# michiyasunaga/qagnn

Measured on AMD Instinct MI355X. Metric: QA-subgraphs/sec (batch x num_choice) fwd+bwd, higher is better.
Workload: dtype f32; 1 GPU; configs[1]: CSQA-shaped batch 64 questions x 5 choices = 320 subgraphs per GPU, n=200 node slots, 400..2000 edges/subgraph, 38 relations (run_qagnn__csqa.sh), 5-layer GAT d=200 H=4, QAGNN decoder fwd+bwd (LM encoder excluded: random sent_vecs), dropout 0.2, train-mode BN; subgraphs_per_gpu=320, nodes=64000, edges=396800, edges_with_self_loops=460800, graph_input=load-time int32 blobs (qagnn_graph_from_blobs), 13.3 B/edge on the wire, parallelism=single

## Files before the change

### include/qagnn_hip.h

```cpp
#ifndef QAGNN_HIP_H
#define QAGNN_HIP_H

#include <stdint.h>

#ifdef __cplusplus
extern "C" {
#endif

#define QAGNN_OK 0
#define QAGNN_EINVAL 1
#define QAGNN_EUNSUPPORTED 2
#define QAGNN_EHIP 3

typedef void* qagnn_stream_t;

const char* qagnn_last_error(void);
int qagnn_abi_version(void);

typedef struct qagnn_graph {
  int32_t N, E, Ep, R, T, C;
  int32_t* rowptr_s;
  int32_t* tgt_s;
  int32_t* src_s;
  int32_t* cls_s;
// ... 147 lines not shown

int qagnn_seed_epoch_advance(uint64_t delta, qagnn_stream_t stream);
int qagnn_seed_epoch_set(uint64_t value, qagnn_stream_t stream);

int qagnn_edge_attn_fwd_f32(const qagnn_graph* g, const float* KMQ, int32_t ldk, const float* EkEm, int32_t lde, int32_t HP,
                            float qscale, float* score, float* a, float* alpha, float* aggr, int32_t lda,
                            qagnn_stream_t stream);
int qagnn_edge_attn_bwd_f32(const qagnn_graph* g, const float* KMQ, int32_t ldk, const float* EkEm, int32_t lde, int32_t HP,
                            float qscale, const float* a, const float* alpha, const float* G, int32_t ldg, float* dKMQ,
                            float* dEkEm, float* ga, float* rs, float* cls_part, qagnn_stream_t stream);

typedef struct qagnn_hop_args {
  const qagnn_graph* g;
  int32_t N, DP, SP, HP, T;
  float qscale;
  const float* X;
  const float* S;
  const int64_t* ntype;
  const float* Wx_t; const float* Wx;
  const float* Ws_t; const float* Ws;
  const float* TT;
  const float* EkEm;
  const float* W1t; const float* W1; const float* b1;
  const float* gamma; const float* beta;
  const float* W2t; const float* W2; const float* b2;
  int32_t batch_stats;
  float eps;
  const float* run_mean_p; const float* run_var_p;
  float* run_mean; float* run_var; int64_t* num_batches_tracked;
  const int64_t* dense_pos; int32_t d; float momentum;
  int32_t apply_act; float p_drop; uint64_t seed;
  float* KMQ;
  float* a; float* alpha;
  float* aggr; float* h1; float* out; float* y;
  float* stats;
  const float* dy;
  float* dX;
  float* dS;
  int32_t accumulate_dS; int32_t accumulate_dX;
  float* dWx_t; float* dWs_t;
  float* dTT; float* dEkEm;
  float* dW1t; float* db1;
  float* dbn;
  float* dW2t; float* db2;
  float* ws; int64_t ws_elems;
  int32_t gemm_split;
  int32_t ones_col;
  int32_t tab_col;
  qagnn_stream_t side_stream;
  uint32_t* amax;
  const uint32_t* x_amax;
  const uint32_t* s_amax;
} qagnn_hop_args;
#define QAGNN_HOP_AMAX_WORDS 16
int64_t qagnn_hop_fwd_workspace_elems(int32_t N, int32_t Ep, int32_t DP);
int64_t qagnn_hop_bwd_workspace_elems(int32_t N, int32_t Ep, int32_t DP, int32_t SP,
                                      int32_t cls_part_rows );
int qagnn_hop_fwd_f32(const qagnn_hop_args* h, qagnn_stream_t stream);
int qagnn_hop_bwd_f32(const qagnn_hop_args* h, qagnn_stream_t stream);
int qagnn_stack_fwd_f32(const qagnn_hop_args* hops, int32_t k, qagnn_stream_t stream);
int qagnn_stack_bwd_f32(const qagnn_hop_args* hops, int32_t k, qagnn_stream_t stream);

int qagnn_node_prep_f32(const float* raw_scores, const int64_t* adj_len, const int64_t* node_type, const int64_t* concept_ids,
                        int32_t B, int32_t n, float* score, uint8_t* mask, int64_t* ridx, int64_t table_rows, int32_t* err,
                        qagnn_stream_t stream);

int qagnn_radam_step_f32(int32_t n_tensors, float* const* p, const float* const* g, float* const* m, float* const* v,
                         const int64_t* numel, double beta1, double beta2, double eps, double lr, double weight_decay, double step_size,
                         int32_t mode, qagnn_stream_t stream);

#ifdef __cplusplus
}
#endif
#endif
```

### qagnn_amd/_lib.py

```python
import ctypes as C
import functools
import os

import torch

_HERE = os.path.dirname(os.path.abspath(__file__))
LIB_PATH = os.environ.get('QAGNN_LIB') or os.path.join(_HERE, 'libqagnn_hip.so')

EXPORTS = ['qagnn_last_error', 'qagnn_abi_version', 'qagnn_graph_storage_elems', 'qagnn_graph_prep', 'qagnn_graph_prep_blocked',
           'qagnn_graph_from_blobs', 'qagnn_radam_step_f32', 'qagnn_node_prep_f32', 'qagnn_seed_epoch_advance', 'qagnn_seed_epoch_set',
           'qagnn_gemm_nn_f32', 'qagnn_gemm_nn_split_f32', 'qagnn_gemm_nn_pack_bytes', 'qagnn_gemm_nn_ws_bytes', 'qagnn_gemm_nn_split_ws_f32', 'qagnn_gemm_nn_prepack_bytes', 'qagnn_gemm_nn_prepack_f32',
           'qagnn_gemm_nn_prepack_clear', 'qagnn_gemm_tn_workspace_elems', 'qagnn_gemm_tn_f32', 'qagnn_gemm_tn2_f32', 'qagnn_gemm_tn_colsum_f32',
           'qagnn_colreduce_workspace_elems', 'qagnn_colreduce_f32', 'qagnn_bn_finalize_f32', 'qagnn_bn_stats_finalize_f32', 'qagnn_bn_relu_bwd_f32',
           'qagnn_gelu_dropout_fwd_f32', 'qagnn_gelu_dropout_bwd_f32', 'qagnn_sin_basis_f32',
           'qagnn_bn_relu_bwd_colsum_f32',
           'qagnn_pool_attn_fwd_f32', 'qagnn_pool_attn_bwd_f32', 'qagnn_head_post_fwd_f32', 'qagnn_head_post_bwd_f32', 'qagnn_add_row0_f32', 'qagnn_gather_multi_f32', 'qagnn_gather_multi_sum_f32',
           'qagnn_edge_attn_fwd_f32', 'qagnn_edge_attn_bwd_f32',
           'qagnn_hop_fwd_workspace_elems', 'qagnn_hop_bwd_workspace_elems', 'qagnn_hop_fwd_f32', 'qagnn_hop_bwd_f32',
           'qagnn_stack_fwd_f32', 'qagnn_stack_bwd_f32', 'qagnn_absmax_f32', 'qagnn_zero_words', 'qagnn_gemm_tn_h2_f32', 'qagnn_gelu_dropout_fwd_amax_f32', 'qagnn_gelu_dropout_amax_scratch_elems',
           'qagnn_timing_enable', 'qagnn_timing_read', 'qagnn_gemm_tn_h1_f32', 'qagnn_gelu_dropout_bwd_amax_f32', 'qagnn_packed_min_rows']

CLS_SLICES = 4
ABI_VERSION = 22

_i32, _i64, _f32, _u64, _vp = C.c_int32, C.c_int64, C.c_float, C.c_uint64, C.c_void_p


class qagnn_graph(C.Structure):
    _fields_ = ([(n, _i32) for n in ('N', 'E', 'Ep', 'R', 'T', 'C')] +
                [(n, _vp) for n in ('rowptr_s', 'tgt_s', 'src_s', 'cls_s', 'eid_s', 'rowptr_t', 'src_t', 'tgt_t', 'cls_t', 'pos_t',
                                    'cls_count', 'src_c', 'tgt_c', 'pos_c', 'chunk_cls', 'chunk_beg',
                                    'chunk_len', 'n_chunks', 'chunkptr')] +
                [('max_chunks', _i32), ('err', _vp), ('block_n', _i32), ('n_groups', _i32)])


GATHER_MAX = 160


class qagnn_gather_tabs(C.Structure):
    _fields_ = [('p', _vp * GATHER_MAX), ('n', _i32)]


class qagnn_pack_desc(C.Structure):
    _fields_ = [('B1n', _vp), ('ldn1', _i32), ('K1', _i32), ('B2n', _vp), ('ldn2', _i32), ('K2', _i32), ('No', _i32), ('pieces', _i32)]


class qagnn_gemm_nn_args(C.Structure):
    _fields_ = [('A1', _vp), ('lda1', _i32), ('K1', _i32), ('B1', _vp), ('ldb1', _i32),
                ('A2', _vp), ('lda2', _i32), ('K2', _i32), ('B2', _vp), ('ldb2', _i32),
                ('C', _vp), ('ldc', _i32), ('M', _i32), ('No', _i32),
                ('bias', _vp), ('rowtab', _vp), ('ldt', _i32), ('rowidx', _vp),
                ('a_scale', _vp), ('a_shift', _vp), ('accumulate', _i32), ('a_rowidx', _vp), ('xcd_remap', _i32), ('colstat_part', _vp),
                ('a_amax1', _vp), ('a_amax2', _vp), ('a_rows', _i64), ('pieces', _i32)]


class qagnn_hop_args(C.Structure):
    _fields_ = ([('g', C.POINTER(qagnn_graph))] + [(n, _i32) for n in ('N', 'DP', 'SP', 'HP', 'T')] + [('qscale', _f32)] +
                [(n, _vp) for n in ('X', 'S', 'ntype', 'Wx_t', 'Wx', 'Ws_t', 'Ws', 'TT', 'EkEm', 'W1t', 'W1', 'b1', 'gamma', 'beta',
                                    'W2t', 'W2', 'b2')] +
                [('batch_stats', _i32), ('eps', _f32), ('run_mean_p', _vp), ('run_var_p', _vp), ('run_mean', _vp), ('run_var', _vp),
                 ('num_batches_tracked', _vp), ('dense_pos', _vp), ('d', _i32), ('momentum', _f32),
                 ('apply_act', _i32), ('p_drop', _f32), ('seed', _u64)] +
                [(n, _vp) for n in ('KMQ', 'a', 'alpha', 'aggr', 'h1', 'out', 'y', 'stats', 'dy', 'dX', 'dS')] +
                [('accumulate_dS', _i32), ('accumulate_dX', _i32)] +
                [(n, _vp) for n in ('dWx_t', 'dWs_t', 'dTT', 'dEkEm', 'dW1t', 'db1', 'dbn', 'dW2t', 'db2', 'ws')] +
                [('ws_elems', _i64), ('gemm_split', _i32), ('ones_col', _i32), ('tab_col', _i32), ('side_stream', _vp), ('amax', _vp), ('x_amax', _vp), ('s_amax', _vp)])


HOP_AMAX_WORDS = 16


def load_library(path=LIB_PATH):
    if not os.path.exists(path):
        raise OSError(f'{path} not found: build it with `python -m qagnn_amd.build` (hipcc, gfx950)')
    lib = C.CDLL(path)
    lib.qagnn_last_error.restype = C.c_char_p
    lib.qagnn_abi_version.restype = _i32
    lib.qagnn_graph_storage_elems.restype = _i64
    lib.qagnn_graph_storage_elems.argtypes = [_i32, _i32, _i32, _i32]
    lib.qagnn_graph_prep.argtypes = [C.POINTER(qagnn_graph), _vp, _vp, _vp, _vp, _i32, _i32, _i32, _i32, _vp]
    lib.qagnn_graph_prep_blocked.argtypes = [C.POINTER(qagnn_graph), _vp, _vp, _vp, _vp, _i32, _i32, _i32, _i32, _i32, _vp]
    lib.qagnn_graph_from_blobs.argtypes = [C.POINTER(qagnn_graph), _vp, _vp, _vp, _vp, _vp, _i32, _i32, _i32, _i32, _i32, _vp]
    lib.qagnn_node_prep_f32.argtypes = [_vp, _vp, _vp, _vp, _i32, _i32, _vp, _vp, _vp, _i64, _vp, _vp]
    lib.qagnn_seed_epoch_advance.argtypes = [_u64, _vp]
    lib.qagnn_seed_epoch_set.argtypes = [_u64, _vp]
    lib.qagnn_radam_step_f32.argtypes = [_i32, _vp, _vp, _vp, _vp, _vp] + [C.c_double] * 6 + [_i32, _vp]
    lib.qagnn_gemm_nn_f32.argtypes = [C.POINTER(qagnn_gemm_nn_args), _vp]
    lib.qagnn_gemm_nn_split_f32.argtypes = [C.POINTER(qagnn_gemm_nn_args), _vp, _i32, _vp, _i32, _vp]
    lib.qagnn_gemm_nn_pack_bytes.restype = _i64
    lib.qagnn_gemm_nn_pack_bytes.argtypes = [_i32, _i32, _i32]
    lib.qagnn_gemm_nn_split_ws_f32.argtypes = [C.POINTER(qagnn_gemm_nn_args), _vp, _i32, _vp, _i32, _vp, _i64, _vp]
    lib.qagnn_gemm_nn_ws_bytes.restype = _i64
    lib.qagnn_gemm_nn_ws_bytes.argtypes = [C.POINTER(qagnn_gemm_nn_args), _vp, _i32, _vp, _i32]
    lib.qagnn_gemm_nn_prepack_bytes.restype = _i64
    lib.qagnn_gemm_nn_prepack_bytes.argtypes = [C.POINTER(qagnn_pack_desc), _i32]
    lib.qagnn_gemm_nn_prepack_f32.argtypes = [C.POINTER(qagnn_pack_desc), _i32, _vp, _i64, _i64, _vp]
    lib.qagnn_gemm_nn_prepack_clear.argtypes = [_i64]
    lib.qagnn_gemm_tn_workspace_elems.restype = _i64
    lib.qagnn_gemm_tn_workspace_elems.argtypes = [_i32, _i32, _i32]
    lib.qagnn_gemm_tn_f32.argtypes = [_vp, _i32, _vp, _i32, _vp, _i32, _i32, _i32, _i32, _vp, _vp, _vp, _i32, _vp, _vp]
    lib.qagnn_gemm_tn2_f32.argtypes = [_vp, _i32, _i32, _vp, _i32, _i32, _vp, _i32, _vp, _i32, _i32, _i32, _vp, _vp]
    lib.qagnn_gemm_tn_h2_f32.argtypes = [_vp, _i32, _i32, _vp, _i32, _i32, _vp, _i32, _vp, _i32, _i32, _i32, _vp, _vp, _vp, _vp, _vp, _vp, _vp]
    lib.qagnn_gemm_tn_h1_f32.argtypes = lib.qagnn_gemm_tn_h2_f32.argtypes
    lib.qagnn_absmax_f32.argtypes = [_vp, _i64, _vp, _vp]
    lib.qagnn_zero_words.argtypes = [_vp, _i64, _vp]
    lib.qagnn_timing_enable.argtypes = [_i32]
    lib.qagnn_timing_read.argtypes = [_vp, _vp]
    lib.qagnn_packed_min_rows.restype = _i64
    lib.qagnn_packed_min_rows.argtypes = [_i64]
    lib.qagnn_gemm_tn_colsum_f32.argtypes = [_vp, _i32, _vp, _i32, _vp, _i32, _i32, _i32, _i32, _vp, _vp, _vp, _i32, _vp, _vp, _i32,
                                             _vp, _vp]
    lib.qagnn_colreduce_workspace_elems.restype = _i64
    lib.qagnn_colreduce_workspace_elems.argtypes = [_i32, _i32, _i32]
    lib.qagnn_colreduce_f32.argtypes = [_i32, _vp, _i32, _vp, _i32, _i32, _i32, _vp, _i32, _vp, _vp, _vp, _vp, _vp, _f32, _vp, _vp, _vp]
    lib.qagnn_bn_finalize_f32.argtypes = [_vp, _vp, _vp, _vp, _f32, _vp, _vp, _vp, _i32, _vp, _vp, _vp, _vp, _i32, _f32, _f32, _i32, _vp]
    lib.qagnn_bn_stats_finalize_f32.argtypes = [_vp, _i32, _i32, _i32, _vp, _vp, _f32, _vp, _vp, _vp, _vp, _vp, _i32, _f32, _f32, _i32, _vp]
    lib.qagnn_bn_relu_bwd_f32.argtypes = [_vp, _vp, _vp, _i32, _i32, _i32, _vp, _vp, _vp, _vp, _vp, _vp, _vp, _f32, _vp, _vp]
    lib.qagnn_gelu_dropout_fwd_f32.argtypes = [_vp, _vp, _i64, _f32, _u64, _vp]
    lib.qagnn_gelu_dropout_bwd_f32.argtypes = [_vp, _vp, _vp, _i64, _f32, _u64, _vp]
    lib.qagnn_gelu_dropout_fwd_amax_f32.argtypes = [_vp, _vp, _i64, _f32, _u64, _vp, _vp, _vp]
    lib.qagnn_gelu_dropout_bwd_amax_f32.argtypes = [_vp, _vp, _vp, _i64, _f32, _u64, _vp, _vp, _vp]
    lib.qagnn_gelu_dropout_amax_scratch_elems.restype = _i64
# ... 821 lines not shown
```

### qagnn_amd/csrc/common.h

```cpp
#pragma once
#include <hip/hip_runtime.h>
#include <stdint.h>
#include <stdio.h>

#include <type_traits>

#include "../../include/qagnn_hip.h"

namespace qagnn {

void set_error(const char* fmt, ...);

struct NnProduct {
  const qagnn_gemm_nn_args* a;
  bool split;
  const float* B1n; int ldn1; const float* B2n; int ldn2;
  void* ws; int64_t ws_bytes;
};
enum class NnFamily { FP32, SPLIT, NN2 };
enum class NnB { IN_KERNEL, PACK, IMAGE };
struct NnRoute {
  NnFamily family;
  int nt, np, wv;
  bool affine, flat, stats;
  NnB b; const void* image;
  int64_t ws_bytes;
  int ntiles, grid;
};
inline int num_cus() {
  static int n = [] {
    int dev = 0, v = 0;
    if (hipGetDevice(&dev) != hipSuccess || hipDeviceGetAttribute(&v, hipDeviceAttributeMultiprocessorCount, dev) != hipSuccess || v <= 0) v = 256;
    return v;
  }();
  return n;
}
static inline int cdiv(int64_t a, int64_t b) { return (int)((a + b - 1) / b); }
inline void nn_grid(NnRoute& r, int M, int No, int rows_per_tile, int per_cu) {
  r.ntiles = cdiv(No, r.nt * 16) * cdiv(M, rows_per_tile);
  const int cap = (num_cus() * per_cu) & ~7;
  r.grid = r.ntiles < cap ? r.ntiles : cap;
}
NnRoute nn_route(const NnProduct& p);
bool nn_rows_packed(int64_t M);
int gemm_nn(const NnProduct& p, hipStream_t stream);
int launch_nn(const NnRoute& r, const qagnn_gemm_nn_args& a, hipStream_t stream);
int launch_nn_split(const NnRoute& r, const qagnn_gemm_nn_args& a, const float* B1n, int ldn1, const float* B2n, int ldn2, hipStream_t stream);
int launch_nn2(const NnRoute& r, const qagnn_gemm_nn_args& a, const float* B1n, int ldn1, const float* B2n, int ldn2, hipStream_t stream);
int launch_pack_b(int np, const qagnn_gemm_nn_args& a, const float* B1n, int ldn1, const float* B2n, int ldn2, void* ws, hipStream_t stream);
namespace nn2 { int walk_tiles(int K1, int K2); }
int64_t nn2_pack_bytes(int No, int K1, int K2, int np);
const void* nn2_prepack_lookup(const float* B1n, int ldn1, int K1, const float* B2n, int ldn2, int K2, int No, int np);

struct TnProduct {
  const float* A1; int lda1, Ka1;
  const float* A2; int lda2, Ka2; bool two;
  const float* B; int ldb;
  float* C; int ldc, R, No;
  const float* a_scale; const float* a_shift; const int64_t* a_rowidx; int accumulate;
  float* bsum; const int64_t* b_rowidx; int groups;
  const uint32_t* amax[3]; int np;
  float* ws;
};
inline TnProduct tn_product(const float* A1, int lda1, int Ka1, const float* A2, int lda2, int Ka2, const float* B, int ldb, float* C, int ldc, int R,
                            int No, const float* a_scale, const float* a_shift, float* ws, const uint32_t* amax_a1 = nullptr,
                            const uint32_t* amax_a2 = nullptr, const uint32_t* amax_b = nullptr, int np = 3) {
  TnProduct p = {};
  p.A1 = A1; p.lda1 = lda1; p.Ka1 = Ka1;
  if (A2 && Ka2 > 0) { p.A2 = A2; p.lda2 = lda2; p.Ka2 = Ka2; p.two = true; }
  p.B = B; p.ldb = ldb; p.C = C; p.ldc = ldc; p.R = R; p.No = No; p.a_scale = a_scale; p.a_shift = a_shift; p.ws = ws;
  p.amax[0] = amax_a1; p.amax[1] = amax_a2; p.amax[2] = amax_b; p.np = np;
  return p;
}
enum class TnFamily { RUNTIME, STRIP, SPLIT, WS, PAIR };
struct TnRoute {
  TnFamily family;
  int kt, nt, waves, np;
  bool affine, gather, colsum;
  int chunk_rows, nchunks;
  bool sum_by4;
  dim3 grid;
  int64_t ws_elems;
};
TnRoute tn_route(const TnProduct& p);
int gemm_tn(const TnProduct& p, hipStream_t stream);
int launch_tn(const TnRoute& r, const TnProduct& p, float* Pcs, hipStream_t stream);
int launch_tn_strip(const TnRoute& r, const TnProduct& p, float* Pcs, hipStream_t stream);
int launch_tn_split(const TnRoute& r, const TnProduct& p, hipStream_t stream);
int launch_tn_ws(const TnRoute& r, const TnProduct& p, hipStream_t stream);
int launch_sum_chunks(const float* P, float* C, int ldc, int rows, int No, int nchunks, int accumulate, bool by4, hipStream_t stream);

int launch_gelu_dropout(const float* X, const float* dY, float* out, int64_t n, float p, uint64_t seed, uint32_t* amax, float* amax_part,
                        hipStream_t stream);
int64_t gelu_amax_scratch_elems(int64_t n);
int launch_bn_relu_bwd_colsum(const float* dR, const float* Hh, float* dH, int ld, int R, int Cc, const float* mean, const float* invstd,
                              const float* scale, const float* shift, const float* gamma, const float* sum_dy, const float* sum_dy_hhat,
                              float inv_rows, const float* roww, float* colsum, float* workspace, uint32_t* amax, hipStream_t stream);
int launch_bn_stats_finalize(const float* part, int n_tiles, int R, int Cc, const float* gamma, const float* beta, float eps, float* stats,
                             float* run_mean, float* run_var, int64_t* nbt, int d, float momentum, float unbias, int ones_col, uint32_t* amax_bound,
                             hipStream_t stream);

int launch_edge_attn_fwd(const qagnn_graph* g, const float* KMQ, int32_t ldk, const float* EkEm, int32_t lde, int32_t HP, float qscale,
                         float* score, float* a, float* alpha, float* aggr, int32_t lda, float* amax_part , hipStream_t stream);
int launch_edge_attn_bwd(const qagnn_graph* g, const float* KMQ, int32_t ldk, const float* EkEm, int32_t lde, int32_t HP, float qscale,
                         const float* a, const float* alpha, const float* G, int32_t ldg, float* dKMQ, float* dEkEm, float* ga, float* rs,
                         float* cls_part, float* amax_part , uint32_t* amax_slot, hipStream_t stream);
int launch_amax_reduce(const float* part, int64_t n, uint32_t* slot, hipStream_t stream);

struct TimedScope {
  int kind;
  hipStream_t s;
  hipEvent_t e0, e1;
  bool counted;
  TimedScope(int kind, hipStream_t s);
  ~TimedScope();
  TimedScope(const TimedScope&) = delete;
  TimedScope& operator=(const TimedScope&) = delete;
};

#define QAGNN_REQUIRE(cond, code, ...) \
  do {                                 \
    if (!(cond)) {                     \
      qagnn::set_error(__VA_ARGS__);   \
      return (code);                   \
    }                                  \
  } while (0)

#define QAGNN_LAUNCH_CHECK(name)                                               \
  do {                                                                         \
    hipError_t e__ = hipGetLastError();                                        \
    if (e__ != hipSuccess) {                                                   \
      qagnn::set_error("%s launch failed: %s", name, hipGetErrorString(e__));  \
      return QAGNN_EHIP;                                                       \
    }                                                                          \
  } while (0)

#ifndef QAGNN_NN_OCC
#define QAGNN_NN_OCC 2
#endif

template <int V0, int... Vs, class F>
inline int dispatch_int(int v, F&& f) {
  if constexpr (sizeof...(Vs) == 0) return f(std::integral_constant<int, V0>{});
  else return v == V0 ? f(std::integral_constant<int, V0>{}) : dispatch_int<Vs...>(v, f);
}
template <class F>
inline int dispatch_bool(bool v, F&& f) { return v ? f(std::true_type{}) : f(std::false_type{}); }

template <auto KERNEL>
inline int raise_lds_limit(int bytes, const char* name) {
  static bool raised[64] = {};
  int dev = 0;
  if (hipGetDevice(&dev) != hipSuccess) dev = 0;
  if (bytes <= 64 * 1024 || raised[dev & 63]) return QAGNN_OK;
  hipError_t e = hipFuncSetAttribute((const void*)KERNEL, hipFuncAttributeMaxDynamicSharedMemorySize, bytes);
  if (e != hipSuccess) { set_error("%s: cannot raise the dynamic LDS limit: %s", name, hipGetErrorString(e)); return QAGNN_EHIP; }
// ... 96 lines not shown
  const f16x2 l = {(_Float16)(xs - (float)h[0]), (_Float16)(ys - (float)h[1])};
  hi = __builtin_bit_cast(uint32_t, h);
  lo = __builtin_bit_cast(uint32_t, l);
}
#define QAGNN_BF(V) __builtin_bit_cast(bf16x8, V)
#define QAGNN_HF(V) __builtin_bit_cast(f16x8, V)
template <int NP, bool SWAP = false>
__device__ __forceinline__ f32x4s mfma_pieces(const u32x4s* __restrict__ a, const u32x4s* __restrict__ b, f32x4s c) {
#define QAGNN_MF3(I, J) c = SWAP ? __builtin_amdgcn_mfma_f32_16x16x32_bf16(QAGNN_BF(b[J]), QAGNN_BF(a[I]), c, 0, 0, 0) \
                                 : __builtin_amdgcn_mfma_f32_16x16x32_bf16(QAGNN_BF(a[I]), QAGNN_BF(b[J]), c, 0, 0, 0);
#define QAGNN_MF2(I, J) c = SWAP ? __builtin_amdgcn_mfma_f32_16x16x32_f16(QAGNN_HF(b[J]), QAGNN_HF(a[I]), c, 0, 0, 0) \
                                 : __builtin_amdgcn_mfma_f32_16x16x32_f16(QAGNN_HF(a[I]), QAGNN_HF(b[J]), c, 0, 0, 0);
  if constexpr (NP == 3) {
    QAGNN_MF3(2, 0) QAGNN_MF3(0, 2) QAGNN_MF3(1, 1) QAGNN_MF3(1, 0) QAGNN_MF3(0, 1) QAGNN_MF3(0, 0)
  } else if constexpr (NP == 2) {
    QAGNN_MF2(1, 0) QAGNN_MF2(0, 1) QAGNN_MF2(0, 0)
  } else {
    QAGNN_MF2(0, 0)
  }
#undef QAGNN_MF3
#undef QAGNN_MF2
  return c;
}

__device__ __forceinline__ float4 ld4(const float* p) { return *reinterpret_cast<const float4*>(p); }
__device__ __forceinline__ void st4(float* p, float4 v) { *reinterpret_cast<float4*>(p) = v; }
__device__ __forceinline__ float dot4(float4 a, float4 b) { return a.x * b.x + a.y * b.y + a.z * b.z + a.w * b.w; }
__device__ __forceinline__ float4 add4(float4 a, float4 b) { return make_float4(a.x + b.x, a.y + b.y, a.z + b.z, a.w + b.w); }
__device__ __forceinline__ float4 fma4(float s, float4 a, float4 acc) {
  return make_float4(fmaf(s, a.x, acc.x), fmaf(s, a.y, acc.y), fmaf(s, a.z, acc.z), fmaf(s, a.w, acc.w));
}

__device__ __forceinline__ float wave_amax_lane63(float m) {
  m = row16_max(m);
  int b = __builtin_bit_cast(int, m);
  m = fmaxf(m, __builtin_bit_cast(float, __builtin_amdgcn_update_dpp(b, b, 0x142, 0xA, 0xF, false)));
  b = __builtin_bit_cast(int, m);
  m = fmaxf(m, __builtin_bit_cast(float, __builtin_amdgcn_update_dpp(b, b, 0x143, 0xC, 0xF, false)));
  return m;
}
__device__ __forceinline__ void block_amax_merge(float m, uint32_t* __restrict__ amax, float* __restrict__ red) {
  m = wave_amax_lane63(m);
  const int lane = threadIdx.x & 63, w = threadIdx.x >> 6, nw = (blockDim.x + 63) >> 6;
  if (lane == 63) red[w] = m;
  __syncthreads();
  if (threadIdx.x == 0) {
    float t = red[0];
    for (int i = 1; i < nw; ++i) t = fmaxf(t, red[i]);
    if (t > 0.f) __hip_atomic_fetch_max(amax, __builtin_bit_cast(uint32_t, t), __ATOMIC_RELAXED, __HIP_MEMORY_SCOPE_AGENT);
  }
}
__device__ __forceinline__ float absmax4(float4 v) { return fmaxf(fmaxf(fabsf(v.x), fabsf(v.y)), fmaxf(fabsf(v.z), fabsf(v.w))); }


}
```

### qagnn_amd/csrc/edge_attn.hip

```cpp
#include "common.h"

namespace qagnn {

#ifndef EDGE_UNROLL
#define EDGE_UNROLL 4
#endif
#define TGT_UNROLL 4

typedef __amdgpu_buffer_rsrc_t rsrc_t;
constexpr uint32_t OOB_OFF = 0x7FFFFFF0u;
__device__ __forceinline__ rsrc_t make_rsrc(const void* base, uint32_t bytes) {
  return __builtin_amdgcn_make_buffer_rsrc(const_cast<void*>(base), 0, (int)bytes, 0x00020000);
}
__device__ __forceinline__ float4 buf_ld4(rsrc_t r, uint32_t voff, uint32_t soff) {
  return __builtin_bit_cast(float4, __builtin_amdgcn_raw_buffer_load_b128(r, (int)voff, (int)soff, 0));
}

constexpr int SLAB_ROWS = 72;

struct Lane {
  int lane, w, g, j;
  bool act;
  uint32_t voff;
  int off;
// ... 100 lines not shown
    sc[grp] = -INFINITY;
    if (grp * 16 < cnt) {
      const int gcnt = min(16, cnt - grp * 16);
      for (int i = 0; i < gcnt; i += EDGE_UNROLL) {
        float4 k[EDGE_UNROLL], ek[EDGE_UNROLL];
#pragma unroll
        for (int u = 0; u < EDGE_UNROLL; ++u) {
          const int idx = min(grp * 16 + i + u, cnt - 1);
          k[u] = buf_ld4(rK, L.voff, rl(tv, idx));
          ek[u] = buf_ld4(rE, L.voff, rl(cv, idx));
        }
#pragma unroll
        for (int u = 0; u < EDGE_UNROLL; ++u) {
          const float p = row16_sum(dot4(q, add4(k[u], ek[u]))) * qscale;
          sc[grp] = (L.j == i + u) ? p : sc[grp];
        }
      }
    }
  }
  float m = sc[0];
  m = (L.j < cnt) ? m : -INFINITY;
#pragma unroll
  for (int grp = 1; grp < 4; ++grp)
    if (grp * 16 < cnt) m = (grp * 16 + L.j < cnt) ? fmaxf(m, sc[grp]) : m;
  m = row16_max(m);
  float ex[4], sum = 0.f;
#pragma unroll
  for (int grp = 0; grp < 4; ++grp) {
    ex[grp] = 0.f;
    if (grp * 16 < cnt) {
      ex[grp] = (grp * 16 + L.j < cnt) ? expf(sc[grp] - m) : 0.f;
      sum += ex[grp];
    }
  }
  sum = row16_sum(sum) + 1e-16f;
#pragma unroll
  for (int grp = 0; grp < 4; ++grp) {
    if (grp * 16 < cnt) {
      if (grp * 16 + L.j < cnt) {
        const float av = ex[grp] / sum;
        const int64_t o = (int64_t)(beg + grp * 16 + L.j) * 4 + L.g;
        a[o] = av;
        alpha[o] = av * deg;
      }
    }
  }
}

__device__ __forceinline__ void node_amax(float m, float* __restrict__ part, int node) {
  m = wave_amax_lane63(m);
  if ((threadIdx.x & 63) == 63) part[node] = m;
}

__global__ __launch_bounds__(256) void k_edge_aggregate(const int* __restrict__ rowptr_t, const int* __restrict__ src_t,
                                                        const int* __restrict__ cls_t, const int* __restrict__ pos_t,
                                                        const float* __restrict__ KMQ, int ldk, const float* __restrict__ EkEm,
                                                        int lde, int HP, const float* __restrict__ alpha,
                                                        float* __restrict__ aggr, int lda, int N, int C, const int* __restrict__ xcd_base,
                                                        float* __restrict__ amax_part) {
  __shared__ float4 slab[4][SLAB_ROWS];
  const int t = wave_node(xcd_base);
  if (t >= N) return;
  const Lane L = lane_info(HP);
  const int DP = 4 * HP;
  const uint32_t pk = (uint32_t)ldk * 4u, pe = (uint32_t)lde * 4u, vm = L.voff + (uint32_t)DP * 4u;
  const rsrc_t rK = make_rsrc(KMQ, (uint32_t)N * pk), rE = make_rsrc(EkEm, (uint32_t)C * pe);
  const int beg = __builtin_amdgcn_readfirstlane(rowptr_t[t]), end = __builtin_amdgcn_readfirstlane(rowptr_t[t + 1]);
  if (end - beg == 1) {
    const int sv = __builtin_amdgcn_readfirstlane(src_t[beg]), cv = __builtin_amdgcn_readfirstlane(cls_t[beg]);
    const int pv = __builtin_amdgcn_readfirstlane(pos_t[beg]);
    const float4 m1 = buf_ld4(rK, vm, (uint32_t)sv * pk), em1 = buf_ld4(rE, vm, (uint32_t)cv * pe);
    const float al = alpha[(int64_t)pv * 4 + L.g];
    const float4 o1 = fma4(al, add4(m1, em1), zero4());
    if (L.act) st4(aggr + (int64_t)t * lda + L.off, o1);
    if (amax_part) node_amax(L.act ? absmax4(o1) : 0.f, amax_part, t);
    return;
  }
  slab_init(slab[L.w], L.lane);
  const float* const sl = reinterpret_cast<const float*>(slab[L.w]) + L.g;
  float4 acc = zero4();
  for (int e0 = beg; e0 < end; e0 += 64) {
    const int cnt = min(64, end - e0), lc = e0 + min(L.lane, cnt - 1);
    const uint32_t sv = (uint32_t)src_t[lc] * pk, cv = (uint32_t)cls_t[lc] * pe;
    slab[L.w][L.lane] = L.lane < cnt ? ld4(alpha + (int64_t)pos_t[lc] * 4) : zero4();
    for (int i = 0; i < cnt; i += EDGE_UNROLL) {
      float4 m[EDGE_UNROLL], em[EDGE_UNROLL];
#pragma unroll
      for (int u = 0; u < EDGE_UNROLL; ++u) {
        const int idx = min(i + u, cnt - 1);
        m[u] = buf_ld4(rK, vm, rl(sv, idx));
        em[u] = buf_ld4(rE, vm, rl(cv, idx));
      }
#pragma unroll
      for (int u = 0; u < EDGE_UNROLL; ++u) acc = fma4(sl[(i + u) * 4], add4(m[u], em[u]), acc);
    }
  }
  if (L.act) st4(aggr + (int64_t)t * lda + L.off, acc);
  if (amax_part) node_amax(L.act ? absmax4(acc) : 0.f, amax_part, t);
}

__global__ __launch_bounds__(256) void k_edge_bwd_src1(const int* __restrict__ rowptr_s, const int* __restrict__ tgt_s,
                                                       const int* __restrict__ cls_s, const float* __restrict__ KMQ, int ldk,
                                                       const float* __restrict__ EkEm, int lde, int HP,
                                                       const float* __restrict__ a, const float* __restrict__ alpha,
                                                       const float* __restrict__ G, int ldg, float* __restrict__ dKMQ,
                                                       float* __restrict__ ga, float* __restrict__ rs, int N, int C,
                                                       const int* __restrict__ xcd_base, float* __restrict__ amax_part) {
  __shared__ float4 slab[3][4][SLAB_ROWS];
  const int s = wave_node(xcd_base);
  if (s >= N) return;
  const Lane L = lane_info(HP);
  const int DP = 4 * HP;
  const uint32_t pk = (uint32_t)ldk * 4u, pe = (uint32_t)lde * 4u, pg = (uint32_t)ldg * 4u, vm = L.voff + (uint32_t)DP * 4u;
  const rsrc_t rK = make_rsrc(KMQ, (uint32_t)N * pk), rE = make_rsrc(EkEm, (uint32_t)C * pe), rG = make_rsrc(G, (uint32_t)N * pg);
  const int beg = __builtin_amdgcn_readfirstlane(rowptr_s[s]), end = __builtin_amdgcn_readfirstlane(rowptr_s[s + 1]);
  if (end - beg == 1) {
    const float4 g1 = buf_ld4(rG, L.voff, (uint32_t)s * pg);
    if (L.act) st4(dKMQ + (int64_t)s * ldk + DP + L.off, g1);
    if (amax_part) node_amax(L.act ? absmax4(g1) : 0.f, amax_part, s);
    if (L.lane == 0) {
      st4(ga + (int64_t)beg * 4, zero4());
      st4(rs + (int64_t)s * 4, zero4());
    }
    return;
  }
  const float4 mrow = buf_ld4(rK, vm, (uint32_t)s * pk);
  const float deg = (float)(end - beg);
  slab_init(slab[0][L.w], L.lane);
  slab_init(slab[1][L.w], L.lane);
  const float* const sl_a = reinterpret_cast<const float*>(slab[0][L.w]) + L.g;
  const float* const sl_al = reinterpret_cast<const float*>(slab[1][L.w]) + L.g;
  float* const sl_ga = reinterpret_cast<float*>(slab[2][L.w]) + L.g;
  float4 dM = zero4();
  float r = 0.f;
  for (int e0 = beg; e0 < end; e0 += 64) {
    const int cnt = min(64, end - e0), lc = e0 + min(L.lane, cnt - 1);
    const uint32_t tv = (uint32_t)tgt_s[lc] * pg, cv = (uint32_t)cls_s[lc] * pe;
    slab[0][L.w][L.lane] = L.lane < cnt ? ld4(a + (int64_t)lc * 4) : zero4();
    slab[1][L.w][L.lane] = L.lane < cnt ? ld4(alpha + (int64_t)lc * 4) : zero4();
    for (int i = 0; i < cnt; i += EDGE_UNROLL) {
      float4 g4[EDGE_UNROLL], em[EDGE_UNROLL];
#pragma unroll
      for (int u = 0; u < EDGE_UNROLL; ++u) {
        const int idx = min(i + u, cnt - 1);
        g4[u] = buf_ld4(rG, L.voff, rl(tv, idx));
        em[u] = buf_ld4(rE, vm, rl(cv, idx));
      }
#pragma unroll
      for (int u = 0; u < EDGE_UNROLL; ++u) {
        dM = fma4(sl_al[(i + u) * 4], g4[u], dM);
        const float gae = deg * row16_sum(dot4(add4(mrow, em[u]), g4[u]));
// ... 165 lines not shown
    int seen = 0;
    for (int g = sl; g < NG; g += QAGNN_CLS_SLICES) {
      const int kb = cp_lo[g], ke = cp_hi[g];
      const int first = (part - seen % P + P) % P;
      for (int k = kb + first; k < ke; k += P) acc = add4(acc, ld4(cls_part + (int64_t)k * DP2 + col4 * 4));
      seen += ke - kb;
    }
    sm4[part * ncol4 + col4] = acc;
  }
  __syncthreads();
  if (threadIdx.x < ncol4) {
    float4 s = sm4[threadIdx.x];
    for (int q = 1; q < P; ++q) s = add4(s, sm4[q * ncol4 + threadIdx.x]);
    st4(slices + ((int64_t)c * QAGNN_CLS_SLICES + sl) * DP2 + threadIdx.x * 4, s);
  }
}
__global__ __launch_bounds__(256) void k_cls_reduce2(const float* __restrict__ slices, float* __restrict__ dEkEm, int lde, int DP2, int C,
                                                     const float* __restrict__ amax_part, int npart, uint32_t* __restrict__ amax_slot) {
  const int ncol4 = DP2 >> 2;
  const int i = blockIdx.x * blockDim.x + threadIdx.x;
  if (i < C * ncol4) {
    const int c = i / ncol4, col4 = i - c * ncol4;
    const float* p = slices + (int64_t)c * QAGNN_CLS_SLICES * DP2 + col4 * 4;
    float4 s = ld4(p);
#pragma unroll
    for (int q = 1; q < QAGNN_CLS_SLICES; ++q) s = add4(s, ld4(p + (int64_t)q * DP2));
    st4(dEkEm + (int64_t)c * lde + col4 * 4, s);
  }
  if (amax_part) {
    __shared__ float red[16];
    float m = 0.f;
    for (int k = i; k < npart; k += (int)(gridDim.x * blockDim.x)) m = fmaxf(m, amax_part[k]);
    block_amax_merge(m, amax_slot, red);
  }
}

static int check_common(const qagnn_graph* g, const float* KMQ, int ldk, const float* EkEm, int lde, int HP, const char* who) {
  QAGNN_REQUIRE(g && KMQ && EkEm, QAGNN_EINVAL, "%s: null pointer", who);
  QAGNN_REQUIRE(HP > 0 && HP % 4 == 0 && HP <= 64, QAGNN_EUNSUPPORTED, "%s: head pitch HP=%d must be a multiple of 4, <= 64", who, HP);
  QAGNN_REQUIRE(ldk >= 12 * HP && ldk % 4 == 0 && lde >= 8 * HP && lde % 4 == 0, QAGNN_EINVAL, "%s: ldk=%d lde=%d too small for HP=%d",
                who, ldk, lde, HP);
  QAGNN_REQUIRE(aligned16(KMQ) && aligned16(EkEm), QAGNN_EINVAL, "%s: operands must be 16-byte aligned", who);
  QAGNN_REQUIRE((int64_t)g->N * ldk * 4 < (int64_t)OOB_OFF && (int64_t)g->C * lde * 4 < (int64_t)OOB_OFF, QAGNN_EUNSUPPORTED,
                "%s: N=%d x ldk=%d floats exceed the 2 GiB a buffer descriptor of these kernels addresses", who, g->N, ldk);
  return QAGNN_OK;
}

}

using namespace qagnn;

namespace qagnn {
int launch_edge_attn_fwd(const qagnn_graph* g, const float* KMQ, int32_t ldk, const float* EkEm, int32_t lde, int32_t HP, float qscale,
                         float* score, float* a, float* alpha, float* aggr, int32_t lda, float* amax_part, hipStream_t stream) {
  TimedScope timed(2, stream);
  int rc = check_common(g, KMQ, ldk, EkEm, lde, HP, "edge_attn_fwd");
  if (rc != QAGNN_OK) return rc;
  QAGNN_REQUIRE(score && a && alpha && aggr && lda >= 4 * HP && lda % 4 == 0 && aligned16(aggr), QAGNN_EINVAL,
                "edge_attn_fwd: bad output arguments");
  const int nb = 8 * edge_xcd_cap(g->N);
  k_edge_scores<<<nb, 256, 0, stream>>>(g->rowptr_s, g->tgt_s, g->cls_s, KMQ, ldk, EkEm, lde, HP, qscale, score, a, alpha, g->N, g->C, g->err + 4);
  QAGNN_LAUNCH_CHECK("k_edge_scores");
  k_edge_aggregate<<<nb, 256, 0, stream>>>(g->rowptr_t, g->src_t, g->cls_t, g->pos_t, KMQ, ldk, EkEm, lde, HP, alpha, aggr, lda, g->N, g->C, g->err + 4, amax_part);
  QAGNN_LAUNCH_CHECK("k_edge_aggregate");
  return QAGNN_OK;
}
}

extern "C" int qagnn_edge_attn_fwd_f32(const qagnn_graph* g, const float* KMQ, int32_t ldk, const float* EkEm, int32_t lde,
                                       int32_t HP, float qscale, float* score, float* a, float* alpha, float* aggr, int32_t lda,
                                       qagnn_stream_t stream_) {
  return launch_edge_attn_fwd(g, KMQ, ldk, EkEm, lde, HP, qscale, score, a, alpha, aggr, lda, nullptr, (hipStream_t)stream_);
}

extern "C" int qagnn_edge_attn_bwd_f32(const qagnn_graph* g, const float* KMQ, int32_t ldk, const float* EkEm, int32_t lde,
                                       int32_t HP, float qscale, const float* a, const float* alpha, const float* G, int32_t ldg,
                                       float* dKMQ, float* dEkEm, float* ga, float* rs, float* cls_part, qagnn_stream_t stream_) {
  return launch_edge_attn_bwd(g, KMQ, ldk, EkEm, lde, HP, qscale, a, alpha, G, ldg, dKMQ, dEkEm, ga, rs, cls_part, nullptr, nullptr, (hipStream_t)stream_);
}

int qagnn::launch_edge_attn_bwd(const qagnn_graph* g, const float* KMQ, int32_t ldk, const float* EkEm, int32_t lde, int32_t HP, float qscale,
                                const float* a, const float* alpha, const float* G, int32_t ldg, float* dKMQ, float* dEkEm, float* ga, float* rs,
                                float* cls_part, float* amax_part, uint32_t* amax_slot, hipStream_t stream) {
  TimedScope timed(3, stream);
  int rc = check_common(g, KMQ, ldk, EkEm, lde, HP, "edge_attn_bwd");
  if (rc != QAGNN_OK) return rc;
  QAGNN_REQUIRE(a && alpha && G && dKMQ && dEkEm && ga && rs && cls_part, QAGNN_EINVAL, "edge_attn_bwd: null pointer");
  QAGNN_REQUIRE(ldg >= 4 * HP && ldg % 4 == 0 && aligned16(G) && aligned16(dKMQ) && aligned16(dEkEm) && aligned16(cls_part),
                QAGNN_EINVAL, "edge_attn_bwd: bad pitch / alignment");
  QAGNN_REQUIRE((int64_t)g->N * ldg * 4 < (int64_t)OOB_OFF, QAGNN_EUNSUPPORTED, "edge_attn_bwd: G exceeds 2 GiB");
  const int DP2 = 8 * HP;
  QAGNN_REQUIRE(DP2 / 4 <= 1024, QAGNN_EUNSUPPORTED, "edge_attn_bwd: HP too large");
  const int nb = 8 * edge_xcd_cap(g->N);
  k_edge_bwd_src1<<<nb, 256, 0, stream>>>(g->rowptr_s, g->tgt_s, g->cls_s, KMQ, ldk, EkEm, lde, HP, a, alpha, G, ldg, dKMQ, ga, rs, g->N, g->C, g->err + 4, amax_part);
  QAGNN_LAUNCH_CHECK("k_edge_bwd_src1");
  k_edge_bwd_src2<<<nb, 256, 0, stream>>>(g->rowptr_s, g->tgt_s, g->cls_s, KMQ, ldk, EkEm, lde, HP, qscale, a, dKMQ, ga, rs, g->N, g->C, g->err + 4, amax_part ? amax_part + g->N : nullptr);
  QAGNN_LAUNCH_CHECK("k_edge_bwd_src2");
  k_edge_bwd_tgt<<<nb, 256, 0, stream>>>(g->rowptr_t, g->src_t, g->pos_t, KMQ, ldk, HP, ga, dKMQ, g->N, g->err + 4, amax_part ? amax_part + 2 * (int64_t)g->N : nullptr);
  QAGNN_LAUNCH_CHECK("k_edge_bwd_tgt");
  k_edge_bwd_cls<<<cdiv(g->max_chunks, 4), 256, 0, stream>>>(g->n_chunks, g->chunk_beg, g->chunk_len, g->src_c, g->tgt_c, g->pos_c,
                                                             KMQ, ldk, HP, alpha, ga, G, ldg, cls_part, g->N);
  QAGNN_LAUNCH_CHECK("k_edge_bwd_cls");
  const int cr_threads = g->Ep < 65536 && DP2 / 4 <= 128 ? 256 : 1024;
  const int P = cr_threads / (DP2 / 4);
  float* slices = cls_part + (int64_t)g->max_chunks * DP2;
  k_cls_reduce<<<dim3(g->C, QAGNN_CLS_SLICES), cr_threads, (size_t)P * (DP2 / 4) * sizeof(float4), stream>>>(g->chunkptr, cls_part, slices, DP2,
                                                                                                          g->C, g->n_groups);
  QAGNN_LAUNCH_CHECK("k_cls_reduce");
  k_cls_reduce2<<<cdiv((int64_t)g->C * (DP2 / 4), 256), 256, 0, stream>>>(slices, dEkEm, lde, DP2, g->C, amax_slot ? amax_part : nullptr, 3 * g->N, amax_slot);
  QAGNN_LAUNCH_CHECK("k_cls_reduce2");
  return QAGNN_OK;
}
```

### qagnn_amd/csrc/elementwise.hip

```cpp
#include "common.h"

namespace qagnn {

constexpr int CR_WR_BIG = 32, CR_WR_SMALL = 8;
static inline int cr_wr(int R) { return R < 32768 ? CR_WR_SMALL : CR_WR_BIG; }

template <int MODE, int CR_WR>
__global__ __launch_bounds__(256) void k_colreduce(const float* __restrict__ X, int ldx, const float* __restrict__ X2, int ldx2,
                                                   int R, int Cc, const int64_t* __restrict__ rowidx, int groups,
                                                   const float* __restrict__ mean, const float* __restrict__ invstd,
                                                   const float* __restrict__ scale, const float* __restrict__ shift,
                                                   const float* __restrict__ roww, float* __restrict__ part) {
  constexpr int NOUT = MODE == 0 ? 4 : (MODE == 2 ? 2 : 1);
  __shared__ __attribute__((aligned(16))) float red[4][NOUT][256];
  const int lane = threadIdx.x & 63, w = threadIdx.x >> 6;
  const int col = blockIdx.x * 256 + lane * 4;
  const bool act = col < Cc;
  constexpr int CR_ROWS = 4 * CR_WR;
  const int r0 = blockIdx.y * CR_ROWS + w * CR_WR;
  float4 acc[NOUT];
#pragma unroll
  for (int o = 0; o < NOUT; ++o) acc[o] = make_float4(0.f, 0.f, 0.f, 0.f);
  float4 mu = make_float4(0.f, 0.f, 0.f, 0.f), is = mu, sc = mu, sh = mu;
  if (act && MODE >= 1) mu = ld4(mean + col);
// ... 174 lines not shown
    }
    __syncthreads();
  }
  if (q == 0 && c < Cc) {
    const float mean = a.mean, var = fmaxf(a.m2 / (float)R, 0.f);
    const float is = rsqrtf(var + eps), sc = gamma[c] * is;
    stats[c] = mean;
    stats[Cc + c] = var;
    stats[2 * Cc + c] = is;
    stats[3 * Cc + c] = c == ones_col ? 0.f : sc;
    stats[4 * Cc + c] = c == ones_col ? 1.f : beta[c] - mean * sc;
    if (amax_bound) {
      const float bnd = c == ones_col ? 1.f : 1.01f * (fabsf(gamma[c]) * sqrtf((float)R) + fabsf(beta[c]));
      atomicMax(amax_bound, __builtin_bit_cast(uint32_t, bnd));
    }
    if (run_mean) {
      const int HP = Cc >> 2, dh = d >> 2, h = c / HP, j = c - h * HP;
      if (j < dh) {
        const int i = h * dh + j;
        run_mean[i] += momentum * (mean - run_mean[i]);
        run_var[i] += momentum * (var * unbias - run_var[i]);
      }
    }
  }
  if (nbt && blockIdx.x == 0 && threadIdx.x == 0) *nbt += 1;
}

__device__ __forceinline__ float gelu_f(float x) {
  const float u = 0.7978845608028654f * (x + 0.044715f * x * x * x);
  return 0.5f * x * (1.f + tanhf(u));
}
__device__ __forceinline__ float gelu_grad_f(float x) {
  const float x2 = x * x;
  const float u = 0.7978845608028654f * (x + 0.044715f * x * x2);
  const float t = tanhf(u);
  return 0.5f * (1.f + t) + 0.5f * x * (1.f - t * t) * 0.7978845608028654f * (1.f + 3.f * 0.044715f * x2);
}
template <bool BWD>
__device__ __forceinline__ float4 gelu_dropout_val(float4 x, float4 g, int64_t i, float p, uint64_t seed, float inv) {
  float4 o;
#define ONE(f, k)                                                                  \
  {                                                                                \
    const float keep = (p > 0.f && uniform01(seed, (uint64_t)i * 4 + k) < p) ? 0.f : inv; \
    o.f = BWD ? g.f * keep * gelu_grad_f(x.f) : keep * gelu_f(x.f);                \
  }
  ONE(x, 0) ONE(y, 1) ONE(z, 2) ONE(w, 3)
#undef ONE
  return o;
}
template <bool BWD>
__device__ __forceinline__ float4 gelu_dropout_one(const float* __restrict__ X, const float* __restrict__ dY, int64_t i, float p, uint64_t seed, float inv) {
  return gelu_dropout_val<BWD>(ld4(X + i * 4), BWD ? ld4(dY + i * 4) : make_float4(1.f, 1.f, 1.f, 1.f), i, p, seed, inv);
}
template <bool BWD, bool AMAX = false>
__global__ __launch_bounds__(256) void k_gelu_dropout(const float* __restrict__ X, const float* __restrict__ dY, float* __restrict__ out, int64_t n4,
                                                      float p, uint64_t seed, const unsigned long long* __restrict__ epoch,
                                                      float* __restrict__ amax_part = nullptr) {
  if (p > 0.f) seed = epoch_seed(seed, epoch);
  const float inv = p > 0.f ? 1.f / (1.f - p) : 1.f;
  const int64_t i = (int64_t)blockIdx.x * blockDim.x + threadIdx.x;
  if (!AMAX && i >= n4) return;
  float4 o = make_float4(0.f, 0.f, 0.f, 0.f);
  if (i < n4) {
    o = gelu_dropout_one<BWD>(X, dY, i, p, seed, inv);
    st4(out + i * 4, o);
  }
  if constexpr (AMAX) {
    __shared__ float red[4];
    const float m = wave_amax_lane63(absmax4(o));
    if ((threadIdx.x & 63) == 63) red[threadIdx.x >> 6] = m;
    __syncthreads();
    if (threadIdx.x == 0) amax_part[blockIdx.x] = fmaxf(fmaxf(red[0], red[1]), fmaxf(red[2], red[3]));
  }
}

template <bool N1>
__global__ __launch_bounds__(256) void k_absmax(const float* __restrict__ x, int64_t n, uint32_t* __restrict__ slot) {
  __shared__ float red[16];
  float m = 0.f;
  for (int64_t i = (int64_t)blockIdx.x * 256 + threadIdx.x; i < n; i += (int64_t)gridDim.x * 256) {
    if constexpr (N1) m = fmaxf(m, fabsf(x[i]));
    else m = fmaxf(m, absmax4(ld4(x + i * 4)));
  }
  block_amax_merge(m, slot, red);
}
__global__ void k_zero_words(uint32_t* __restrict__ p, int64_t n) {
  for (int64_t i = (int64_t)blockIdx.x * blockDim.x + threadIdx.x; i < n; i += (int64_t)gridDim.x * blockDim.x) p[i] = 0u;
}

template <int CR_WR>
__global__ __launch_bounds__(256) void k_bn_relu_bwd_colsum(const float* __restrict__ dR, const float* __restrict__ Hh, float* __restrict__ dH,
                                                            int ld, int R, int Cc, const float* __restrict__ mean,
                                                            const float* __restrict__ invstd, const float* __restrict__ scale,
                                                            const float* __restrict__ shift, const float* __restrict__ gamma,
                                                            const float* __restrict__ k1v, const float* __restrict__ k2v, float inv_rows,
                                                            const float* __restrict__ roww, float* __restrict__ part,
                                                            uint32_t* __restrict__ amax) {
  __shared__ __attribute__((aligned(16))) float red[4][256];
  const int lane = threadIdx.x & 63, w = threadIdx.x >> 6;
  const int col = blockIdx.x * 256 + lane * 4;
  const bool act = col < Cc;
  constexpr int CR_ROWS = 4 * CR_WR;
  const int r0 = blockIdx.y * CR_ROWS + w * CR_WR;
  float4 acc = make_float4(0.f, 0.f, 0.f, 0.f);
  float am = 0.f;
  if (act) {
    const float4 mu = ld4(mean + col), is = ld4(invstd + col), sc = ld4(scale + col), sh = ld4(shift + col);
    const float4 ga = ld4(gamma + col), k1 = ld4(k1v + col), k2 = ld4(k2v + col);
    const int rend = min(R, r0 + CR_WR);
    for (int rb = r0; rb < rend; rb += 8) {
      float4 xs[8], hs[8];
#pragma unroll
      for (int u = 0; u < 8; ++u) {
        const int r = min(rb + u, rend - 1);
        xs[u] = ld4(dR + (int64_t)r * ld + col);
        hs[u] = ld4(Hh + (int64_t)r * ld + col);
      }
#pragma unroll
      for (int u = 0; u < 8; ++u) {
        const int r = rb + u;
        if (r >= rend) break;
        const float4 x = xs[u], h = hs[u];
        const float ir = roww ? roww[r] : inv_rows;
        float4 o;
#define ONE(f)                                                          \
// ... 118 lines not shown

namespace qagnn {
int launch_bn_stats_finalize(const float* part, int n_tiles, int R, int Cc, const float* gamma, const float* beta, float eps, float* stats,
                             float* run_mean, float* run_var, int64_t* nbt, int d, float momentum, float unbias, int ones_col, uint32_t* amax_bound,
                             hipStream_t stream) {
  k_bn_stats_finalize<<<cdiv(Cc, BF_COLS), BF_COLS * BF_PARTS, 0, stream>>>(part, n_tiles, R, Cc, gamma, beta, eps, stats, run_mean, run_var, nbt, d,
                                                                            momentum, unbias, ones_col, amax_bound);
  QAGNN_LAUNCH_CHECK("k_bn_stats_finalize");
  return QAGNN_OK;
}
}

extern "C" int qagnn_bn_stats_finalize_f32(const float* part, int32_t n_tiles, int32_t R, int32_t Cc, const float* gamma, const float* beta,
                                           float eps, float* stats, float* run_mean, float* run_var, int64_t* num_batches_tracked,
                                           const int64_t* dense_pos, int32_t d, float momentum, float unbias, int32_t ones_col,
                                           qagnn_stream_t stream_) {
  hipStream_t stream = (hipStream_t)stream_;
  QAGNN_REQUIRE(part && gamma && beta && stats && R > 0 && Cc > 0 && n_tiles == cdiv(R, ST_TILE), QAGNN_EINVAL,
                "bn_stats_finalize: bad arguments (R=%d needs %d tiles of %d rows, got %d)", R, cdiv(R, ST_TILE), ST_TILE, n_tiles);
  QAGNN_REQUIRE(!run_mean || (run_var && d > 0 && d % 4 == 0 && Cc % 4 == 0 && d <= Cc), QAGNN_EINVAL, "bn_stats_finalize: running-stat arguments");
  (void)dense_pos;
  return launch_bn_stats_finalize(part, n_tiles, R, Cc, gamma, beta, eps, stats, run_mean, run_var, num_batches_tracked, d, momentum, unbias, ones_col,
                                  nullptr, stream);
}

__global__ __launch_bounds__(256) void k_gather_multi(qagnn_gather_tabs t, const int* __restrict__ tid, const int* __restrict__ off,
                                                     float* __restrict__ out, int total) {
  __shared__ const float* ps[QAGNN_GATHER_MAX];
  for (int i = threadIdx.x; i < t.n; i += blockDim.x) ps[i] = t.p[i];
  __syncthreads();
  const int i = blockIdx.x * blockDim.x + threadIdx.x;
  if (i >= total) return;
  const int k = tid[i];
  out[i] = k >= 0 ? ps[k][off[i]] : 0.f;
}

__global__ __launch_bounds__(256) void k_gather_multi_sum(qagnn_gather_tabs t, const int* __restrict__ tid, const int* __restrict__ off, int K, int S,
                                                         float* __restrict__ out) {
  __shared__ const float* ps[QAGNN_GATHER_MAX];
  for (int i = threadIdx.x; i < t.n; i += blockDim.x) ps[i] = t.p[i];
  __syncthreads();
  const int s = blockIdx.x * blockDim.x + threadIdx.x;
  if (s >= S) return;
  float acc = 0.f;
  for (int k = 0; k < K; ++k) {
    const int g = tid[(int64_t)k * S + s];
    const float* p = g >= 0 ? ps[g] : nullptr;
    const float v = p != nullptr ? p[off[(int64_t)k * S + s]] : 0.f;
    acc = k == 0 ? v : acc + v;
  }
  out[s] = acc;
}

extern "C" int qagnn_gather_multi_f32(const qagnn_gather_tabs* t, const int32_t* tid, const int32_t* off, float* out, int32_t total,
                                      qagnn_stream_t stream_) {
  QAGNN_REQUIRE(t && t->n > 0 && t->n <= QAGNN_GATHER_MAX && tid && off && out && total > 0, QAGNN_EINVAL, "gather_multi: bad arguments");
  for (int i = 0; i < t->n; ++i) QAGNN_REQUIRE(t->p[i] != nullptr, QAGNN_EINVAL, "gather_multi: null source %d", i);
  k_gather_multi<<<cdiv(total, 256), 256, 0, (hipStream_t)stream_>>>(*t, tid, off, out, total);
  QAGNN_LAUNCH_CHECK("k_gather_multi");
  return QAGNN_OK;
}

extern "C" int qagnn_gather_multi_sum_f32(const qagnn_gather_tabs* t, const int32_t* tid, const int32_t* off, int32_t K, int32_t S, float* out,
                                          qagnn_stream_t stream_) {
  QAGNN_REQUIRE(t && t->n > 0 && t->n <= QAGNN_GATHER_MAX && tid && off && out && K > 0 && S > 0, QAGNN_EINVAL, "gather_multi_sum: bad arguments");
  k_gather_multi_sum<<<cdiv(S, 256), 256, 0, (hipStream_t)stream_>>>(*t, tid, off, K, S, out);
  QAGNN_LAUNCH_CHECK("k_gather_multi_sum");
  return QAGNN_OK;
}

namespace qagnn {
int64_t gelu_amax_scratch_elems(int64_t n) { return cdiv(n / 4, 256); }
int launch_gelu_dropout(const float* X, const float* dY, float* out, int64_t n, float p, uint64_t seed, uint32_t* amax, float* amax_part,
                        hipStream_t stream) {
  const int grid = cdiv(n / 4, 256);
  if (amax && !amax_part) { set_error("gelu_dropout: the maximum needs its scratch"); return QAGNN_EINVAL; }
  if (dY) {
    if (amax) k_gelu_dropout<true, true><<<grid, 256, 0, stream>>>(X, dY, out, n / 4, p, seed, seed_epoch_ptr(), amax_part);
    else k_gelu_dropout<true><<<grid, 256, 0, stream>>>(X, dY, out, n / 4, p, seed, seed_epoch_ptr());
  } else {
    if (amax) k_gelu_dropout<false, true><<<grid, 256, 0, stream>>>(X, nullptr, out, n / 4, p, seed, seed_epoch_ptr(), amax_part);
    else k_gelu_dropout<false><<<grid, 256, 0, stream>>>(X, nullptr, out, n / 4, p, seed, seed_epoch_ptr());
  }
  QAGNN_LAUNCH_CHECK("k_gelu_dropout");
  return amax ? launch_amax_reduce(amax_part, grid, amax, stream) : QAGNN_OK;
}
}

extern "C" int qagnn_gelu_dropout_fwd_f32(const float* X, float* Y, int64_t n, float p, uint64_t seed, qagnn_stream_t stream_) {
  hipStream_t stream = (hipStream_t)stream_;
  QAGNN_REQUIRE(X && Y && n > 0 && n % 4 == 0 && aligned16(X) && aligned16(Y), QAGNN_EINVAL, "gelu_dropout_fwd: bad args");
  QAGNN_REQUIRE(p >= 0.f && p < 1.f, QAGNN_EINVAL, "gelu_dropout_fwd: p=%f", p);
  return launch_gelu_dropout(X, nullptr, Y, n, p, seed, nullptr, nullptr, stream);
}

extern "C" int64_t qagnn_gelu_dropout_amax_scratch_elems(int64_t n) { return gelu_amax_scratch_elems(n); }
extern "C" int qagnn_gelu_dropout_fwd_amax_f32(const float* X, float* Y, int64_t n, float p, uint64_t seed, uint32_t* amax, float* scratch,
                                               qagnn_stream_t stream_) {
  QAGNN_REQUIRE(X && Y && amax && scratch && n > 0 && n % 4 == 0 && aligned16(X) && aligned16(Y), QAGNN_EINVAL, "gelu_dropout_fwd_amax: bad args");
  QAGNN_REQUIRE(p >= 0.f && p < 1.f, QAGNN_EINVAL, "gelu_dropout_fwd_amax: p=%f", p);
  return launch_gelu_dropout(X, nullptr, Y, n, p, seed, amax, scratch, (hipStream_t)stream_);
}

extern "C" int qagnn_gelu_dropout_bwd_amax_f32(const float* X, const float* dY, float* dX, int64_t n, float p, uint64_t seed, uint32_t* amax,
                                               float* scratch, qagnn_stream_t stream_) {
  QAGNN_REQUIRE(X && dY && dX && amax && scratch && n > 0 && n % 4 == 0 && aligned16(X) && aligned16(dY) && aligned16(dX), QAGNN_EINVAL,
                "gelu_dropout_bwd_amax: bad args");
  QAGNN_REQUIRE(p >= 0.f && p < 1.f, QAGNN_EINVAL, "gelu_dropout_bwd_amax: p=%f", p);
  return launch_gelu_dropout(X, dY, dX, n, p, seed, amax, scratch, (hipStream_t)stream_);
}

extern "C" int qagnn_gelu_dropout_bwd_f32(const float* X, const float* dY, float* dX, int64_t n, float p, uint64_t seed,
                                          qagnn_stream_t stream_) {
  hipStream_t stream = (hipStream_t)stream_;
  QAGNN_REQUIRE(X && dY && dX && n > 0 && n % 4 == 0 && aligned16(X) && aligned16(dY) && aligned16(dX), QAGNN_EINVAL,
                "gelu_dropout_bwd: bad args");
  QAGNN_REQUIRE(p >= 0.f && p < 1.f, QAGNN_EINVAL, "gelu_dropout_bwd: p=%f", p);
  return launch_gelu_dropout(X, dY, dX, n, p, seed, nullptr, nullptr, stream);
}

extern "C" int qagnn_absmax_f32(const float* x, int64_t n, uint32_t* slot, qagnn_stream_t stream_) {
  QAGNN_REQUIRE(x && slot && n > 0 && n % 4 == 0 && aligned16(x), QAGNN_EINVAL, "absmax: bad arguments");
  const int64_t n4 = n / 4;
  const int grid = (int)(n4 / 256 + 1 < 1024 ? n4 / 256 + 1 : 1024);
  k_absmax<false><<<grid, 256, 0, (hipStream_t)stream_>>>(x, n4, slot);
  QAGNN_LAUNCH_CHECK("k_absmax");
  return QAGNN_OK;
}

int qagnn::launch_amax_reduce(const float* part, int64_t n, uint32_t* slot, hipStream_t stream) {
  const int grid = (int)(n / 1024 + 1 < 64 ? n / 1024 + 1 : 64);
  k_absmax<true><<<grid, 256, 0, stream>>>(part, n, slot);
  QAGNN_LAUNCH_CHECK("k_amax_reduce");
  return QAGNN_OK;
}

extern "C" int qagnn_zero_words(uint32_t* p, int64_t n, qagnn_stream_t stream_) {
  QAGNN_REQUIRE(p && n > 0, QAGNN_EINVAL, "zero_words: bad arguments");
// ... 110 lines not shown
```

### qagnn_amd/csrc/gemm_dispatch.hip

```cpp
#include <stdlib.h>

#include <atomic>
#include <initializer_list>

#include "common.h"

namespace qagnn {

static int pick_nt(int No) {
  const int cands[5] = {13, 7, 8, 4, 2};
  for (int c : cands)
    if (No % (c * 16) == 0) return c;
  int best = 4;
  int64_t best_cost = INT64_MAX;
  for (int c : cands) {
    const int64_t cost = (int64_t)cdiv(No, c * 16) * c * 16;
    if (cost < best_cost) { best_cost = cost; best = c; }
  }
  return best;
}

static std::atomic<int64_t> g_pack_min_m{8192};
bool nn_rows_packed(int64_t M) { return M >= g_pack_min_m.load(std::memory_order_relaxed); }

// ... 2 lines not shown
  if (a.a_rowidx && !(a.a_rows > 0 && a.a_rows * (int64_t)a.lda1 * 4 < lim && a.K2 == 0)) return false;
  if (a.K1 % 8 != 0 || a.K2 % 8 != 0) return false;
  if ((int64_t)a.M * a.lda1 * 4 >= lim || (int64_t)a.No * ldn1 * 4 >= lim || (int64_t)a.M * a.ldc * 4 >= lim) return false;
  if (a.K2 > 0 && ((int64_t)a.M * a.lda2 * 4 >= lim || (int64_t)a.No * ldn2 * 4 >= lim)) return false;
  if (a.K2 > 0 && (a.K1 & 31) != 0 && a.K2 < 32 - (a.K1 & 31)) return false;
  if (a.a_scale && a.K1 > 256) return false;
  return true;
}
static bool nn2_staggered(int nt, const qagnn_gemm_nn_args& a) {
  return nt >= 8 && nn2::walk_tiles(a.K1, a.K2) >= 10 && (int64_t)cdiv(a.No, nt * 16) * cdiv(a.M, 256) * 10 >= num_cus() * 9;
}

NnRoute nn_route(const NnProduct& p) {
  const qagnn_gemm_nn_args& a = *p.a;
  NnRoute r = {};
  r.np = 3;
  r.affine = a.a_scale != nullptr;
  if (!p.split) {
    r.family = NnFamily::FP32;
    r.nt = pick_nt(a.No);
    r.wv = 8;
    nn_grid(r, a.M, a.No, 128, QAGNN_NN_OCC > 0 ? QAGNN_NN_OCC : 1);
    return r;
  }
  const int nt16 = cdiv(a.No, 16);
  r.nt = nt16 >= 13 ? 13 : nt16 >= 8 ? 8 : nt16 >= 7 ? 7 : nt16 >= 4 ? 4 : 2;
  for (int c : {7, 4, 2})
    if (cdiv(a.M, 128) * cdiv(a.No, r.nt * 16) < num_cus() * 3 / 2 && c < r.nt) r.nt = c;
  r.wv = 4;
  r.stats = a.colstat_part != nullptr;
  if (!nn2_ok(a, p.ldn1, p.ldn2)) {
    const int64_t lim = (int64_t)0x7FFFFFFF;
    r.family = NnFamily::SPLIT;
    r.flat = a.a_rowidx || (int64_t)a.M * a.lda1 * 4 >= lim || (int64_t)a.M * a.lda2 * 4 >= lim || (int64_t)a.No * p.ldn1 * 4 >= lim ||
             (int64_t)a.No * p.ldn2 * 4 >= lim;
    nn_grid(r, a.M, a.No, 128, 2);
    return r;
  }
  r.family = NnFamily::NN2;
  auto image = [&](int np) {
    const int64_t need = nn2_pack_bytes(a.No, a.K1, a.K2, np);
    if ((r.image = nn2_prepack_lookup(p.B1n, p.ldn1, a.K1, p.B2n, p.ldn2, a.K2, a.No, np))) r.b = NnB::IMAGE;
    else if (p.ws && nn_rows_packed(a.M) && p.ws_bytes >= need && (np == 3 || aligned16(p.ws))) { r.b = NnB::PACK; r.ws_bytes = need; }
    else return false;
    r.np = np;
    return true;
  };
  const bool scaled = nn_rows_packed(a.M) && a.a_amax1 && (a.K2 == 0 || a.a_amax2);
  if (!(scaled && image(a.pieces == 1 ? 1 : 2)) && !image(3)) r.b = NnB::IN_KERNEL;
  if (r.b != NnB::IN_KERNEL && r.np == 3 && nn2_staggered(r.nt, a)) r.wv = 8;
  nn_grid(r, a.M, a.No, r.wv * 32, r.wv == 8 ? 1 : 2);
  return r;
}

static int nn_validate(const NnProduct& p) {
  QAGNN_REQUIRE(p.a, QAGNN_EINVAL, "gemm_nn: null pointer");
  const qagnn_gemm_nn_args& a = *p.a;
  const float* B1 = p.split ? p.B1n : a.B1, *B2 = p.split ? p.B2n : a.B2;
  const int ldb1 = p.split ? p.ldn1 : a.ldb1, ldb2 = p.split ? p.ldn2 : a.ldb2, km = p.split ? 4 : 16;
  QAGNN_REQUIRE(a.A1 && B1 && a.C, QAGNN_EINVAL, "gemm_nn: null pointer");
  QAGNN_REQUIRE(a.M > 0 && a.No > 0 && a.K1 > 0, QAGNN_EINVAL, "gemm_nn: bad sizes M=%d No=%d K1=%d", a.M, a.No, a.K1);
  QAGNN_REQUIRE(a.K1 % km == 0 && a.K2 % km == 0 && a.K2 >= 0, QAGNN_EINVAL, "gemm_nn: K1=%d K2=%d must be multiples of %d", a.K1, a.K2, km);
  QAGNN_REQUIRE(a.No % 4 == 0, QAGNN_EINVAL, "gemm_nn: No=%d must be a multiple of 4", a.No);
  QAGNN_REQUIRE(a.lda1 % 4 == 0 && ldb1 % 4 == 0 && (!p.split || ldb1 >= a.K1) && aligned16(a.A1) && aligned16(B1), QAGNN_EINVAL,
                "gemm_nn: operand 1 must be 16-byte aligned with pitches multiple of 4");
  QAGNN_REQUIRE(a.K2 == 0 || (a.A2 && B2 && a.lda2 % 4 == 0 && ldb2 % 4 == 0 && (!p.split || ldb2 >= a.K2) && aligned16(a.A2) && aligned16(B2)),
                QAGNN_EINVAL, "gemm_nn: operand 2 must be 16-byte aligned with pitches multiple of 4");
  QAGNN_REQUIRE(!a.rowtab || a.rowidx, QAGNN_EINVAL, "gemm_nn: rowtab without rowidx");
  QAGNN_REQUIRE(a.ldc % 4 == 0 && aligned16(a.C) && (!a.bias || aligned16(a.bias)) && (!a.rowtab || (aligned16(a.rowtab) && a.ldt % 4 == 0)),
                QAGNN_EINVAL, "gemm_nn: C / bias / rowtab must be 16-byte aligned with pitches multiple of 4");
  QAGNN_REQUIRE(!a.a_scale || (a.a_shift && aligned16(a.a_scale) && aligned16(a.a_shift)), QAGNN_EINVAL,
                "gemm_nn: a_scale/a_shift must both be given and 16-byte aligned");
  if (p.split && a.colstat_part) {
    const int64_t lim = (int64_t)0x7FFFFFFF;
    QAGNN_REQUIRE(cdiv(a.No, 16) == 13 && !a.a_scale && !a.a_rowidx && !a.rowtab && !a.accumulate && a.K2 == 0, QAGNN_EUNSUPPORTED,
                  "gemm_nn: column statistics need 193..208 output columns and a bias-only epilogue (No=%d)", a.No);
    QAGNN_REQUIRE((int64_t)a.M * a.lda1 * 4 < lim && (int64_t)a.No * ldb1 * 4 < lim, QAGNN_EUNSUPPORTED,
                  "gemm_nn: column statistics with operands of 2 GB and more");
  }
  return QAGNN_OK;
}

int gemm_nn(const NnProduct& p, hipStream_t stream) {
  TimedScope timed(0, stream);
  if (int rc = nn_validate(p)) return rc;
  const qagnn_gemm_nn_args& a = *p.a;
  const NnRoute r = nn_route(p);
  if (r.family == NnFamily::FP32) return launch_nn(r, a, stream);
  if (r.family == NnFamily::SPLIT) return launch_nn_split(r, a, p.B1n, p.ldn1, p.B2n, p.ldn2, stream);
  if (r.b == NnB::IN_KERNEL) return launch_nn2(r, a, p.B1n, p.ldn1, p.B2n, p.ldn2, stream);
  if (r.b == NnB::PACK) {
    QAGNN_REQUIRE(aligned16(p.ws), QAGNN_EINVAL, "gemm_nn: the pack workspace must be 16-byte aligned");
    if (int rc = launch_pack_b(r.np, a, p.B1n, p.ldn1, p.B2n, p.ldn2, p.ws, stream)) return rc;
  }
  return launch_nn2(r, a, static_cast<const float*>(r.b == NnB::PACK ? p.ws : r.image), cdiv(a.No, 16), nullptr, 0, stream);
}

static int tn_chunk_rows(int R, int blocks_per_chunk, int per_cu, int ktile, int lo) {
  const int target = num_cus() * per_cu / blocks_per_chunk;
  const int rows = cdiv(cdiv(R, target > 0 ? target : 1), ktile) * ktile, lo_k = cdiv(lo, ktile) * ktile;
  return rows > lo_k ? rows : lo_k;
}
static int tn_min_chunk(int R, bool split) { return R > 4096 ? 256 : split ? 32 : 64; }
static int64_t tn_ws_bound(int R, int Ka, int No) { return (int64_t)cdiv(R, tn_min_chunk(R, true)) * ((int64_t)Ka * No + 4 * (int64_t)No); }
constexpr int TN_WS_MIN_TILES = 28;

static int pick_tn_waves(int Ka) {
  int best = 4, best_waste = INT32_MAX;
  for (int nw = 16; nw >= 4; --nw) {
    const int bm = nw * 16, waste = cdiv(Ka, bm) * bm - Ka;
    if (waste < best_waste) { best_waste = waste; best = nw; }
  }
  return best;
}
static bool tn_split_ok(const TnProduct& p, int Ka, int lda) {
  static const int mode = getenv("QAGNN_GEMM_SPLIT") ? atoi(getenv("QAGNN_GEMM_SPLIT")) : 1;
  const bool gather = p.a_rowidx != nullptr;
  const int64_t big = (int64_t)p.R * ((lda > p.ldb && !gather) ? lda : p.ldb) * 4;
  if (gather && (Ka <= 112 || p.a_scale)) return false;
  return mode != 0 && Ka >= 64 && p.No >= 104 && p.R >= 1024 && big < (int64_t)0x7FFFFFFF;
}

TnRoute tn_route(const TnProduct& p) {
  TnRoute r = {};
  r.np = 3;
  r.affine = p.a_scale != nullptr;
  r.gather = p.a_rowidx != nullptr;
  r.colsum = p.bsum != nullptr;
  r.sum_by4 = p.ldc % 4 == 0 && aligned16(p.C);
  const bool split = !r.colsum && tn_split_ok(p, p.Ka1, p.lda1) && (!p.two || (r.sum_by4 && tn_split_ok(p, p.Ka2, p.lda2)));
  const int lo = tn_min_chunk(p.R, split);
  int row_blocks;
  if (split) {
    if (r.sum_by4 && !r.gather && p.amax[0] && p.amax[2] && (!p.two || p.amax[1])) r.np = p.np;
    r.kt = (p.two || p.Ka1 <= 112) ? 7 : 13;
    r.nt = 20 - r.kt;
    row_blocks = cdiv(p.Ka1, r.kt * 16) + (p.two ? cdiv(p.Ka2, r.kt * 16) : 0);
    const int bpc = cdiv(p.No, r.nt * 16) * row_blocks;
    r.chunk_rows = tn_chunk_rows(p.R, bpc, 2, 32, lo);
    r.family = TnFamily::SPLIT;
    if (p.two) {
      const int rows1 = tn_chunk_rows(p.R, bpc, 1, 32, lo);
      if (rows1 >= 2 * TN_WS_MIN_TILES * 32) r.chunk_rows = rows1;
      if (r.chunk_rows >= TN_WS_MIN_TILES * 32) r.family = TnFamily::WS;
    }
  } else if (p.two) {
    r.family = TnFamily::PAIR;
    return r;
// ... 123 lines not shown
```

### qagnn_amd/csrc/gemm_nn2.hip

```cpp
#include <stdlib.h>


#include "common.h"

namespace qagnn {


namespace nn2 {

#ifndef QAGNN_NN2_ABL
#define QAGNN_NN2_ABL 0
#endif

constexpr int BK = 32;
constexpr uint32_t OOB = 0x80000000u;

__device__ __forceinline__ u32x4s bload(__amdgpu_buffer_rsrc_t rsrc, uint32_t voff, uint32_t soff) {
  return __builtin_bit_cast(u32x4s, __builtin_amdgcn_raw_buffer_load_b128(rsrc, (int)voff, (int)soff, 0));
}

__device__ __forceinline__ void split3(uint32_t u, uint32_t& h1, uint32_t& h2, uint32_t& h3) {
  h1 = u & 0xFFFF0000u;
  const float r1 = __builtin_bit_cast(float, u) - __builtin_bit_cast(float, h1);
  h2 = __builtin_bit_cast(uint32_t, r1) & 0xFFFF0000u;
// ... 12 lines not shown
    float x = __builtin_bit_cast(float, ux), y = __builtin_bit_cast(float, uy);
    if constexpr (AFFINE) {
      x = fmaxf(fmaf(x, sc[e], sh[e]), lo);
      y = fmaxf(fmaf(y, sc[e + 1], sh[e + 1]), lo);
    }
    if constexpr (NP == 2) split2(x, y, s, ph[e >> 1], pl[e >> 1]);
    else split1(x, y, s, ph[e >> 1]);
  }
  f[0] = (u32x4s){ph[0], ph[1], ph[2], ph[3]};
  if constexpr (NP == 2) f[1] = (u32x4s){pl[0], pl[1], pl[2], pl[3]};
}

template <bool AFFINE>
__device__ __forceinline__ void split_frag(const u32x4s (&r)[2], u32x4s (&f)[3], const float* __restrict__ sc, const float* __restrict__ sh, float lo) {
  uint32_t h1[8], h2[8], h3[8];
#pragma unroll
  for (int e = 0; e < 8; ++e) {
    uint32_t u = r[e >> 2][e & 3];
    if constexpr (AFFINE) u = __builtin_bit_cast(uint32_t, fmaxf(fmaf(__builtin_bit_cast(float, u), sc[e], sh[e]), lo));
    split3(u, h1[e], h2[e], h3[e]);
  }
  const u32x4s p1 = {pack_hi(h1[0], h1[1]), pack_hi(h1[2], h1[3]), pack_hi(h1[4], h1[5]), pack_hi(h1[6], h1[7])};
  const u32x4s p2 = {pack_hi(h2[0], h2[1]), pack_hi(h2[2], h2[3]), pack_hi(h2[4], h2[5]), pack_hi(h2[6], h2[7])};
  const u32x4s p3 = {pack_hi(h3[0], h3[1]), pack_hi(h3[2], h3[3]), pack_hi(h3[4], h3[5]), pack_hi(h3[6], h3[7])};
  f[0] = p1;
  f[1] = p2;
  f[2] = p3;
}

__device__ __forceinline__ void store_b4(unsigned char* __restrict__ dst, u32x4s v) {
  uint32_t a1, a2, a3, b1, b2, b3, c1, c2, c3, d1, d2, d3;
  split3(v[0], a1, a2, a3);
  split3(v[1], b1, b2, b3);
  split3(v[2], c1, c2, c3);
  split3(v[3], d1, d2, d3);
  *reinterpret_cast<uint2*>(dst) = make_uint2(pack_hi(a1, b1), pack_hi(c1, d1));
  *reinterpret_cast<uint2*>(dst + 1024) = make_uint2(pack_hi(a2, b2), pack_hi(c2, d2));
  *reinterpret_cast<uint2*>(dst + 2048) = make_uint2(pack_hi(a3, b3), pack_hi(c3, d3));
}

#define QAGNN_NN2_SIX_T(C, AF, BF) C = mfma_pieces<NP, true>(AF, BF, C);
#define QAGNN_NN2_SIX(C, AF, BF) C = mfma_pieces<NP>(AF, BF, C);

template <int NT, bool STATS, int WV, int NP = 3>
constexpr int nn2_lds_bytes(int aff_bytes) {
  const int ring = (WV == 8 ? 3 : 2) * NT * NP * 1024 + aff_bytes;
  const int epi = WV * 16 * (NT * 16 + 4) * 4 + (STATS ? WV * 2 * NT * 16 * 4 : 0);
  return ring > epi ? ring : epi;
}

template <int NT, bool AFFINE, bool STATS, int NP, bool PACKED, int WV = 4>
__global__ __launch_bounds__(WV * 64) __attribute__((amdgpu_waves_per_eu(2, 2))) void k_gemm_nn2(qagnn_gemm_nn_args a, const float* __restrict__ B1n,
                                                                                          int ldn1, const float* __restrict__ B2n, int ldn2,
                                                                                          int ntiles) {
  static_assert(WV == 4 || (WV == 8 && PACKED), "the staggered block takes B by DMA only");
  static_assert(NP == 3 || (NP <= 2 && PACKED && WV == 4), "the scaled fp16 forms (two pieces: three MFMAs; one piece: one MFMA): packed B, 4-wave blocks");
  static_assert(!(AFFINE && STATS), "no product needs both");
  constexpr bool STAG = WV == 8;
  constexpr bool DIRECT = PACKED && !STATS;
  constexpr int THR = WV * 64, BM = WV * 32;
  constexpr int BN = NT * 16;
  constexpr int IMG = NT * NP * 1024;
  constexpr int RING_B = (STAG ? 3 : 2) * IMG;
  constexpr int BR = (NT + 1) / 2;
  constexpr int PS = BN + 4, SLAB_ROWS = 16;
  constexpr int SLAB_B = WV * SLAB_ROWS * PS * 4;
  static_assert(DIRECT || SLAB_B + (STATS ? WV * 2 * BN * 4 : 0) <= (AFFINE ? RING_B : nn2_lds_bytes<NT, STATS, WV, NP>(0)), "the epilogue reuses the k-loop's LDS");
  extern __shared__ __attribute__((aligned(16))) unsigned char smem[];
  float* const aff = reinterpret_cast<float*>(smem + RING_B);

  const int tid = threadIdx.x, lane = tid & 63;
  const int w = __builtin_amdgcn_readfirstlane(tid >> 6);
  const int M = a.M, No = a.No, K1 = a.K1, K2 = a.K2;
  const int ncb = (No + BN - 1) / BN;
  const int r1 = K2 > 0 ? (K1 & 31) : 0;
  const int mixi = r1 != 0 ? 1 : 0;
  const int n1 = mixi ? (K1 >> 5) : ((K1 + 31) >> 5);
  const int s2 = mixi ? 32 - r1 : 0;
  const int n2 = K2 > s2 ? ((K2 - s2 + 31) >> 5) : 0;
  const int nkt = mixi + n1 + n2;
  const int KA = (K1 + 31) & ~31;

  const __amdgpu_buffer_rsrc_t rA1 = __builtin_amdgcn_make_buffer_rsrc(const_cast<float*>(a.A1), 0, (a.a_rowidx ? (int)a.a_rows : M) * a.lda1 * 4, 0x00020000);
  const __amdgpu_buffer_rsrc_t rA2 = __builtin_amdgcn_make_buffer_rsrc(const_cast<float*>(a.A2), 0, K2 > 0 ? M * a.lda2 * 4 : 0, 0x00020000);
  const __amdgpu_buffer_rsrc_t rB1 = __builtin_amdgcn_make_buffer_rsrc(const_cast<float*>(B1n), 0, No * ldn1 * 4, 0x00020000);
  const __amdgpu_buffer_rsrc_t rB2 = __builtin_amdgcn_make_buffer_rsrc(const_cast<float*>(B2n), 0, K2 > 0 ? No * ldn2 * 4 : 0, 0x00020000);
  const uint32_t bstep1 = 128u * (uint32_t)ldn1, bstep2 = 128u * (uint32_t)ldn2;
  const unsigned char* const pk = reinterpret_cast<const unsigned char*>(B1n);

  if constexpr (AFFINE) {
    for (int i = tid; i < 2 * KA; i += THR) {
      const int k = i < KA ? i : i - KA;
      aff[i] = k < K1 ? (i < KA ? a.a_scale[k] : a.a_shift[k]) : 0.f;
    }
  }

  uint32_t fa = 127u;
  float sa = 1.f;
  if constexpr (NP <= 2) {
    uint32_t mb = a.a_amax1[0];
    if (K2 > 0 && a.a_amax2) mb = max(mb, a.a_amax2[0]);
    fa = __builtin_amdgcn_readfirstlane(h2_scale_field(mb));
    sa = h2_field_to_scale(fa);
  }
  const int ac = lane >> 4;
  const int nl = tid >> 3, kq = tid & 7;
  const int bx = nl & 15, bc = kq >> 1;
  const int wr_off = ((nl >> 4) * 3 * 64 + ((bx ^ (2 * bc)) + 16 * bc)) * 16 + (kq & 1) * 8;
  const int rd_off = (((lane & 15) ^ (2 * ac)) + 16 * ac) * 16;
  const bool last_round_on = (NT & 1) == 0 || w < 2;

  int g = 0;
  if constexpr (STAG) {
    int* const cnt = reinterpret_cast<int*>(smem);
    if (tid < 4) cnt[tid] = 0;
    __syncthreads();
    const int simd = (int)__builtin_amdgcn_s_getreg((1 << 11) | (4 << 6) | 4) & 3;
    int slot = 0;
    if (lane == 0) slot = atomicAdd(&cnt[simd], 1);
    g = __builtin_amdgcn_readfirstlane(slot) & 1;
    __syncthreads();
  }

  int tile = 0, m0 = 0, n0 = 0;
  uint32_t arow1[2], arow2[2];
#define QAGNN_NN2_SET_TILE(VB)                                                                                           \
  {                                                                                                                      \
    tile = a.xcd_remap ? xcd_remap((VB), ntiles) : (VB);                                                                 \
    m0 = (tile / ncb) * BM;                                                                                              \
    n0 = (tile % ncb) * BN;                                                                                              \
    _Pragma("unroll") for (int i = 0; i < 2; ++i) {                                                                      \
      const int row = m0 + w * 32 + i * 16 + (lane & 15);                                                                \
         \
      const int64_t grow = (a.a_rowidx && row < M) ? a.a_rowidx[row] : (int64_t)row;                                     \
      arow1[i] = (row < M && grow >= 0) ? (uint32_t)grow * (uint32_t)a.lda1 * 4u + (uint32_t)ac * 32u : OOB;             \
      arow2[i] = row < M ? (uint32_t)row * (uint32_t)a.lda2 * 4u + (uint32_t)ac * 32u : OOB;                             \
    }                                                                                                                    \
  }
  bool loaded = false;
  u32x4s ra[2][2];
  for (int vb = blockIdx.x; vb < ntiles; vb += gridDim.x) {
    if (!loaded) QAGNN_NN2_SET_TILE(vb)
    const int nvalid = min(BN, No - n0) - nl;

    f32x4s acc[2][NT];
#pragma unroll
    for (int i = 0; i < 2; ++i)
#pragma unroll
      for (int j = 0; j < NT; ++j) acc[i][j] = (f32x4s){0.f, 0.f, 0.f, 0.f};

    const uint32_t bbase1 = (uint32_t)(n0 + nl) * (uint32_t)ldn1 * 4u + (uint32_t)kq * 16u;
    const uint32_t bbase2 = (uint32_t)(n0 + nl) * (uint32_t)ldn2 * 4u + (uint32_t)kq * 16u;

// ... 334 lines not shown
#pragma unroll
            for (int r = 0; r < SLAB_ROWS; ++r) {
              const float dlt = r < rows ? (v[r] + bcv) - x0r[cc] : 0.f;
              s1[cc] += dlt;
              s2v[cc] = fmaf(dlt, dlt, s2v[cc]);
            }
          }
        }
      }
#pragma unroll
      for (int itx = 0; itx < ST_IT; ++itx) {
        const int idx = lane + itx * 64;
        if (idx >= TILE_F4) break;
        const int slr = idx / ROW_F4, c4 = idx % ROW_F4;
        const int row = m0 + (w * 2 + i) * 16 + slr, col = n0 + c4 * 4;
        if (row >= M || col >= No) continue;
        float4 v = ld4(St + slr * PS + c4 * 4);
        if (a.bias) v = add4(v, ld4(a.bias + col));
        if (a.rowtab) v = add4(v, ld4(a.rowtab + (int64_t)a.rowidx[row] * a.ldt + col));
        float* dst = a.C + (int64_t)row * a.ldc + col;
        if (a.accumulate) v = add4(v, ld4(dst));
        if constexpr (QAGNN_NN2_ABL & 64) {
          if (v.x == 1.2345e-30f) st4(dst, v);
        } else {
          st4(dst, v);
        }
      }
    }
    if constexpr (STATS) {
#pragma unroll
      for (int cc = 0; cc < SC; ++cc) {
        const int c = lane + cc * 64;
        if (c < BN) { cstat[w][0][c] = s1[cc]; cstat[w][1][c] = s2v[cc]; }
      }
      __syncthreads();
      const int hw = w & 3, hf = w >> 2, col = hw * 64 + lane;
      if (col < BN && n0 + col < No && m0 + hf * 128 < M) {
        float x0c = x0r[0];
#pragma unroll
        for (int cc = 1; cc < SC; ++cc) x0c = (hw == cc) ? x0r[cc] : x0c;
        float* const pt = a.colstat_part + ((int64_t)(tile / ncb) * (WV / 4) + hf) * 3 * No + n0 + col;
        const int w0 = hf * 4;
        pt[0] = x0c;
        pt[No] = (cstat[w0][0][col] + cstat[w0 + 1][0][col]) + (cstat[w0 + 2][0][col] + cstat[w0 + 3][0][col]);
        pt[2 * No] = (cstat[w0][1][col] + cstat[w0 + 1][1][col]) + (cstat[w0 + 2][1][col] + cstat[w0 + 3][1][col]);
      }
    }
  }
}
#undef QAGNN_NN2_SIX
#undef QAGNN_NN2_SIX_T

template <int NT, bool AFFINE, bool STATS, int NP, bool PACKED, int WV>
static int launch_i(const NnRoute& r, const qagnn_gemm_nn_args& b, const float* B1n, int ldn1, const float* B2n, int ldn2, hipStream_t stream) {
  const size_t lds = nn2_lds_bytes<NT, STATS, WV, NP>(AFFINE ? 2 * ((b.K1 + 31) & ~31) * 4 : 0);
  constexpr int lds_max = nn2_lds_bytes<NT, STATS, WV, NP>(AFFINE ? 2 * 256 * 4 : 0);
  if (int rc = raise_lds_limit<k_gemm_nn2<NT, AFFINE, STATS, NP, PACKED, WV>>(lds_max, "k_gemm_nn2")) return rc;
  k_gemm_nn2<NT, AFFINE, STATS, NP, PACKED, WV><<<r.grid, WV * 64, lds, stream>>>(b, B1n, ldn1, B2n, ldn2, r.ntiles);
  QAGNN_LAUNCH_CHECK("k_gemm_nn2");
  return QAGNN_OK;
}

template <int NP>
__device__ __forceinline__ void pack_b_wave(const float* __restrict__ B1n, int ldn1, int K1, const float* __restrict__ B2n, int ldn2, int K2, int No,
                                            int NJ, int nkt, int it, int j, unsigned char* __restrict__ out) {
  const int lane = threadIdx.x & 63;
  if (j >= NJ) return;
  float sb = 1.f;
  if constexpr (NP <= 2) {
    const int nn = j * 16 + (lane & 15);
    float m = 0.f;
    if (nn < No) {
      for (int k = (lane >> 4) * 4; k < K1; k += 16) {
        const float4 v = ld4(B1n + (int64_t)nn * ldn1 + k);
        m = fmaxf(fmaxf(m, fmaxf(fabsf(v.x), fabsf(v.y))), fmaxf(fabsf(v.z), fabsf(v.w)));
      }
      for (int k = (lane >> 4) * 4; k < K2; k += 16) {
        const float4 v = ld4(B2n + (int64_t)nn * ldn2 + k);
        m = fmaxf(fmaxf(m, fmaxf(fabsf(v.x), fabsf(v.y))), fmaxf(fabsf(v.z), fabsf(v.w)));
      }
    }
    const uint32_t fb = h2_scale_field(__builtin_bit_cast(uint32_t, wave_max(m)));
    sb = h2_field_to_scale(fb);
    if (it == 0 && lane == 0) reinterpret_cast<uint32_t*>(out + ((int64_t)nkt * NJ + 13) * (NP * 1024))[j] = fb;
  }
  const int r1 = K2 > 0 ? (K1 & 31) : 0;
  const int mixi = r1 != 0 ? 1 : 0;
  const int n1 = mixi ? (K1 >> 5) : ((K1 + 31) >> 5);
  const int s2 = mixi ? 32 - r1 : 0;
  const int kk = (lane >> 4) * 8, n = j * 16 + (lane & 15);
  const float* src = nullptr;
  if (n < No) {
    if (mixi && it == 0) {
      if (kk < r1) src = B1n + (int64_t)n * ldn1 + (K1 - r1 + kk);
      else if (kk - r1 < K2) src = B2n + (int64_t)n * ldn2 + (kk - r1);
    } else {
      const int u = it - mixi;
      if (u < n1) {
        if (u * 32 + kk < K1) src = B1n + (int64_t)n * ldn1 + (u * 32 + kk);
      } else {
        const int k2 = s2 + (u - n1) * 32 + kk;
        if (k2 < K2) src = B2n + (int64_t)n * ldn2 + k2;
      }
    }
  }
  u32x4s r[2] = {{0u, 0u, 0u, 0u}, {0u, 0u, 0u, 0u}};
  if (src) {
    r[0] = *reinterpret_cast<const u32x4s*>(src);
    r[1] = *reinterpret_cast<const u32x4s*>(src + 4);
  }
  u32x4s f[NP];
  if constexpr (NP <= 2) split_frag2<false, NP>(r, f, nullptr, nullptr, 0.f, sb);
  else split_frag<false>(r, f, nullptr, nullptr, 0.f);
  unsigned char* dst = out + ((int64_t)it * NJ + j) * (NP * 1024) + (((lane & 15) ^ (2 * (lane >> 4))) + 16 * (lane >> 4)) * 16;
#pragma unroll
  for (int p = 0; p < NP; ++p) *reinterpret_cast<u32x4s*>(dst + p * 1024) = f[p];
}

template <int NP>
__global__ __launch_bounds__(256) void k_pack_b(const float* __restrict__ B1n, int ldn1, int K1, const float* __restrict__ B2n, int ldn2, int K2,
                                               int No, int NJ, int nkt, unsigned char* __restrict__ out) {
  pack_b_wave<NP>(B1n, ldn1, K1, B2n, ldn2, K2, No, NJ, nkt, blockIdx.y, blockIdx.x * 4 + (threadIdx.x >> 6), out);
}

constexpr int PACK_MAX = 60;
struct PackOne { const float* B1n; const float* B2n; long long out_off; int ldn1, K1, ldn2, K2, No, NJ, jb, blk0, np, nkt; };
struct PackArgs { int n; int nblk; PackOne d[PACK_MAX]; };
__global__ __launch_bounds__(256) void k_pack_b_multi(PackArgs a, unsigned char* __restrict__ out) {
  int i = 0;
  while (i + 1 < a.n && (int)blockIdx.x >= a.d[i + 1].blk0) ++i;
  const PackOne& d = a.d[i];
  const int lb = (int)blockIdx.x - d.blk0;
  const int it = lb / d.jb, j = (lb % d.jb) * 4 + (threadIdx.x >> 6);
  if (d.np == 2) pack_b_wave<2>(d.B1n, d.ldn1, d.K1, d.B2n, d.ldn2, d.K2, d.No, d.NJ, d.nkt, it, j, out + d.out_off);
  else if (d.np == 1) pack_b_wave<1>(d.B1n, d.ldn1, d.K1, d.B2n, d.ldn2, d.K2, d.No, d.NJ, d.nkt, it, j, out + d.out_off);
  else pack_b_wave<3>(d.B1n, d.ldn1, d.K1, d.B2n, d.ldn2, d.K2, d.No, d.NJ, d.nkt, it, j, out + d.out_off);
}

int walk_tiles(int K1, int K2) {
  const int r1 = K2 > 0 ? (K1 & 31) : 0;
  const int mixi = r1 != 0 ? 1 : 0;
  const int n1 = mixi ? (K1 >> 5) : ((K1 + 31) >> 5);
  const int s2 = mixi ? 32 - r1 : 0;
  const int n2 = K2 > s2 ? ((K2 - s2 + 31) >> 5) : 0;
  return mixi + n1 + n2;
}

}

int launch_nn2(const NnRoute& r, const qagnn_gemm_nn_args& a, const float* B1n, int ldn1, const float* B2n, int ldn2, hipStream_t stream) {
  qagnn_gemm_nn_args b = a;
  b.xcd_remap = 1;
  const int shape = r.b == NnB::IN_KERNEL ? 0 : r.wv == 8 ? 4 : r.np;
  return dispatch_int<13, 8, 7, 4, 2>(r.nt, [&](auto nt) {
    return dispatch_int<0, 1, 2, 3, 4>(shape, [&](auto sh) {
      constexpr int NT = nt.value, NP = (sh.value == 0 || sh.value == 4) ? 3 : sh.value, WV = sh.value == 4 ? 8 : 4;
      constexpr bool PACKED = sh.value != 0;
      if constexpr (WV == 8 && NT != 13 && NT != 8) {
        set_error("k_gemm_nn2: no staggered block with %d column tiles", NT);
        return QAGNN_EUNSUPPORTED;
      } else {
        if constexpr (NT != 8) {
          if (r.stats) return nn2::launch_i<NT, false, true, NP, PACKED, WV>(r, b, B1n, ldn1, B2n, ldn2, stream);
        }
        return dispatch_bool(r.affine, [&](auto aff) { return nn2::launch_i<NT, aff.value, false, NP, PACKED, WV>(r, b, B1n, ldn1, B2n, ldn2, stream); });
      }
    });
  });
}

int64_t nn2_pack_bytes(int No, int K1, int K2, int np) {
  const int64_t img = ((int64_t)nn2::walk_tiles(K1, K2) * cdiv(No, 16) + 13) * (np * 1024);
  return np <= 2 ? img + (((int64_t)cdiv(No, 16) + 13) * 4 + 15) / 16 * 16 : img;
}

int launch_pack_b(int np, const qagnn_gemm_nn_args& a, const float* B1n, int ldn1, const float* B2n, int ldn2, void* ws, hipStream_t stream) {
  const int NJ = cdiv(a.No, 16), nkt = nn2::walk_tiles(a.K1, a.K2);
  return dispatch_int<3, 2, 1>(np, [&](auto p) {
    nn2::k_pack_b<p.value><<<dim3(cdiv(NJ, 4), nkt), 256, 0, stream>>>(B1n, ldn1, a.K1, B2n, ldn2, a.K2, a.No, NJ, nkt, reinterpret_cast<unsigned char*>(ws));
    QAGNN_LAUNCH_CHECK("k_pack_b");
    return QAGNN_OK;
  });
}

}
#include <mutex>
#include <vector>
namespace qagnn {
struct PrepackEntry { long long tag; const float* B1n; const float* B2n; int ldn1, K1, ldn2, K2, No, np; const void* pk; };
static std::mutex g_prepack_mu;
static std::vector<PrepackEntry> g_prepack;

const void* nn2_prepack_lookup(const float* B1n, int ldn1, int K1, const float* B2n, int ldn2, int K2, int No, int np) {
  std::lock_guard<std::mutex> lk(g_prepack_mu);
  for (size_t i = g_prepack.size(); i-- > 0;) {
    const PrepackEntry& e = g_prepack[i];
    if (e.np == np && e.B1n == B1n && e.K1 == K1 && e.No == No && e.ldn1 == ldn1 && e.K2 == K2 && (K2 == 0 || (e.B2n == B2n && e.ldn2 == ldn2))) return e.pk;
  }
  return nullptr;
}

static bool prepack_takes(const qagnn_pack_desc& d) {
  if (!d.B1n || d.No <= 0 || d.K1 < 8 || d.K1 % 8 != 0 || d.K2 < 0 || d.K2 % 8 != 0 || d.ldn1 < d.K1 || d.ldn1 % 4 != 0 || !aligned16(d.B1n)) return false;
  if (d.K2 > 0 && (!d.B2n || d.ldn2 < d.K2 || d.ldn2 % 4 != 0 || !aligned16(d.B2n))) return false;
  if (d.K2 > 0 && (d.K1 & 31) != 0 && d.K2 < 32 - (d.K1 & 31)) return false;
  return true;
}

}

using namespace qagnn;

extern "C" int64_t qagnn_gemm_nn_prepack_bytes(const qagnn_pack_desc* d, int32_t n) {
  int64_t tot = 0;
  for (int i = 0; i < n; ++i)
    if (prepack_takes(d[i])) tot += nn2_pack_bytes(d[i].No, d[i].K1, d[i].K2, (d[i].pieces == 2 || d[i].pieces == 1) ? d[i].pieces : 3);
  return tot;
}
// ... 46 lines not shown
```

### qagnn_amd/csrc/gemm_split.hip

```cpp
#include <stdlib.h>

#include <type_traits>

#include "common.h"

namespace qagnn {


__device__ __forceinline__ float4 bload4(__amdgpu_buffer_rsrc_t rsrc, uint32_t voff, uint32_t soff = 0) {
  return __builtin_bit_cast(float4, __builtin_amdgcn_raw_buffer_load_b128(rsrc, (int)voff, (int)soff, 0));
}

constexpr int SBK = 32, SBM = 128, SWAVES = 4, SRT = 2, STHR = SWAVES * 64;

__device__ __forceinline__ void split3(float x, uint32_t& h1, uint32_t& h2, uint32_t& h3) {
  const uint32_t u = __builtin_bit_cast(uint32_t, x);
  h1 = u & 0xFFFF0000u;
  const float r1 = x - __builtin_bit_cast(float, h1);
  h2 = __builtin_bit_cast(uint32_t, r1) & 0xFFFF0000u;
  const float r2 = r1 - __builtin_bit_cast(float, h2);
  h3 = __builtin_bit_cast(uint32_t, r2);
}
__device__ __forceinline__ uint32_t pack_hi(uint32_t lo, uint32_t hi) { return __builtin_amdgcn_perm(hi, lo, 0x07060302u); }

// ... 275 lines not shown
        QAGNN_LAUNCH_CHECK("k_gemm_nn_split");
        return QAGNN_OK;
      });
    });
  });
}


constexpr int TKR = 32, TCP = 40, TTHR = 256;

template <int NP>
__device__ __forceinline__ void store_col8(uint16_t* __restrict__ dst, int img_elems, const float (&x)[8], float s) {
  if constexpr (NP == 2) {
    uint32_t ph[4], pl[4];
#pragma unroll
    for (int e = 0; e < 8; e += 2) split2(x[e], x[e + 1], s, ph[e >> 1], pl[e >> 1]);
    *reinterpret_cast<uint4*>(dst) = make_uint4(ph[0], ph[1], ph[2], ph[3]);
    *reinterpret_cast<uint4*>(dst + img_elems) = make_uint4(pl[0], pl[1], pl[2], pl[3]);
    return;
  }
  if constexpr (NP == 1) {
    uint32_t ph[4];
#pragma unroll
    for (int e = 0; e < 8; e += 2) split1(x[e], x[e + 1], s, ph[e >> 1]);
    *reinterpret_cast<uint4*>(dst) = make_uint4(ph[0], ph[1], ph[2], ph[3]);
    return;
  }
  uint32_t h1[8], h2[8], h3[8];
#pragma unroll
  for (int i = 0; i < 8; ++i) split3(x[i], h1[i], h2[i], h3[i]);
  *reinterpret_cast<uint4*>(dst) = make_uint4(pack_hi(h1[0], h1[1]), pack_hi(h1[2], h1[3]), pack_hi(h1[4], h1[5]), pack_hi(h1[6], h1[7]));
  *reinterpret_cast<uint4*>(dst + img_elems) = make_uint4(pack_hi(h2[0], h2[1]), pack_hi(h2[2], h2[3]), pack_hi(h2[4], h2[5]), pack_hi(h2[6], h2[7]));
  *reinterpret_cast<uint4*>(dst + 2 * img_elems) = make_uint4(pack_hi(h3[0], h3[1]), pack_hi(h3[2], h3[3]), pack_hi(h3[4], h3[5]), pack_hi(h3[6], h3[7]));
}

template <bool AFF, int NP>
__device__ __forceinline__ void store_task(uint16_t* __restrict__ img, int img_elems, int off, const float4 (&r)[8], float4 sc, float4 sh, float s) {
#pragma unroll
  for (int j = 0; j < 4; ++j) {
    float x[8];
#pragma unroll
    for (int i = 0; i < 8; ++i) {
      float v = j == 0 ? r[i].x : j == 1 ? r[i].y : j == 2 ? r[i].z : r[i].w;
      if (AFF) {
        const float s = j == 0 ? sc.x : j == 1 ? sc.y : j == 2 ? sc.z : sc.w, h = j == 0 ? sh.x : j == 1 ? sh.y : j == 2 ? sh.z : sh.w;
        v = fmaxf(fmaf(v, s, h), 0.f);
      }
      x[i] = v;
    }
    store_col8<NP>(img + off + j * TCP, img_elems, x, s);
  }
}

struct TnAmax { const uint32_t* a; const uint32_t* a2; const uint32_t* b; };
template <int KT, int NT, bool AFFINE, bool GATHER, int NP = 3>
__global__ __launch_bounds__(TTHR) __attribute__((amdgpu_waves_per_eu(2, 2))) void k_gemm_tn_split(
    const float* __restrict__ A, int lda, const float* __restrict__ B, int ldb, float* __restrict__ P, int R, int Ka, int No,
    const float* __restrict__ a_scale, const float* __restrict__ a_shift, int chunk_rows, const int64_t* __restrict__ a_rowidx,
    const float* __restrict__ A2, int lda2, int Ka2, TnAmax amax) {
  extern __shared__ __attribute__((aligned(16))) unsigned char smem_tn[];
  constexpr int AC = KT * 16, BC = NT * 16, A_EL = AC * TCP, B_EL = BC * TCP;
  constexpr int MT = KT / 4, REM = KT % 4, RS = (REM * NT + 3) / 4;
  constexpr int A_TW = (AC + 63) / 64, B_TW = (BC + 63) / 64;
  constexpr bool A_MAJOR = A_TW >= B_TW;
  constexpr int MAJ_TW = A_MAJOR ? A_TW : B_TW, MIN_TW = A_MAJOR ? B_TW : A_TW;
  constexpr int MAJ_C = A_MAJOR ? AC : BC, MIN_C = A_MAJOR ? BC : AC, MAJ_EL = A_MAJOR ? A_EL : B_EL, MIN_EL = A_MAJOR ? B_EL : A_EL;
  static_assert(MAJ_TW <= 4 && MIN_TW <= 4, "task-waves per operand");
  static_assert(NP == 3 || !GATHER, "the gathered table goes through the exact split");
  uint16_t* const As = reinterpret_cast<uint16_t*>(smem_tn);
  uint16_t* const Bs = As + NP * A_EL;
  uint16_t* const Maj = A_MAJOR ? As : Bs;
  uint16_t* const Min = A_MAJOR ? Bs : As;
  const int tid = threadIdx.x, lane = tid & 63, w = __builtin_amdgcn_readfirstlane(tid >> 6);
  const int ka_total = Ka + (A2 ? Ka2 : 0);
  int bx = blockIdx.x, by = blockIdx.y, chunk = blockIdx.z, row_shift = 0;
  if (chunk_rows < 0) {
    chunk_rows = -chunk_rows;
  } else {
    const int lin = bx + (int)gridDim.x * (by + (int)gridDim.y * chunk);
    const int v = xcd_remap(lin, (int)(gridDim.x * gridDim.y * gridDim.z));
    bx = v % (int)gridDim.x;
    by = (v / (int)gridDim.x) % (int)gridDim.y;
    chunk = v / (int)(gridDim.x * gridDim.y);
  }
  bool second = false;
  if (A2 != nullptr) {
    const int n1 = (Ka + AC - 1) / AC;
    if (by >= n1) { by -= n1; row_shift = Ka; A = A2; lda = lda2; Ka = Ka2; second = true; }
  }
  uint32_t fa = 127u, fb = 127u;
  float sa = 1.f, sb = 1.f;
  if constexpr (NP <= 2) {
    fa = __builtin_amdgcn_readfirstlane(h2_scale_field(second ? amax.a2[0] : amax.a[0]));
    fb = __builtin_amdgcn_readfirstlane(h2_scale_field(amax.b[0]));
    sa = h2_field_to_scale(fa);
    sb = h2_field_to_scale(fb);
  }
  const int n0 = bx * BC, m0 = by * AC;
  const int r_beg = chunk * chunk_rows, r_end = min(R, r_beg + chunk_rows);
  const int ntile = (r_end - r_beg + TKR - 1) / TKR;

  static_assert(!GATHER || A_MAJOR, "the gathered operand is handled as the wide one");
  const __amdgpu_buffer_rsrc_t rsA = __builtin_amdgcn_make_buffer_rsrc(const_cast<float*>(A), 0, GATHER ? 0 : R * lda * 4, 0x00020000);
  const __amdgpu_buffer_rsrc_t rsB = __builtin_amdgcn_make_buffer_rsrc(const_cast<float*>(B), 0, R * ldb * 4, 0x00020000);
  const __amdgpu_buffer_rsrc_t rsMaj = A_MAJOR ? rsA : rsB, rsMin = A_MAJOR ? rsB : rsA;
  const int maj0 = A_MAJOR ? m0 : n0, min0 = A_MAJOR ? n0 : m0, majDim = A_MAJOR ? Ka : No, minDim = A_MAJOR ? No : Ka;
  const uint32_t ldMaj4 = (uint32_t)(A_MAJOR ? lda : ldb) * 4u, ldMin4 = (uint32_t)(A_MAJOR ? ldb : lda) * 4u;
  constexpr uint32_t OOB = 0x80000000u;

  const int g = lane & 3;
  const int c4j = w * 16 + (lane >> 2);
  const bool maj_act = w < MAJ_TW && c4j * 4 < MAJ_C;
  const bool maj_in = maj_act && maj0 + c4j * 4 < majDim;
  uint32_t maj_voff = maj_in ? ((uint32_t)(r_beg + g * 8) * ldMaj4 + (uint32_t)(maj0 + c4j * 4) * 4u) : OOB;
  const int maj_off = c4j * 4 * TCP + ((g ^ ((c4j ^ (c4j >> 1)) & 1)) << 3);
  float4 scj = make_float4(1.f, 1.f, 1.f, 1.f), shj = make_float4(0.f, 0.f, 0.f, 0.f);
  if (AFFINE && A_MAJOR) {
    const int cc = min(maj0 + c4j * 4, Ka - 4);
    scj = ld4(a_scale + cc);
    shj = ld4(a_shift + cc);
  }

  f32x4s acc[MT > 0 ? MT : 1][NT], accr[RS > 0 ? RS : 1];
#pragma unroll
  for (int i = 0; i < MT; ++i)
#pragma unroll
    for (int j = 0; j < NT; ++j) acc[i][j] = (f32x4s){0.f, 0.f, 0.f, 0.f};
#pragma unroll
  for (int q = 0; q < RS; ++q) accr[q] = (f32x4s){0.f, 0.f, 0.f, 0.f};

  float4 rj[8], rn[8];
  int gi[GATHER ? 8 : 1];
  const float* const Acol = A + min(maj0 + c4j * 4, Ka - 4);
  auto gidx = [&](int t) {
    if constexpr (GATHER) {
      const int r0 = r_beg + t * TKR + g * 8;
#pragma unroll
      for (int i = 0; i < 8; ++i) {
        const int64_t v = a_rowidx[min(r0 + i, R - 1)];
        gi[i] = (maj_in && r0 + i < R && v >= 0) ? (int)v : -1;
      }
    }
  };
  auto gload = [&](int t) {
    if constexpr (GATHER) {
#pragma unroll
      for (int i = 0; i < 8; ++i) {
// ... 112 lines not shown
#pragma unroll
  for (int j = 0; j < 4; ++j) {
    float x[8];
#pragma unroll
    for (int i = 0; i < 8; ++i) {
      float v = j == 0 ? r[i].x : j == 1 ? r[i].y : j == 2 ? r[i].z : r[i].w;
      if (AFF) {
        const float s_ = j == 0 ? sc.x : j == 1 ? sc.y : j == 2 ? sc.z : sc.w, h = j == 0 ? sh.x : j == 1 ? sh.y : j == 2 ? sh.z : sh.w;
        v = fmaxf(fmaf(v, s_, h), lo);
      }
      x[i] = v;
    }
    store_col8<NP>(img + off + j * TCP, img_elems, x, s);
  }
}

template <int KT, int NT, bool AFFINE, int NP = 3>
__global__ __launch_bounds__(WTHR) __attribute__((amdgpu_waves_per_eu(2, 2))) void k_gemm_tn_ws(
    const float* __restrict__ A, int lda, const float* __restrict__ B, int ldb, float* __restrict__ P, int R, int Ka, int No,
    const float* __restrict__ a_scale, const float* __restrict__ a_shift, int chunk_rows, const float* __restrict__ A2, int lda2, int Ka2,
    TnAmax amax) {
  extern __shared__ __attribute__((aligned(16))) unsigned char smem_tw[];
  constexpr int AC = KT * 16, BC = NT * 16, A_EL = AC * TCP, B_EL = BC * TCP;
  constexpr int IMG_EL = NP * (A_EL + B_EL), IMG_B = IMG_EL * 2;
  constexpr bool MAJ_A = KT >= NT;
  constexpr int MAJT = MAJ_A ? KT : NT, MINT = MAJ_A ? NT : KT;
  constexpr int MT = MAJT / 4, REM = MAJT % 4, RS = (REM * MINT + 3) / 4;
  constexpr int MAJ_PIECE = (MAJ_A ? A_EL : B_EL) * 2, MIN_PIECE = (MAJ_A ? B_EL : A_EL) * 2;
  constexpr int STRIP_B = 16 * TCP * 2;
  constexpr int NC4 = (AC + BC) / 4, NTW = (NC4 + 15) / 16;
  static_assert(MT >= 1 && NTW >= 4 && NTW <= 8, "shapes: (13, 7) and (7, 13)");
  const int tid = threadIdx.x, lane = tid & 63, w = __builtin_amdgcn_readfirstlane(tid >> 6);

  const int ka_total = Ka + (A2 ? Ka2 : 0);
  int bx = blockIdx.x, by = blockIdx.y, chunk = blockIdx.z, row_shift = 0;
  if (chunk_rows < 0) {
    chunk_rows = -chunk_rows;
  } else {
    const int lin = bx + (int)gridDim.x * (by + (int)gridDim.y * chunk);
    const int v = xcd_remap(lin, (int)(gridDim.x * gridDim.y * gridDim.z));
    bx = v % (int)gridDim.x;
    by = (v / (int)gridDim.x) % (int)gridDim.y;
    chunk = v / (int)(gridDim.x * gridDim.y);
  }
  bool second = false;
  if (A2 != nullptr) {
    const int n1 = (Ka + AC - 1) / AC;
    if (by >= n1) { by -= n1; row_shift = Ka; A = A2; lda = lda2; Ka = Ka2; second = true; }
  }
  uint32_t fa = 127u, fb = 127u;
  float sa = 1.f, sb = 1.f;
  if constexpr (NP <= 2) {
    fa = __builtin_amdgcn_readfirstlane(h2_scale_field(second ? amax.a2[0] : amax.a[0]));
    fb = __builtin_amdgcn_readfirstlane(h2_scale_field(amax.b[0]));
    sa = h2_field_to_scale(fa);
    sb = h2_field_to_scale(fb);
  }
  const int n0 = bx * BC, m0 = by * AC;
  const int r_beg = chunk * chunk_rows, r_end = min(R, r_beg + chunk_rows);
  const int ntile = (r_end - r_beg + TKR - 1) / TKR;

  int* const ctl = reinterpret_cast<int*>(smem_tw + 2 * IMG_B);
  if (tid < 8) ctl[tid] = 0;
  __syncthreads();
  int role, idx;
  {
    const int simd = (int)__builtin_amdgcn_s_getreg((1 << 11) | (4 << 6) | 4) & 3;
    int v = 0;
    if (lane == 0) v = atomicAdd(&ctl[simd], 1);
    role = __builtin_amdgcn_readfirstlane(v) & 1;
    if (lane == 0) v = atomicAdd(&ctl[4 + role], 1);
    idx = __builtin_amdgcn_readfirstlane(v);
    __syncthreads();
    if (ctl[4] != 4 || ctl[5] != 4) { role = w >> 2; idx = w & 3; }
  }
#define QAGNN_TNW_BAR                                                  \
  {                                                                    \
    __builtin_amdgcn_sched_barrier(0);                                 \
    asm volatile("s_waitcnt lgkmcnt(0)\n\ts_barrier" ::: "memory");    \
    __builtin_amdgcn_sched_barrier(0);                                 \
  }
  __syncthreads();

  const int ntile4 = (ntile + 3) & ~3;
  if (role == 1) {
    auto produce = [&](auto IDXC) {
      constexpr int IDX = decltype(IDXC)::value;
      const int g = lane & 3;
      const __amdgpu_buffer_rsrc_t rsA = __builtin_amdgcn_make_buffer_rsrc(const_cast<float*>(A), 0, R * lda * 4, 0x00020000);
      const __amdgpu_buffer_rsrc_t rsB = __builtin_amdgcn_make_buffer_rsrc(const_cast<float*>(B), 0, R * ldb * 4, 0x00020000);
      constexpr uint32_t OOB = 0x80000000u;
      const uint32_t ldA4 = (uint32_t)lda * 4u, ldB4 = (uint32_t)ldb * 4u;
      constexpr int TW[2] = {IDX, 4};
      constexpr bool HAS_A[2] = {TW[0] * 16 < AC / 4, TW[1] * 16 < AC / 4};
      constexpr bool HAS_B[2] = {TW[0] * 16 + 15 >= AC / 4, TW[1] * 16 + 15 >= AC / 4};
      uint32_t voA[2], voB[2];
      int off[2], iel[2];
      float4 sc[2], sh[2];
      float lo[2], ssc[2];
#pragma unroll
      for (int k = 0; k < 2; ++k) {
        const int c4u = TW[k] * 16 + (lane >> 2);
        const bool act = c4u < NC4 && (k == 0 || NTW > 4);
        const bool isA = c4u < AC / 4;
        const int c4 = isA ? c4u : c4u - AC / 4;
        voA[k] = act && isA && m0 + c4 * 4 < Ka ? (uint32_t)(r_beg + g * 8) * ldA4 + (uint32_t)(m0 + c4 * 4) * 4u : OOB;
        voB[k] = act && !isA && n0 + c4 * 4 < No ? (uint32_t)(r_beg + g * 8) * ldB4 + (uint32_t)(n0 + c4 * 4) * 4u : OOB;
// ... 155 lines not shown
#pragma unroll
      for (int s_ = 0; s_ < MT; ++s_) {
        f32x4s c = acc[s_][n];
        if constexpr (MAJ_A) { QAGNN_TNW_SIX(c, mf[s_], bfn) } else { QAGNN_TNW_SIX(c, bfn, mf[s_]) }
        acc[s_][n] = c;
      }
      __builtin_amdgcn_sched_barrier(0);
    }
#pragma unroll
    for (int s_ = 0; s_ < RS; ++s_) {
      if (ci + 4 * s_ < REM * MINT) {
        u32x4s ar[NP], br[NP];
        QAGNN_TNW_FRAG(ar, rem_maj[s_] + cur, 0, MAJ_PIECE)
        QAGNN_TNW_FRAG(br, rem_min[s_] + cur, 0, MIN_PIECE)
        QAGNN_TNW_WAIT(ar, 0);
        QAGNN_TNW_TOUCH(br)
        f32x4s c = accr[s_];
        if constexpr (MAJ_A) { QAGNN_TNW_SIX(c, ar, br) } else { QAGNN_TNW_SIX(c, br, ar) }
        accr[s_] = c;
      }
    }
    __builtin_amdgcn_s_setprio(0);
    QAGNN_TNW_BAR
  }
#undef QAGNN_TNW_FRAG
#undef QAGNN_TNW_WAIT
#undef QAGNN_TNW_TOUCH
#undef QAGNN_TNW_SIX
#undef QAGNN_TNW_BAR

  float* const Pc = P + (int64_t)chunk * ka_total * No;
  const float inv = NP <= 2 ? h2_inv_scale(fa, fb) : 1.f;
  auto put = [&](int maj_strip, int min_tile, const f32x4s& c) {
    const int rstrip = MAJ_A ? maj_strip : min_tile, ctile = MAJ_A ? min_tile : maj_strip;
#pragma unroll
    for (int r = 0; r < 4; ++r) {
      const int row = m0 + rstrip * 16 + (lane >> 4) * 4 + r, col = n0 + ctile * 16 + (lane & 15);
      if (row < Ka && col < No) Pc[(int64_t)(row + row_shift) * No + col] = NP <= 2 ? c[r] * inv : c[r];
    }
  };
#pragma unroll
  for (int s_ = 0; s_ < MT; ++s_)
#pragma unroll
    for (int n = 0; n < MINT; ++n) put(ci + 4 * s_, n, acc[s_][n]);
#pragma unroll
  for (int s_ = 0; s_ < RS; ++s_) {
    const int q = ci + 4 * s_;
    if (q < REM * MINT) put(4 * MT + q / MINT, q % MINT, accr[s_]);
  }
}

#define QAGNN_TN_ARGS p.A1, p.lda1, p.B, p.ldb, p.ws, p.R, p.Ka1, p.No, p.a_scale, p.a_shift, r.chunk_rows
static TnAmax tn_amax(const TnRoute& r, const TnProduct& p) {
  return r.np == 3 ? TnAmax{nullptr, nullptr, nullptr} : TnAmax{p.amax[0], p.two ? p.amax[1] : nullptr, p.amax[2]};
}
template <int KT, int NT, bool AFFINE, int NP = 3>
static int launch_tn_ws_i(const TnRoute& r, const TnProduct& p, hipStream_t stream) {
  constexpr int lds = 2 * NP * (KT * 16 + NT * 16) * TCP * (int)sizeof(uint16_t) + 64;
  if (int rc = raise_lds_limit<k_gemm_tn_ws<KT, NT, AFFINE, NP>>(lds, "k_gemm_tn_ws")) return rc;
  k_gemm_tn_ws<KT, NT, AFFINE, NP><<<r.grid, WTHR, lds, stream>>>(QAGNN_TN_ARGS, p.A2, p.lda2, p.Ka2, tn_amax(r, p));
  QAGNN_LAUNCH_CHECK("k_gemm_tn_ws");
  return QAGNN_OK;
}
template <int KT, int NT, bool AFFINE, bool GATHER = false, int NP = 3>
static int launch_tn_split_i(const TnRoute& r, const TnProduct& p, hipStream_t stream) {
  constexpr int lds = NP * (KT * 16 + NT * 16) * TCP * (int)sizeof(uint16_t);
  if (int rc = raise_lds_limit<k_gemm_tn_split<KT, NT, AFFINE, GATHER, NP>>(lds, "k_gemm_tn_split")) return rc;
  k_gemm_tn_split<KT, NT, AFFINE, GATHER, NP><<<r.grid, TTHR, lds, stream>>>(QAGNN_TN_ARGS, p.a_rowidx, p.A2, p.lda2, p.Ka2, tn_amax(r, p));
  QAGNN_LAUNCH_CHECK("k_gemm_tn_split");
  return QAGNN_OK;
}
#undef QAGNN_TN_ARGS

int launch_tn_ws(const TnRoute& r, const TnProduct& p, hipStream_t stream) {
  return dispatch_int<3, 2, 1>(r.np, [&](auto np) { return launch_tn_ws_i<7, 13, false, np.value>(r, p, stream); });
}
int launch_tn_split(const TnRoute& r, const TnProduct& p, hipStream_t stream) {
  if (r.gather) return launch_tn_split_i<13, 7, false, true>(r, p, stream);
  return dispatch_bool(r.kt == 7, [&](auto wide_b) {
    return dispatch_bool(r.affine, [&](auto aff) {
      return dispatch_int<3, 2, 1>(r.np, [&](auto np) {
        constexpr int KT = wide_b.value ? 7 : 13;
        return launch_tn_split_i<KT, 20 - KT, aff.value, false, np.value>(r, p, stream);
      });
    });
  });
}

}
```

### qagnn_amd/csrc/graph_prep.hip

```cpp
#include <stdarg.h>

#include <stdlib.h>

#include "common.h"

namespace qagnn {

static thread_local char g_err[512] = "";
void set_error(const char* fmt, ...) {
  va_list ap;
  va_start(ap, fmt);
  vsnprintf(g_err, sizeof(g_err), fmt, ap);
  va_end(ap);
}

__global__ void k_decode_count(const int64_t* __restrict__ edge_index, const int64_t* __restrict__ edge_type,
                               const int64_t* __restrict__ node_type, int N, int E, int R, int T, int* __restrict__ es,
                               int* __restrict__ et, int* __restrict__ ec, int* __restrict__ cnt_s, int* __restrict__ cnt_t,
                               int* __restrict__ err, int block_n) {
  const int e = blockIdx.x * blockDim.x + threadIdx.x;
  const int Ep = E + N;
  if (e >= Ep) return;
  int s, t, c;
  bool bad = false;
// ... 373 lines not shown
  int32_t *eid_t, *gc_cnt, *gcptr, *nch, *cnt_s, *cnt_t, *es, *et, *ec, *tmp_s, *tmp_t, *srcpos, *hist;
  int nblk, gb, NG, pairs;
};
static carved carve(qagnn_graph* g, int32_t* storage, int N, int E, int R, int T, int block_n) {
  carved cv;
  const int Ep = E + N, C = R * T * T + T;
  cls_groups(Ep, &cv.nblk, &cv.gb, &cv.NG);
  cv.pairs = cv.NG * C;
  const int maxch = Ep / QAGNN_CLS_CHUNK + cv.pairs + 1;
  int32_t* p = storage;
  auto take = [&](int64_t n) { int32_t* r = p; p += up4(n); return r; };
  g->N = N; g->E = E; g->Ep = Ep; g->R = R; g->T = T; g->C = C; g->max_chunks = maxch; g->block_n = block_n;
  g->n_groups = cv.NG;
  g->rowptr_s = take(N + 1); g->rowptr_t = take(N + 1);
  g->tgt_s = take(Ep); g->src_s = take(Ep); g->cls_s = take(Ep); g->eid_s = take(Ep);
  g->src_t = take(Ep); g->tgt_t = take(Ep); g->cls_t = take(Ep); g->pos_t = take(Ep);
  g->src_c = take(Ep); g->tgt_c = take(Ep); g->pos_c = take(Ep);
  cv.eid_t = take(Ep);
  cv.gc_cnt = take(cv.pairs + 1); cv.gcptr = take(cv.pairs + 1);
  g->chunkptr = take(cv.pairs + 1);
  cv.nch = take(cv.pairs + 1);
  g->cls_count = take(C);
  g->chunk_cls = take(maxch); g->chunk_beg = take(maxch); g->chunk_len = take(maxch);
  g->n_chunks = take(4); g->err = take(16);
  cv.cnt_s = take(N); cv.cnt_t = take(N);
  cv.es = take(Ep); cv.et = take(Ep); cv.ec = take(Ep);
  cv.tmp_s = take(Ep); cv.tmp_t = take(Ep); cv.srcpos = take(Ep);
  cv.hist = take((int64_t)cv.nblk * C);
  return cv;
}

static int class_pass(qagnn_graph* g, int32_t* hist, int32_t* gc_cnt, int32_t* gcptr, int32_t* nch, int nblk, int gb, int NG, int pairs,
                      hipStream_t stream) {
  const int TB = 256, C = g->C;
  const int* Ep = g->rowptr_s + g->N;
  k_cls_hist<<<nblk, 256, C * sizeof(int), stream>>>(g->cls_s, hist, g->cls_count, Ep, C);
  QAGNN_LAUNCH_CHECK("k_cls_hist");
  k_grp_count<<<cdiv(pairs, TB), TB, 0, stream>>>(hist, gc_cnt, nblk, C, gb, NG);
  QAGNN_LAUNCH_CHECK("k_grp_count");
  k_chunk_counts<<<cdiv(pairs, 1024), 1024, 0, stream>>>(gc_cnt, nch, pairs);
  QAGNN_LAUNCH_CHECK("k_chunk_counts");
  k_scan_pairs<<<2, 1024, 0, stream>>>(gc_cnt, gcptr, nch, g->chunkptr, pairs);
  QAGNN_LAUNCH_CHECK("k_scan_pairs");
  k_grp_base<<<cdiv(pairs, TB), TB, 0, stream>>>(hist, gcptr, nblk, C, gb, NG);
  QAGNN_LAUNCH_CHECK("k_grp_base");
  k_cls_scatter<<<nblk, 64, C * sizeof(int), stream>>>(g->cls_s, g->src_s, g->tgt_s, hist, g->src_c, g->tgt_c, g->pos_c, Ep, C);
  QAGNN_LAUNCH_CHECK("k_cls_scatter");
  k_chunk_fill<<<cdiv(pairs, 256), 256, 0, stream>>>(gcptr, g->chunkptr, g->chunk_cls, g->chunk_beg, g->chunk_len, g->n_chunks, C, pairs);
  QAGNN_LAUNCH_CHECK("k_chunk_fill");
  return QAGNN_OK;
}

extern "C" const char* qagnn_last_error(void) { return g_err; }
extern "C" int qagnn_abi_version(void) { return 22; }

extern "C" int64_t qagnn_graph_storage_elems(int32_t N, int32_t E, int32_t R, int32_t T) {
  const int64_t Ep = (int64_t)E + N, C = (int64_t)R * T * T + T;
  int nblk_i, gb, NG;
  cls_groups((int)Ep, &nblk_i, &gb, &NG);
  const int64_t pairs = (int64_t)NG * C;
  const int64_t maxch = Ep / QAGNN_CLS_CHUNK + pairs + 1;
  const int64_t nblk = nblk_i;
  int64_t tot = 0;
  tot += 2 * up4(N + 1);
  tot += 12 * up4(Ep);
  tot += 4 * up4(pairs + 1);
  tot += up4(C);
  tot += 3 * up4(maxch);
  tot += up4(4) + up4(16);
  tot += 2 * up4(N);
  tot += 6 * up4(Ep);
  tot += up4(nblk * C);
  return tot;
}

extern "C" int qagnn_graph_prep(qagnn_graph* g, int32_t* storage, const int64_t* edge_index, const int64_t* edge_type,
                                const int64_t* node_type, int32_t N, int32_t E, int32_t R, int32_t T, qagnn_stream_t stream_) {
  return qagnn_graph_prep_blocked(g, storage, edge_index, edge_type, node_type, N, E, R, T, 0, stream_);
}

extern "C" int qagnn_graph_prep_blocked(qagnn_graph* g, int32_t* storage, const int64_t* edge_index, const int64_t* edge_type,
                                        const int64_t* node_type, int32_t N, int32_t E, int32_t R, int32_t T, int32_t block_n,
                                        qagnn_stream_t stream_) {
  hipStream_t stream = (hipStream_t)stream_;
  QAGNN_REQUIRE(block_n >= 0 && (block_n == 0 || N % block_n == 0), QAGNN_EINVAL, "graph_prep: N=%d is not a multiple of block_n=%d", N, block_n);
  QAGNN_REQUIRE(g && storage && node_type, QAGNN_EINVAL, "graph_prep: null pointer");
  QAGNN_REQUIRE(N > 0 && E >= 0 && R > 0 && T > 0, QAGNN_EINVAL, "graph_prep: bad sizes N=%d E=%d R=%d T=%d", N, E, R, T);
  QAGNN_REQUIRE(E == 0 || (edge_index && edge_type), QAGNN_EINVAL, "graph_prep: null edge arrays with E=%d", E);
  QAGNN_REQUIRE(aligned16(storage), QAGNN_EINVAL, "graph_prep: storage must be 16-byte aligned");
  const int64_t Ep64 = (int64_t)E + N, C64 = (int64_t)R * T * T + T;
  QAGNN_REQUIRE(Ep64 < (1ll << 30), QAGNN_EUNSUPPORTED, "graph_prep: E+N=%lld too large", (long long)Ep64);
  QAGNN_REQUIRE(C64 <= 8192, QAGNN_EUNSUPPORTED, "graph_prep: %lld edge classes > 8192", (long long)C64);
  const int Ep = (int)Ep64;
  carved cv = carve(g, storage, N, E, R, T, block_n);
  int32_t *cnt_s = cv.cnt_s, *cnt_t = cv.cnt_t, *es = cv.es, *et = cv.et, *ec = cv.ec, *tmp_s = cv.tmp_s, *tmp_t = cv.tmp_t;
  int32_t *srcpos = cv.srcpos, *eid_t = cv.eid_t, *hist = cv.hist, *gc_cnt = cv.gc_cnt, *gcptr = cv.gcptr, *nch = cv.nch;
  const int nblk = cv.nblk, gb = cv.gb, NG = cv.NG, pairs = cv.pairs;

  hipError_t he = zero_range(g->cls_count, (size_t)((char*)es - (char*)g->cls_count), stream);
  if (he != hipSuccess) { set_error("graph_prep: k_zero16 failed: %s", hipGetErrorString(he)); return QAGNN_EHIP; }
  const int TB = 256;
  k_decode_count<<<cdiv(Ep, TB), TB, 0, stream>>>(edge_index, edge_type, node_type, N, E, R, T, es, et, ec, cnt_s, cnt_t,
                                                   g->err, block_n);
  QAGNN_LAUNCH_CHECK("k_decode_count");
  k_scan3<<<2, 1024, 0, stream>>>(cnt_s, g->rowptr_s, N, cnt_t, g->rowptr_t, N, nullptr, nullptr, 0);
  QAGNN_LAUNCH_CHECK("k_scan3");
  k_fill<<<cdiv(Ep, TB), TB, 0, stream>>>(es, et, g->rowptr_s, g->rowptr_t, cnt_s, cnt_t, tmp_s, tmp_t, Ep);
// ... 35 lines not shown
```

### qagnn_amd/csrc/hop.hip

```cpp
#include "common.h"

#include <mutex>

namespace qagnn {

static inline int64_t up4(int64_t x) { return (x + 3) & ~(int64_t)3; }
static inline int64_t max64(int64_t a, int64_t b) { return a > b ? a : b; }

struct Carver {
  float* p;
  float* end;
  float* take(int64_t n) {
    float* r = p;
    p += up4(n);
    return r;
  }
  bool ok() const { return p <= end; }
};

static int check_hop(const qagnn_hop_args* h, const char* who) {
  QAGNN_REQUIRE(h && h->g, QAGNN_EINVAL, "%s: null argument block / graph", who);
  QAGNN_REQUIRE(h->N == h->g->N && h->N > 0, QAGNN_EINVAL, "%s: N=%d does not match the graph (N=%d)", who, h->N, h->g->N);
  QAGNN_REQUIRE(h->HP > 0 && h->HP % 4 == 0 && h->DP == 4 * h->HP, QAGNN_EINVAL, "%s: DP=%d must be 4*HP (HP=%d)", who, h->DP, h->HP);
  QAGNN_REQUIRE(h->DP % 16 == 0 && h->SP >= 0 && h->SP % 16 == 0, QAGNN_EUNSUPPORTED,
                "%s: DP=%d and SP=%d must be multiples of 16 (GEMM k-tile)", who, h->DP, h->SP);
  QAGNN_REQUIRE(h->T >= 1 && h->T <= 4, QAGNN_EUNSUPPORTED, "%s: %d node types (the type-table gradient handles 1..4)", who, h->T);
  QAGNN_REQUIRE(h->X && h->ntype && h->Wx_t && h->Wx && h->TT && h->EkEm && h->W1t && h->W1 && h->b1 && h->gamma && h->beta &&
                    h->W2t && h->W2 && h->b2,
                QAGNN_EINVAL, "%s: null parameter pointer", who);
  QAGNN_REQUIRE(h->SP == 0 || (h->S && h->Ws_t && h->Ws), QAGNN_EINVAL, "%s: SP=%d but S / Ws_t / Ws missing", who, h->SP);
  QAGNN_REQUIRE(h->KMQ && h->a && h->alpha && h->aggr && h->h1 && h->out && h->stats, QAGNN_EINVAL, "%s: null saved-buffer pointer", who);
  QAGNN_REQUIRE(h->batch_stats || (h->run_mean_p && h->run_var_p), QAGNN_EINVAL, "%s: running statistics missing", who);
  QAGNN_REQUIRE(!h->apply_act || h->y, QAGNN_EINVAL, "%s: apply_act without an output buffer y", who);
  QAGNN_REQUIRE(h->ws, QAGNN_EINVAL, "%s: null workspace", who);
  return QAGNN_OK;
}

enum { AM_X = 0, AM_S = 1, AM_AGGR = 2, AM_H1 = 3, AM_Y = 4, AM_DOUT = 5, AM_DH1 = 6, AM_DKMQ = 7 };
struct HopAmax {
  bool on;
  uint32_t* x;
  uint32_t* s;
  uint32_t* y;
  uint32_t* own;
};
static bool hop_h2(const qagnn_hop_args* h) { return h->gemm_split >= 2 && h->amax != nullptr && h->batch_stats && nn_rows_packed(h->N); }
static int hop_pieces(const qagnn_hop_args* h) { return h->gemm_split == 3 ? 1 : 0; }
static HopAmax hop_amax_single(const qagnn_hop_args* h) {
  HopAmax m{hop_h2(h), nullptr, nullptr, nullptr, h->amax};
  if (m.on) {
    m.x = h->x_amax ? const_cast<uint32_t*>(h->x_amax) : h->amax + AM_X;
    m.s = h->s_amax ? const_cast<uint32_t*>(h->s_amax) : h->amax + AM_S;
    m.y = h->amax + AM_Y;
  }
  return m;
}
static HopAmax hop_amax_stack(const qagnn_hop_args* hops, int k, int l) {
  HopAmax m = hop_amax_single(&hops[l]);
  if (!m.on) return m;
  if (l > 0 && hop_h2(&hops[l - 1]) && hops[l].X == hops[l - 1].y && hops[l - 1].apply_act && !hops[l].x_amax) m.x = hops[l - 1].amax + AM_Y;
  if (l > 0 && hop_h2(&hops[0]) && hops[l].S == hops[0].S && hops[l].SP == hops[0].SP && !hops[l].s_amax)
    m.s = hops[0].s_amax ? const_cast<uint32_t*>(hops[0].s_amax) : hops[0].amax + AM_S;
  return m;
}

}

using namespace qagnn;

#define HOP_TRY(call)              \
  do {                             \
    int rc__ = (call);             \
    if (rc__ != QAGNN_OK) return rc__; \
  } while (0)

static int64_t hop_pack_elems(int DP) { return up4((qagnn_gemm_nn_pack_bytes(3 * DP, DP, DP) + 3) / 4); }

extern "C" int64_t qagnn_hop_fwd_workspace_elems(int32_t N, int32_t Ep, int32_t DP) {
  return up4((int64_t)Ep * 4) + up4(max64(qagnn_colreduce_workspace_elems(N, DP, 1), (int64_t)cdiv(N, 128) * 3 * DP)) + hop_pack_elems(DP) +
         up4(max64(N, gelu_amax_scratch_elems((int64_t)N * DP)));
}

static int hop_nn(const qagnn_hop_args* h, const qagnn_gemm_nn_args* a, const float* B1n, int ldn1, const float* B2n, int ldn2,
                  float* pkws, int64_t pk_elems, qagnn_stream_t stream) {
  return gemm_nn(NnProduct{a, h->gemm_split != 0, B1n, ldn1, B2n, ldn2, pkws, pk_elems * 4}, (hipStream_t)stream);
}
static int hop_tn(const qagnn_hop_args* h, const float* A1, int Ka1, const float* A2, int Ka2, const float* B, int No, float* C, const float* sc,
                  const float* sh, const uint32_t* am_a1, const uint32_t* am_a2, const uint32_t* am_b, float* tnws, qagnn_stream_t stream) {
  return gemm_tn(tn_product(A1, Ka1, Ka1, A2, Ka2, Ka2, B, No, C, No, h->N, No, sc, sh, tnws, am_a1, am_a2, am_b, h->gemm_split == 3 ? 1 : 2),
                 (hipStream_t)stream);
}

static int hop_fwd_one(const qagnn_hop_args* h, const HopAmax& am, bool x_ready, bool s_ready, qagnn_stream_t stream) {
  HOP_TRY(check_hop(h, "hop_fwd"));
  const int N = h->N, DP = h->DP, SP = h->SP, Ep = h->g->Ep;
  Carver w{h->ws, h->ws + h->ws_elems};
  float* score = w.take((int64_t)Ep * 4);
  float* crws = w.take(max64(qagnn_colreduce_workspace_elems(N, DP, 1), (int64_t)cdiv(N, 128) * 3 * DP));
  const int64_t pk_elems = hop_pack_elems(DP);
  float* pkws = w.take(pk_elems);
  float* ampart = w.take(max64(N, gelu_amax_scratch_elems((int64_t)N * DP)));
  QAGNN_REQUIRE(w.ok(), QAGNN_EINVAL, "hop_fwd: workspace of %lld floats is too small", (long long)h->ws_elems);
  float* mean = h->stats, *var = h->stats + DP, *invstd = h->stats + 2 * DP, *scale = h->stats + 3 * DP, *shift = h->stats + 4 * DP;

  if (am.on) {
    if (!x_ready) HOP_TRY(qagnn_absmax_f32(h->X, (int64_t)N * DP, am.x, stream));
    if (SP > 0 && !s_ready) HOP_TRY(qagnn_absmax_f32(h->S, (int64_t)N * SP, am.s, stream));
  }
  qagnn_gemm_nn_args ga = {};
  ga.A1 = h->X; ga.lda1 = DP; ga.K1 = DP; ga.B1 = h->Wx_t; ga.ldb1 = 3 * DP;
  if (SP > 0) { ga.A2 = h->S; ga.lda2 = SP; ga.K2 = SP; ga.B2 = h->Ws_t; ga.ldb2 = 3 * DP; }
  ga.C = h->KMQ; ga.ldc = 3 * DP; ga.M = N; ga.No = 3 * DP;
  ga.rowtab = h->TT; ga.ldt = 3 * DP; ga.rowidx = h->ntype;
  if (am.on) { ga.a_amax1 = am.x; ga.a_amax2 = SP > 0 ? am.s : nullptr; ga.pieces = hop_pieces(h); }
  HOP_TRY(hop_nn(h, &ga, h->Wx, DP, SP > 0 ? h->Ws : nullptr, SP, pkws, pk_elems, stream));
  HOP_TRY(launch_edge_attn_fwd(h->g, h->KMQ, 3 * DP, h->EkEm, 2 * DP, h->HP, h->qscale, score, h->a, h->alpha, h->aggr, DP,
                               am.on ? ampart : nullptr, (hipStream_t)stream));
  if (am.on) HOP_TRY(launch_amax_reduce(ampart, N, am.own + AM_AGGR, (hipStream_t)stream));
  qagnn_gemm_nn_args g1 = {};
  g1.A1 = h->aggr; g1.lda1 = DP; g1.K1 = DP; g1.B1 = h->W1t; g1.ldb1 = DP; g1.C = h->h1; g1.ldc = DP; g1.M = N; g1.No = DP; g1.bias = h->b1;
  const bool fused_stats = h->batch_stats && h->gemm_split && DP > 192 && DP <= 208;
  if (fused_stats) g1.colstat_part = crws;
  if (am.on) { g1.a_amax1 = am.own + AM_AGGR; g1.pieces = hop_pieces(h); }
  HOP_TRY(hop_nn(h, &g1, h->W1, DP, nullptr, 0, pkws, pk_elems, stream));
  const double Rd = (double)N;
  const float unbias = (float)(Rd / (Rd - 1.0 > 1.0 ? Rd - 1.0 : 1.0));
  const bool h1_bound = am.on && fused_stats;
  if (fused_stats) {
    QAGNN_REQUIRE(!h->run_mean || (h->run_var && h->d > 0 && h->d % 4 == 0 && h->d <= DP), QAGNN_EINVAL, "hop_fwd: running-stat arguments");
    HOP_TRY(launch_bn_stats_finalize(crws, cdiv(N, 128), N, DP, h->gamma, h->beta, h->eps, h->stats, h->run_mean, h->run_var, h->num_batches_tracked,
                                     h->d, h->momentum, unbias, h->ones_col, h1_bound ? am.own + AM_H1 : nullptr, (hipStream_t)stream));
  } else {
    const float* mean_u = mean;
    const float* var_u = var;
    if (h->batch_stats) {
      const float inv_rows = (float)(1.0 / (double)N);
      HOP_TRY(qagnn_colreduce_f32(0, h->h1, DP, nullptr, DP, N, DP, nullptr, 1, nullptr, nullptr, nullptr, nullptr, nullptr, inv_rows, mean, crws,
                                  stream));
      HOP_TRY(qagnn_colreduce_f32(1, h->h1, DP, nullptr, DP, N, DP, nullptr, 1, mean, nullptr, nullptr, nullptr, nullptr, inv_rows, var, crws,
                                  stream));
    } else {
      mean_u = h->run_mean_p;
      var_u = h->run_var_p;
    }
    HOP_TRY(qagnn_bn_finalize_f32(mean_u, var_u, h->gamma, h->beta, h->eps, invstd, scale, shift, DP, h->run_mean, h->run_var,
                                  h->num_batches_tracked, h->dense_pos, h->d, h->momentum, unbias, h->ones_col, stream));
  }
  qagnn_gemm_nn_args g2 = {};
  g2.A1 = h->h1; g2.lda1 = DP; g2.K1 = DP; g2.B1 = h->W2t; g2.ldb1 = DP; g2.C = h->out; g2.ldc = DP; g2.M = N; g2.No = DP; g2.bias = h->b2;
  g2.a_scale = scale; g2.a_shift = shift;
  if (h1_bound) { g2.a_amax1 = am.own + AM_H1; g2.pieces = hop_pieces(h); }
  HOP_TRY(hop_nn(h, &g2, h->W2, DP, nullptr, 0, pkws, pk_elems, stream));
  if (h->apply_act) {
    QAGNN_REQUIRE(h->p_drop >= 0.f && h->p_drop < 1.f, QAGNN_EINVAL, "hop_fwd: p=%f", h->p_drop);
    HOP_TRY(launch_gelu_dropout(h->out, nullptr, h->y, (int64_t)N * DP, h->p_drop, h->seed, am.on ? am.y : nullptr, ampart, (hipStream_t)stream));
  }
  return QAGNN_OK;
}

extern "C" int qagnn_hop_fwd_f32(const qagnn_hop_args* h, qagnn_stream_t stream) {
  QAGNN_REQUIRE(h, QAGNN_EINVAL, "hop_fwd: null argument block");
  const HopAmax am = hop_amax_single(h);
  if (am.on) HOP_TRY(qagnn_zero_words(h->amax, QAGNN_HOP_AMAX_WORDS, stream));
  return hop_fwd_one(h, am, h->x_amax != nullptr, h->s_amax != nullptr, stream);
}

extern "C" int64_t qagnn_hop_bwd_workspace_elems(int32_t N, int32_t Ep, int32_t DP, int32_t SP, int32_t cls_part_rows) {
  int64_t tn = max64(qagnn_gemm_tn_workspace_elems(N, DP, DP), qagnn_gemm_tn_workspace_elems(N, DP, 3 * DP));
  if (SP > 0) tn = max64(tn, qagnn_gemm_tn_workspace_elems(N, DP + SP, 3 * DP));
  return 2 * (2 * up4((int64_t)N * DP) + up4((int64_t)N * 3 * DP)) + up4((int64_t)N * DP) + up4((int64_t)Ep * 4) + up4((int64_t)N * 4) +
         up4((int64_t)cls_part_rows * 2 * DP) + up4(tn) + up4(qagnn_colreduce_workspace_elems(N, 3 * DP, 4)) + hop_pack_elems(DP) +
         up4(max64((int64_t)3 * N, gelu_amax_scratch_elems((int64_t)N * DP)));
}

namespace qagnn {

constexpr int HOP_MAX_DEV = 16, HOP_EV_POOL = 64;
static hipEvent_t g_hop_ev[HOP_MAX_DEV][HOP_EV_POOL];
static bool g_hop_ev_made[HOP_MAX_DEV];
static std::mutex g_hop_ev_mu;

struct SideSync {
  hipStream_t main, side;
  hipEvent_t* ev;
  int next;
  hipEvent_t take() { return ev[next++ % HOP_EV_POOL]; }
};

static int side_sync_init(SideSync* s, hipStream_t main, hipStream_t side) {
  s->main = main;
  s->side = (side && side != main) ? side : nullptr;
  s->ev = nullptr;
  s->next = 0;
  if (!s->side) return QAGNN_OK;
  int dev = 0;
  hipError_t he = hipGetDevice(&dev);
  QAGNN_REQUIRE(he == hipSuccess && dev >= 0 && dev < HOP_MAX_DEV, QAGNN_EHIP, "hop_bwd: device %d outside the event table", dev);
  std::lock_guard<std::mutex> lk(g_hop_ev_mu);
  if (!g_hop_ev_made[dev]) {
    for (int i = 0; i < HOP_EV_POOL; ++i) {
      he = hipEventCreateWithFlags(&g_hop_ev[dev][i], hipEventDisableTiming);
      QAGNN_REQUIRE(he == hipSuccess, QAGNN_EHIP, "hop_bwd: hipEventCreate failed: %s", hipGetErrorString(he));
    }
    g_hop_ev_made[dev] = true;
  }
  s->ev = g_hop_ev[dev];
  return QAGNN_OK;
}
static int stream_after(hipStream_t to, hipStream_t from, hipEvent_t ev) {
  hipError_t he = hipEventRecord(ev, from);
  if (he == hipSuccess) he = hipStreamWaitEvent(to, ev, 0);
  QAGNN_REQUIRE(he == hipSuccess, QAGNN_EHIP, "hop_bwd: stream fork / join failed: %s", hipGetErrorString(he));
  return QAGNN_OK;
}

static int hop_bwd_one(const qagnn_hop_args* h, const HopAmax& am, SideSync* ss, int set, hipEvent_t* done) {
  HOP_TRY(check_hop(h, "hop_bwd"));
  QAGNN_REQUIRE(h->dy && h->dWx_t && h->dTT && h->dEkEm && h->dW1t && h->db1 && h->dbn && h->dW2t && h->db2, QAGNN_EINVAL,
                "hop_bwd: null gradient pointer");
  QAGNN_REQUIRE(h->SP == 0 || h->dWs_t, QAGNN_EINVAL, "hop_bwd: dWs_t missing");
  const int N = h->N, DP = h->DP, SP = h->SP, Ep = h->g->Ep;
  Carver w{h->ws, h->ws + h->ws_elems};
  float *bufA2[2], *bufC2[2], *dKMQ2[2];
  for (int i = 0; i < 2; ++i) {
    bufA2[i] = w.take((int64_t)N * DP);
    bufC2[i] = w.take((int64_t)N * DP);
    dKMQ2[i] = w.take((int64_t)N * 3 * DP);
  }
  float* bufA = bufA2[set];
  float* bufC = bufC2[set];
  float* dKMQ = dKMQ2[set];
  float* bufB = w.take((int64_t)N * DP);
  float* gab = w.take((int64_t)Ep * 4);
  float* rs = w.take((int64_t)N * 4);
  float* cls_part = w.take(((int64_t)h->g->max_chunks + (int64_t)QAGNN_CLS_SLICES * h->g->C) * 2 * DP);
  int64_t tn = max64(qagnn_gemm_tn_workspace_elems(N, DP, DP), qagnn_gemm_tn_workspace_elems(N, DP, 3 * DP));
  if (SP > 0) tn = max64(tn, qagnn_gemm_tn_workspace_elems(N, DP + SP, 3 * DP));
  float* tnws = w.take(tn);
  float* crws = w.take(qagnn_colreduce_workspace_elems(N, 3 * DP, 4));
  const int64_t pk_elems = hop_pack_elems(DP);
  float* pkws = w.take(pk_elems);
  float* ampart = w.take(max64((int64_t)3 * N, gelu_amax_scratch_elems((int64_t)N * DP)));
  QAGNN_REQUIRE(w.ok(), QAGNN_EINVAL, "hop_bwd: workspace of %lld floats is too small", (long long)h->ws_elems);
  const float* mean = h->batch_stats ? h->stats : h->run_mean_p;
  const float* invstd = h->stats + 2 * DP, *scale = h->stats + 3 * DP, *shift = h->stats + 4 * DP;
  const qagnn_stream_t stream = (qagnn_stream_t)ss->main;
  const qagnn_stream_t wstream = (qagnn_stream_t)(ss->side ? ss->side : ss->main);

  const float* dout = h->dy;
  const bool h2 = am.on && DP > 192 && DP <= 208;
  uint32_t* const w_dout = h2 ? am.own + AM_DOUT : nullptr, *const w_dh1 = h2 ? am.own + AM_DH1 : nullptr, *const w_dkmq = h2 ? am.own + AM_DKMQ : nullptr;
  const uint32_t* const w_h1 = h2 ? am.own + AM_H1 : nullptr, *const w_aggr = h2 ? am.own + AM_AGGR : nullptr;
  if (h->apply_act) {
    HOP_TRY(launch_gelu_dropout(h->out, h->dy, bufA, (int64_t)N * DP, h->p_drop, h->seed, w_dout, ampart, (hipStream_t)stream));
    dout = bufA;
  } else if (h2) {
    HOP_TRY(qagnn_absmax_f32(dout, (int64_t)N * DP, w_dout, stream));
  }
  if (h->ones_col < 0)
    HOP_TRY(qagnn_colreduce_f32(0, dout, DP, nullptr, DP, N, DP, nullptr, 1, nullptr, nullptr, nullptr, nullptr, nullptr, 1.0f, h->db2, crws, stream));
  if (ss->side) HOP_TRY(stream_after(ss->side, ss->main, ss->take()));
  HOP_TRY(hop_tn(h, h->h1, DP, nullptr, 0, dout, DP, h->dW2t, scale, shift, w_h1, nullptr, w_dout, tnws, wstream));
  if (h->ones_col >= 0 && h->db2 != h->dW2t + (int64_t)h->ones_col * DP) {
    hipError_t he = hipMemcpyAsync(h->db2, h->dW2t + (int64_t)h->ones_col * DP, (size_t)DP * sizeof(float), hipMemcpyDeviceToDevice, (hipStream_t)wstream);
    if (he != hipSuccess) { set_error("hop_bwd: db2 copy failed: %s", hipGetErrorString(he)); return QAGNN_EHIP; }
  }
  qagnn_gemm_nn_args gr = {};
  gr.A1 = dout; gr.lda1 = DP; gr.K1 = DP; gr.B1 = h->W2; gr.ldb1 = DP; gr.C = bufB; gr.ldc = DP; gr.M = N; gr.No = DP;
  gr.a_amax1 = w_dout; gr.pieces = hop_pieces(h);
  HOP_TRY(hop_nn(h, &gr, h->W2t, DP, nullptr, 0, pkws, pk_elems, stream));
  HOP_TRY(qagnn_colreduce_f32(2, bufB, DP, h->h1, DP, N, DP, nullptr, 1, mean, invstd, scale, shift, nullptr, 1.0f, h->dbn, crws, stream));
  HOP_TRY(launch_bn_relu_bwd_colsum(bufB, h->h1, bufC, DP, N, DP, mean, invstd, scale, shift, h->gamma, h->dbn, h->dbn + DP,
                                    h->batch_stats ? (float)(1.0 / (double)N) : 0.f, nullptr, h->db1, crws, w_dh1, (hipStream_t)stream));
  if (ss->side) HOP_TRY(stream_after(ss->side, ss->main, ss->take()));
  HOP_TRY(hop_tn(h, h->aggr, DP, nullptr, 0, bufC, DP, h->dW1t, nullptr, nullptr, w_aggr, nullptr, w_dh1, tnws, wstream));
  qagnn_gemm_nn_args gg = {};
  gg.A1 = bufC; gg.lda1 = DP; gg.K1 = DP; gg.B1 = h->W1; gg.ldb1 = DP; gg.C = bufB; gg.ldc = DP; gg.M = N; gg.No = DP;
  gg.a_amax1 = w_dh1; gg.pieces = hop_pieces(h);
  HOP_TRY(hop_nn(h, &gg, h->W1t, DP, nullptr, 0, pkws, pk_elems, stream));
  HOP_TRY(launch_edge_attn_bwd(h->g, h->KMQ, 3 * DP, h->EkEm, 2 * DP, h->HP, h->qscale, h->a, h->alpha, bufB, DP, dKMQ, h->dEkEm, gab, rs, cls_part,
                               h2 ? ampart : nullptr, w_dkmq, (hipStream_t)stream));
  if (ss->side) HOP_TRY(stream_after(ss->side, ss->main, ss->take()));
  if (SP > 0 && h->dWs_t == h->dWx_t + (int64_t)DP * 3 * DP) {
    HOP_TRY(hop_tn(h, h->X, DP, h->S, SP, dKMQ, 3 * DP, h->dWx_t, nullptr, nullptr, am.x, am.s, w_dkmq, tnws, wstream));
  } else {
    HOP_TRY(hop_tn(h, h->X, DP, nullptr, 0, dKMQ, 3 * DP, h->dWx_t, nullptr, nullptr, am.x, nullptr, w_dkmq, tnws, wstream));
    if (SP > 0) HOP_TRY(hop_tn(h, h->S, SP, nullptr, 0, dKMQ, 3 * DP, h->dWs_t, nullptr, nullptr, am.s, nullptr, w_dkmq, tnws, wstream));
  }
  if (SP > 0 && h->tab_col >= 0) {
    QAGNN_REQUIRE(h->tab_col + h->T <= SP, QAGNN_EINVAL, "hop_bwd: tab_col=%d + T=%d exceeds SP=%d", h->tab_col, h->T, SP);
    if (h->dTT != h->dWs_t + (int64_t)h->tab_col * 3 * DP) {
      hipError_t he = hipMemcpyAsync(h->dTT, h->dWs_t + (int64_t)h->tab_col * 3 * DP, (size_t)h->T * 3 * DP * sizeof(float), hipMemcpyDeviceToDevice,
                                     (hipStream_t)wstream);
      if (he != hipSuccess) { set_error("hop_bwd: dTT copy failed: %s", hipGetErrorString(he)); return QAGNN_EHIP; }
    }
  } else {
    HOP_TRY(qagnn_colreduce_f32(0, dKMQ, 3 * DP, nullptr, 3 * DP, N, 3 * DP, h->ntype, h->T, nullptr, nullptr, nullptr, nullptr, nullptr, 1.0f, h->dTT,
                                crws, stream));
  }
  if (ss->side) {
    *done = ss->take();
    hipError_t he = hipEventRecord(*done, ss->side);
    QAGNN_REQUIRE(he == hipSuccess, QAGNN_EHIP, "hop_bwd: hipEventRecord failed: %s", hipGetErrorString(he));
  }
  if (h->dX) {
    qagnn_gemm_nn_args gx = {};
    gx.A1 = dKMQ; gx.lda1 = 3 * DP; gx.K1 = 3 * DP; gx.B1 = h->Wx; gx.ldb1 = DP; gx.C = h->dX; gx.ldc = DP; gx.M = N; gx.No = DP;
    gx.accumulate = h->accumulate_dX;
    gx.a_amax1 = w_dkmq; gx.pieces = hop_pieces(h);
    HOP_TRY(hop_nn(h, &gx, h->Wx_t, 3 * DP, nullptr, 0, pkws, pk_elems, stream));
  }
  if (SP > 0 && h->dS) {
    qagnn_gemm_nn_args gs = {};
    gs.A1 = dKMQ; gs.lda1 = 3 * DP; gs.K1 = 3 * DP; gs.B1 = h->Ws; gs.ldb1 = SP; gs.C = h->dS; gs.ldc = SP; gs.M = N; gs.No = SP;
    gs.accumulate = h->accumulate_dS;
    gs.a_amax1 = w_dkmq; gs.pieces = hop_pieces(h);
    HOP_TRY(hop_nn(h, &gs, h->Ws_t, 3 * DP, nullptr, 0, pkws, pk_elems, stream));
  }
  return QAGNN_OK;
}

static int stack_bwd_impl(const qagnn_hop_args* hops, int k, hipStream_t main) {
  SideSync ss;
// ... 48 lines not shown
```

Before: 44630 QA-subgraphs/s.

## Replace amax partial-reduce passes with slotted atomic-max arrays folded in consumer GEMMs

Producers of absmax values (edge aggregate, gelu-dropout fwd/bwd) now write into 64 strided slot words using relaxed atomic max, guarded by a peek of the current value. Consumer GEMMs fold the slots directly, so the separate amax reduce kernel launches are dropped. The gather_multi kernels also gain a vectorized float4 path. This removes several small kernels and partial-array round trips per hop, at the cost of atomic contention on the slots and a larger per-hop amax block.

New measurement: 44530 QA-subgraphs/s. Within noise of the previous version (-0.2%).

```diff
diff --git a/include/qagnn_hip.h b/include/qagnn_hip.h
--- a/include/qagnn_hip.h
+++ b/include/qagnn_hip.h
@@ -223,7 +223,7 @@
   const uint32_t* x_amax;
   const uint32_t* s_amax;
 } qagnn_hop_args;
-#define QAGNN_HOP_AMAX_WORDS 16
+#define QAGNN_HOP_AMAX_WORDS (16 + 3 * 2048)
 int64_t qagnn_hop_fwd_workspace_elems(int32_t N, int32_t Ep, int32_t DP);
 int64_t qagnn_hop_bwd_workspace_elems(int32_t N, int32_t Ep, int32_t DP, int32_t SP,
                                       int32_t cls_part_rows );
diff --git a/qagnn_amd/_lib.py b/qagnn_amd/_lib.py
--- a/qagnn_amd/_lib.py
+++ b/qagnn_amd/_lib.py
@@ -21,7 +21,7 @@
            'qagnn_timing_enable', 'qagnn_timing_read', 'qagnn_gemm_tn_h1_f32', 'qagnn_gelu_dropout_bwd_amax_f32', 'qagnn_packed_min_rows']
 
 CLS_SLICES = 4
-ABI_VERSION = 22
+ABI_VERSION = 23
 
 _i32, _i64, _f32, _u64, _vp = C.c_int32, C.c_int64, C.c_float, C.c_uint64, C.c_void_p
 
@@ -67,7 +67,7 @@
                 [('ws_elems', _i64), ('gemm_split', _i32), ('ones_col', _i32), ('tab_col', _i32), ('side_stream', _vp), ('amax', _vp), ('x_amax', _vp), ('s_amax', _vp)])
 
 
-HOP_AMAX_WORDS = 16
+HOP_AMAX_WORDS = 16 + 3 * 2048
 
 
 def load_library(path=LIB_PATH):
diff --git a/qagnn_amd/csrc/common.h b/qagnn_amd/csrc/common.h
--- a/qagnn_amd/csrc/common.h
+++ b/qagnn_amd/csrc/common.h
@@ -16,6 +16,7 @@
   bool split;
   const float* B1n; int ldn1; const float* B2n; int ldn2;
   void* ws; int64_t ws_bytes;
+  const uint32_t* a1_slots;
 };
 enum class NnFamily { FP32, SPLIT, NN2 };
 enum class NnB { IN_KERNEL, PACK, IMAGE };
@@ -46,7 +47,8 @@
 int gemm_nn(const NnProduct& p, hipStream_t stream);
 int launch_nn(const NnRoute& r, const qagnn_gemm_nn_args& a, hipStream_t stream);
 int launch_nn_split(const NnRoute& r, const qagnn_gemm_nn_args& a, const float* B1n, int ldn1, const float* B2n, int ldn2, hipStream_t stream);
-int launch_nn2(const NnRoute& r, const qagnn_gemm_nn_args& a, const float* B1n, int ldn1, const float* B2n, int ldn2, hipStream_t stream);
+int launch_nn2(const NnRoute& r, const qagnn_gemm_nn_args& a, const float* B1n, int ldn1, const float* B2n, int ldn2, const uint32_t* a1_slots,
+               hipStream_t stream);
 int launch_pack_b(int np, const qagnn_gemm_nn_args& a, const float* B1n, int ldn1, const float* B2n, int ldn2, void* ws, hipStream_t stream);
 namespace nn2 { int walk_tiles(int K1, int K2); }
 int64_t nn2_pack_bytes(int No, int K1, int K2, int np);
@@ -60,6 +62,7 @@
   const float* a_scale; const float* a_shift; const int64_t* a_rowidx; int accumulate;
   float* bsum; const int64_t* b_rowidx; int groups;
   const uint32_t* amax[3]; int np;
+  const uint32_t* b_slots;
   float* ws;
 };
 inline TnProduct tn_product(const float* A1, int lda1, int Ka1, const float* A2, int lda2, int Ka2, const float* B, int ldb, float* C, int ldc, int R,
@@ -93,6 +96,7 @@
 int launch_gelu_dropout(const float* X, const float* dY, float* out, int64_t n, float p, uint64_t seed, uint32_t* amax, float* amax_part,
                         hipStream_t stream);
 int64_t gelu_amax_scratch_elems(int64_t n);
+int launch_gelu_dropout_slots(const float* X, const float* dY, float* out, int64_t n, float p, uint64_t seed, uint32_t* slots, hipStream_t stream);
 int launch_bn_relu_bwd_colsum(const float* dR, const float* Hh, float* dH, int ld, int R, int Cc, const float* mean, const float* invstd,
                               const float* scale, const float* shift, const float* gamma, const float* sum_dy, const float* sum_dy_hhat,
                               float inv_rows, const float* roww, float* colsum, float* workspace, uint32_t* amax, hipStream_t stream);
@@ -101,7 +105,8 @@
                              hipStream_t stream);
 
 int launch_edge_attn_fwd(const qagnn_graph* g, const float* KMQ, int32_t ldk, const float* EkEm, int32_t lde, int32_t HP, float qscale,
-                         float* score, float* a, float* alpha, float* aggr, int32_t lda, float* amax_part , hipStream_t stream);
+                         float* score, float* a, float* alpha, float* aggr, int32_t lda, uint32_t* amax_slots ,
+                         hipStream_t stream);
 int launch_edge_attn_bwd(const qagnn_graph* g, const float* KMQ, int32_t ldk, const float* EkEm, int32_t lde, int32_t HP, float qscale,
                          const float* a, const float* alpha, const float* G, int32_t ldg, float* dKMQ, float* dEkEm, float* ga, float* rs,
                          float* cls_part, float* amax_part , uint32_t* amax_slot, hipStream_t stream);
@@ -304,5 +309,24 @@
 }
 __device__ __forceinline__ float absmax4(float4 v) { return fmaxf(fmaxf(fabsf(v.x), fabsf(v.y)), fmaxf(fabsf(v.z), fabsf(v.w))); }
 
-
-}
+constexpr int AMAX_SLOTS = 64, AMAX_SLOT_STRIDE = 32, AMAX_SLOT_WORDS = AMAX_SLOTS * AMAX_SLOT_STRIDE;
+__device__ __forceinline__ uint32_t* amax_slot(uint32_t* __restrict__ slots, uint32_t i) { return slots + (i % AMAX_SLOTS) * AMAX_SLOT_STRIDE; }
+__device__ __forceinline__ uint32_t amax_slot_peek(const uint32_t* slot) {
+  return __hip_atomic_load(slot, __ATOMIC_RELAXED, __HIP_MEMORY_SCOPE_AGENT);
+}
+__device__ __forceinline__ void amax_slot_merge(float m, uint32_t seen, uint32_t* slot) {
+  const uint32_t b = __builtin_bit_cast(uint32_t, m);
+  if (m > 0.f && b > seen) __hip_atomic_fetch_max(slot, b, __ATOMIC_RELAXED, __HIP_MEMORY_SCOPE_AGENT);
+}
+__device__ __forceinline__ uint32_t amax_slots_fold(const uint32_t* __restrict__ slots) {
+  uint32_t v = slots[(threadIdx.x & 63) * AMAX_SLOT_STRIDE];
+#pragma unroll
+  for (int o = 32; o > 0; o >>= 1) {
+    const uint32_t u = (uint32_t)__shfl_xor((int)v, o, 64);
+    v = u > v ? u : v;
+  }
+  return v;
+}
+
+
+}
diff --git a/qagnn_amd/csrc/edge_attn.hip b/qagnn_amd/csrc/edge_attn.hip
--- a/qagnn_amd/csrc/edge_attn.hip
+++ b/qagnn_amd/csrc/edge_attn.hip
@@ -176,15 +176,22 @@
   if ((threadIdx.x & 63) == 63) part[node] = m;
 }
 
+__device__ __forceinline__ void node_amax_slot(float m, uint32_t seen, uint32_t* __restrict__ slot) {
+  m = wave_amax_lane63(m);
+  if ((threadIdx.x & 63) == 63) amax_slot_merge(m, seen, slot);
+}
+
 __global__ __launch_bounds__(256) void k_edge_aggregate(const int* __restrict__ rowptr_t, const int* __restrict__ src_t,
                                                         const int* __restrict__ cls_t, const int* __restrict__ pos_t,
                                                         const float* __restrict__ KMQ, int ldk, const float* __restrict__ EkEm,
                                                         int lde, int HP, const float* __restrict__ alpha,
                                                         float* __restrict__ aggr, int lda, int N, int C, const int* __restrict__ xcd_base,
-                                                        float* __restrict__ amax_part) {
+                                                        uint32_t* __restrict__ amax_slots) {
   __shared__ float4 slab[4][SLAB_ROWS];
   const int t = wave_node(xcd_base);
   if (t >= N) return;
+  uint32_t* const slot = amax_slots ? amax_slot(amax_slots, (uint32_t)t) : nullptr;
+  const uint32_t seen = slot ? amax_slot_peek(slot) : 0u;
   const Lane L = lane_info(HP);
   const int DP = 4 * HP;
   const uint32_t pk = (uint32_t)ldk * 4u, pe = (uint32_t)lde * 4u, vm = L.voff + (uint32_t)DP * 4u;
@@ -197,7 +204,7 @@
     const float al = alpha[(int64_t)pv * 4 + L.g];
     const float4 o1 = fma4(al, add4(m1, em1), zero4());
     if (L.act) st4(aggr + (int64_t)t * lda + L.off, o1);
-    if (amax_part) node_amax(L.act ? absmax4(o1) : 0.f, amax_part, t);
+    if (slot) node_amax_slot(L.act ? absmax4(o1) : 0.f, seen, slot);
     return;
   }
   slab_init(slab[L.w], L.lane);
@@ -220,7 +227,7 @@
     }
   }
   if (L.act) st4(aggr + (int64_t)t * lda + L.off, acc);
-  if (amax_part) node_amax(L.act ? absmax4(acc) : 0.f, amax_part, t);
+  if (slot) node_amax_slot(L.act ? absmax4(acc) : 0.f, seen, slot);
 }
 
 __global__ __launch_bounds__(256) void k_edge_bwd_src1(const int* __restrict__ rowptr_s, const int* __restrict__ tgt_s,
@@ -492,7 +499,7 @@
 
 namespace qagnn {
 int launch_edge_attn_fwd(const qagnn_graph* g, const float* KMQ, int32_t ldk, const float* EkEm, int32_t lde, int32_t HP, float qscale,
-                         float* score, float* a, float* alpha, float* aggr, int32_t lda, float* amax_part, hipStream_t stream) {
+                         float* score, float* a, float* alpha, float* aggr, int32_t lda, uint32_t* amax_slots, hipStream_t stream) {
   TimedScope timed(2, stream);
   int rc = check_common(g, KMQ, ldk, EkEm, lde, HP, "edge_attn_fwd");
   if (rc != QAGNN_OK) return rc;
@@ -501,7 +508,7 @@
   const int nb = 8 * edge_xcd_cap(g->N);
   k_edge_scores<<<nb, 256, 0, stream>>>(g->rowptr_s, g->tgt_s, g->cls_s, KMQ, ldk, EkEm, lde, HP, qscale, score, a, alpha, g->N, g->C, g->err + 4);
   QAGNN_LAUNCH_CHECK("k_edge_scores");
-  k_edge_aggregate<<<nb, 256, 0, stream>>>(g->rowptr_t, g->src_t, g->cls_t, g->pos_t, KMQ, ldk, EkEm, lde, HP, alpha, aggr, lda, g->N, g->C, g->err + 4, amax_part);
+  k_edge_aggregate<<<nb, 256, 0, stream>>>(g->rowptr_t, g->src_t, g->cls_t, g->pos_t, KMQ, ldk, EkEm, lde, HP, alpha, aggr, lda, g->N, g->C, g->err + 4, amax_slots);
   QAGNN_LAUNCH_CHECK("k_edge_aggregate");
   return QAGNN_OK;
 }
diff --git a/qagnn_amd/csrc/elementwise.hip b/qagnn_amd/csrc/elementwise.hip
--- a/qagnn_amd/csrc/elementwise.hip
+++ b/qagnn_amd/csrc/elementwise.hip
@@ -250,25 +250,37 @@
 __device__ __forceinline__ float4 gelu_dropout_one(const float* __restrict__ X, const float* __restrict__ dY, int64_t i, float p, uint64_t seed, float inv) {
   return gelu_dropout_val<BWD>(ld4(X + i * 4), BWD ? ld4(dY + i * 4) : make_float4(1.f, 1.f, 1.f, 1.f), i, p, seed, inv);
 }
-template <bool BWD, bool AMAX = false>
+template <bool BWD, int AMAX = 0>
 __global__ __launch_bounds__(256) void k_gelu_dropout(const float* __restrict__ X, const float* __restrict__ dY, float* __restrict__ out, int64_t n4,
                                                       float p, uint64_t seed, const unsigned long long* __restrict__ epoch,
                                                       float* __restrict__ amax_part = nullptr) {
+  uint32_t* slot = nullptr;
+  uint32_t seen = 0u;
+  if constexpr (AMAX == 2) {
+    if (threadIdx.x == 0) {
+      slot = amax_slot(reinterpret_cast<uint32_t*>(amax_part), blockIdx.x);
+      seen = amax_slot_peek(slot);
+    }
+  }
   if (p > 0.f) seed = epoch_seed(seed, epoch);
   const float inv = p > 0.f ? 1.f / (1.f - p) : 1.f;
   const int64_t i = (int64_t)blockIdx.x * blockDim.x + threadIdx.x;
-  if (!AMAX && i >= n4) return;
+  if (AMAX == 0 && i >= n4) return;
   float4 o = make_float4(0.f, 0.f, 0.f, 0.f);
   if (i < n4) {
     o = gelu_dropout_one<BWD>(X, dY, i, p, seed, inv);
     st4(out + i * 4, o);
   }
-  if constexpr (AMAX) {
+  if constexpr (AMAX != 0) {
     __shared__ float red[4];
     const float m = wave_amax_lane63(absmax4(o));
     if ((threadIdx.x & 63) == 63) red[threadIdx.x >> 6] = m;
     __syncthreads();
-    if (threadIdx.x == 0) amax_part[blockIdx.x] = fmaxf(fmaxf(red[0], red[1]), fmaxf(red[2], red[3]));
+    if (threadIdx.x == 0) {
+      const float bm = fmaxf(fmaxf(red[0], red[1]), fmaxf(red[2], red[3]));
+      if constexpr (AMAX == 2) amax_slot_merge(bm, seen, slot);
+      else amax_part[blockIdx.x] = bm;
+    }
   }
 }
 
@@ -493,11 +505,63 @@
   out[s] = acc;
 }
 
+__device__ __forceinline__ float gather1(const float* const* ps, int k, int o) {
+  const float* p = k >= 0 ? ps[k] : nullptr;
+  return p != nullptr ? p[o] : 0.f;
+}
+__device__ __forceinline__ float4 gather4(const float* const* ps, int4 k, int4 o) {
+  if (k.x >= 0 && k.y == k.x && k.z == k.x && k.w == k.x && o.y == o.x + 1 && o.z == o.x + 2 && o.w == o.x + 3) {
+    const float* p = ps[k.x];
+    if (p != nullptr && (reinterpret_cast<uintptr_t>(p + o.x) & 15u) == 0) return ld4(p + o.x);
+  }
+  return make_float4(gather1(ps, k.x, o.x), gather1(ps, k.y, o.y), gather1(ps, k.z, o.z), gather1(ps, k.w, o.w));
+}
+__global__ __launch_bounds__(256) void k_gather_multi4(qagnn_gather_tabs t, const int* __restrict__ tid, const int* __restrict__ off,
+                                                      float* __restrict__ out, int total) {
+  __shared__ const float* ps[QAGNN_GATHER_MAX];
+  for (int i = threadIdx.x; i < t.n; i += blockDim.x) ps[i] = t.p[i];
+  __syncthreads();
+  const int64_t i = ((int64_t)blockIdx.x * blockDim.x + threadIdx.x) * 4;
+  if (i >= total) return;
+  if (i + 4 <= total) {
+    st4(out + i, gather4(ps, *reinterpret_cast<const int4*>(tid + i), *reinterpret_cast<const int4*>(off + i)));
+  } else {
+    for (int64_t e = i; e < total; ++e) out[e] = gather1(ps, tid[e], off[e]);
+  }
+}
+__global__ __launch_bounds__(256) void k_gather_multi_sum4(qagnn_gather_tabs t, const int* __restrict__ tid, const int* __restrict__ off, int K, int S,
+                                                          float* __restrict__ out) {
+  __shared__ const float* ps[QAGNN_GATHER_MAX];
+  for (int i = threadIdx.x; i < t.n; i += blockDim.x) ps[i] = t.p[i];
+  __syncthreads();
+  const int64_t s = ((int64_t)blockIdx.x * blockDim.x + threadIdx.x) * 4;
+  if (s >= S) return;
+  if (s + 4 <= S) {
+    float4 acc = make_float4(0.f, 0.f, 0.f, 0.f);
+    for (int k = 0; k < K; ++k) {
+      const int64_t at = (int64_t)k * S + s;
+      const float4 v = gather4(ps, *reinterpret_cast<const int4*>(tid + at), *reinterpret_cast<const int4*>(off + at));
+      acc = k == 0 ? v : add4(acc, v);
+    }
+    st4(out + s, acc);
+  } else {
+    for (int64_t e = s; e < S; ++e) {
+      float acc = 0.f;
+      for (int k = 0; k < K; ++k) {
+        const float v = gather1(ps, tid[(int64_t)k * S + e], off[(int64_t)k * S + e]);
+        acc = k == 0 ? v : acc + v;
+      }
+      out[e] = acc;
+    }
+  }
+}
+
 extern "C" int qagnn_gather_multi_f32(const qagnn_gather_tabs* t, const int32_t* tid, const int32_t* off, float* out, int32_t total,
                                       qagnn_stream_t stream_) {
   QAGNN_REQUIRE(t && t->n > 0 && t->n <= QAGNN_GATHER_MAX && tid && off && out && total > 0, QAGNN_EINVAL, "gather_multi: bad arguments");
   for (int i = 0; i < t->n; ++i) QAGNN_REQUIRE(t->p[i] != nullptr, QAGNN_EINVAL, "gather_multi: null source %d", i);
-  k_gather_multi<<<cdiv(total, 256), 256, 0, (hipStream_t)stream_>>>(*t, tid, off, out, total);
+  if (aligned16(tid) && aligned16(off) && aligned16(out)) k_gather_multi4<<<cdiv(cdiv(total, 4), 256), 256, 0, (hipStream_t)stream_>>>(*t, tid, off, out, total);
+  else k_gather_multi<<<cdiv(total, 256), 256, 0, (hipStream_t)stream_>>>(*t, tid, off, out, total);
   QAGNN_LAUNCH_CHECK("k_gather_multi");
   return QAGNN_OK;
 }
@@ -505,7 +569,9 @@
 extern "C" int qagnn_gather_multi_sum_f32(const qagnn_gather_tabs* t, const int32_t* tid, const int32_t* off, int32_t K, int32_t S, float* out,
                                           qagnn_stream_t stream_) {
   QAGNN_REQUIRE(t && t->n > 0 && t->n <= QAGNN_GATHER_MAX && tid && off && out && K > 0 && S > 0, QAGNN_EINVAL, "gather_multi_sum: bad arguments");
-  k_gather_multi_sum<<<cdiv(S, 256), 256, 0, (hipStream_t)stream_>>>(*t, tid, off, K, S, out);
+  if (aligned16(tid) && aligned16(off) && aligned16(out) && (K == 1 || S % 4 == 0))
+    k_gather_multi_sum4<<<cdiv(cdiv(S, 4), 256), 256, 0, (hipStream_t)stream_>>>(*t, tid, off, K, S, out);
+  else k_gather_multi_sum<<<cdiv(S, 256), 256, 0, (hipStream_t)stream_>>>(*t, tid, off, K, S, out);
   QAGNN_LAUNCH_CHECK("k_gather_multi_sum");
   return QAGNN_OK;
 }
@@ -517,14 +583,22 @@
   const int grid = cdiv(n / 4, 256);
   if (amax && !amax_part) { set_error("gelu_dropout: the maximum needs its scratch"); return QAGNN_EINVAL; }
   if (dY) {
-    if (amax) k_gelu_dropout<true, true><<<grid, 256, 0, stream>>>(X, dY, out, n / 4, p, seed, seed_epoch_ptr(), amax_part);
+    if (amax) k_gelu_dropout<true, 1><<<grid, 256, 0, stream>>>(X, dY, out, n / 4, p, seed, seed_epoch_ptr(), amax_part);
     else k_gelu_dropout<true><<<grid, 256, 0, stream>>>(X, dY, out, n / 4, p, seed, seed_epoch_ptr());
   } else {
-    if (amax) k_gelu_dropout<false, true><<<grid, 256, 0, stream>>>(X, nullptr, out, n / 4, p, seed, seed_epoch_ptr(), amax_part);
+    if (amax) k_gelu_dropout<false, 1><<<grid, 256, 0, stream>>>(X, nullptr, out, n / 4, p, seed, seed_epoch_ptr(), amax_part);
     else k_gelu_dropout<false><<<grid, 256, 0, stream>>>(X, nullptr, out, n / 4, p, seed, seed_epoch_ptr());
   }
   QAGNN_LAUNCH_CHECK("k_gelu_dropout");
   return amax ? launch_amax_reduce(amax_part, grid, amax, stream) : QAGNN_OK;
+}
+int launch_gelu_dropout_slots(const float* X, const float* dY, float* out, int64_t n, float p, uint64_t seed, uint32_t* slots, hipStream_t stream) {
+  const int grid = cdiv(n / 4, 256);
+  float* const sl = reinterpret_cast<float*>(slots);
+  if (dY) k_gelu_dropout<true, 2><<<grid, 256, 0, stream>>>(X, dY, out, n / 4, p, seed, seed_epoch_ptr(), sl);
+  else k_gelu_dropout<false, 2><<<grid, 256, 0, stream>>>(X, nullptr, out, n / 4, p, seed, seed_epoch_ptr(), sl);
+  QAGNN_LAUNCH_CHECK("k_gelu_dropout");
+  return QAGNN_OK;
 }
 }
 
diff --git a/qagnn_amd/csrc/gemm_dispatch.hip b/qagnn_amd/csrc/gemm_dispatch.hip
--- a/qagnn_amd/csrc/gemm_dispatch.hip
+++ b/qagnn_amd/csrc/gemm_dispatch.hip
@@ -78,6 +78,8 @@
   nn_grid(r, a.M, a.No, r.wv * 32, r.wv == 8 ? 1 : 2);
   return r;
 }
+
+static bool nn_reads_amax(const NnRoute& r) { return r.family == NnFamily::NN2 && r.np <= 2; }
 
 static int nn_validate(const NnProduct& p) {
   QAGNN_REQUIRE(p.a, QAGNN_EINVAL, "gemm_nn: null pointer");
@@ -112,14 +114,20 @@
   if (int rc = nn_validate(p)) return rc;
   const qagnn_gemm_nn_args& a = *p.a;
   const NnRoute r = nn_route(p);
+  const uint32_t* slots = p.a1_slots;
+  if (slots && !nn_reads_amax(r)) {
+    QAGNN_REQUIRE(a.a_amax1, QAGNN_EINVAL, "gemm_nn: slot words without the word they fold into");
+    if (int rc = launch_amax_reduce(reinterpret_cast<const float*>(slots), AMAX_SLOT_WORDS, const_cast<uint32_t*>(a.a_amax1), stream)) return rc;
+    slots = nullptr;
+  }
   if (r.family == NnFamily::FP32) return launch_nn(r, a, stream);
   if (r.family == NnFamily::SPLIT) return launch_nn_split(r, a, p.B1n, p.ldn1, p.B2n, p.ldn2, stream);
-  if (r.b == NnB::IN_KERNEL) return launch_nn2(r, a, p.B1n, p.ldn1, p.B2n, p.ldn2, stream);
+  if (r.b == NnB::IN_KERNEL) return launch_nn2(r, a, p.B1n, p.ldn1, p.B2n, p.ldn2, slots, stream);
   if (r.b == NnB::PACK) {
     QAGNN_REQUIRE(aligned16(p.ws), QAGNN_EINVAL, "gemm_nn: the pack workspace must be 16-byte aligned");
     if (int rc = launch_pack_b(r.np, a, p.B1n, p.ldn1, p.B2n, p.ldn2, p.ws, stream)) return rc;
   }
-  return launch_nn2(r, a, static_cast<const float*>(r.b == NnB::PACK ? p.ws : r.image), cdiv(a.No, 16), nullptr, 0, stream);
+  return launch_nn2(r, a, static_cast<const float*>(r.b == NnB::PACK ? p.ws : r.image), cdiv(a.No, 16), nullptr, 0, slots, stream);
 }
 
 static int tn_chunk_rows(int R, int blocks_per_chunk, int per_cu, int ktile, int lo) {
diff --git a/qagnn_amd/csrc/gemm_nn2.hip b/qagnn_amd/csrc/gemm_nn2.hip
--- a/qagnn_amd/csrc/gemm_nn2.hip
+++ b/qagnn_amd/csrc/gemm_nn2.hip
@@ -88,7 +88,7 @@
 template <int NT, bool AFFINE, bool STATS, int NP, bool PACKED, int WV = 4>
 __global__ __launch_bounds__(WV * 64) __attribute__((amdgpu_waves_per_eu(2, 2))) void k_gemm_nn2(qagnn_gemm_nn_args a, const float* __restrict__ B1n,
                                                                                           int ldn1, const float* __restrict__ B2n, int ldn2,
-                                                                                          int ntiles) {
+                                                                                          int ntiles, const uint32_t* __restrict__ a1_slots) {
   static_assert(WV == 4 || (WV == 8 && PACKED), "the staggered block takes B by DMA only");
   static_assert(NP == 3 || (NP <= 2 && PACKED && WV == 4), "the scaled fp16 forms (two pieces: three MFMAs; one piece: one MFMA): packed B, 4-wave blocks");
   static_assert(!(AFFINE && STATS), "no product needs both");
@@ -134,7 +134,13 @@
   uint32_t fa = 127u;
   float sa = 1.f;
   if constexpr (NP <= 2) {
-    uint32_t mb = a.a_amax1[0];
+    uint32_t mb;
+    if (a1_slots) {
+      mb = amax_slots_fold(a1_slots);
+      if (blockIdx.x == 0 && tid == 0) const_cast<uint32_t*>(a.a_amax1)[0] = mb;
+    } else {
+      mb = a.a_amax1[0];
+    }
     if (K2 > 0 && a.a_amax2) mb = max(mb, a.a_amax2[0]);
     fa = __builtin_amdgcn_readfirstlane(h2_scale_field(mb));
     sa = h2_field_to_scale(fa);
@@ -575,13 +581,26 @@
 #undef QAGNN_NN2_SIX_T
 
 template <int NT, bool AFFINE, bool STATS, int NP, bool PACKED, int WV>
-static int launch_i(const NnRoute& r, const qagnn_gemm_nn_args& b, const float* B1n, int ldn1, const float* B2n, int ldn2, hipStream_t stream) {
+static int launch_i(const NnRoute& r, const qagnn_gemm_nn_args& b, const float* B1n, int ldn1, const float* B2n, int ldn2, const uint32_t* a1_slots,
+                    hipStream_t stream) {
   const size_t lds = nn2_lds_bytes<NT, STATS, WV, NP>(AFFINE ? 2 * ((b.K1 + 31) & ~31) * 4 : 0);
   constexpr int lds_max = nn2_lds_bytes<NT, STATS, WV, NP>(AFFINE ? 2 * 256 * 4 : 0);
   if (int rc = raise_lds_limit<k_gemm_nn2<NT, AFFINE, STATS, NP, PACKED, WV>>(lds_max, "k_gemm_nn2")) return rc;
-  k_gemm_nn2<NT, AFFINE, STATS, NP, PACKED, WV><<<r.grid, WV * 64, lds, stream>>>(b, B1n, ldn1, B2n, ldn2, r.ntiles);
+  k_gemm_nn2<NT, AFFINE, STATS, NP, PACKED, WV><<<r.grid, WV * 64, lds, stream>>>(b, B1n, ldn1, B2n, ldn2, r.ntiles, NP <= 2 ? a1_slots : nullptr);
   QAGNN_LAUNCH_CHECK("k_gemm_nn2");
   return QAGNN_OK;
+}
+
+__device__ __forceinline__ float pack_row_absmax(const float* __restrict__ row, int K, int k0) {
+  float m = 0.f;
+  for (int k = k0; k < K; k += 16 * 8) {
+    float4 v[8];
+#pragma unroll
+    for (int u = 0; u < 8; ++u) v[u] = k + 16 * u < K ? ld4(row + k + 16 * u) : make_float4(0.f, 0.f, 0.f, 0.f);
+#pragma unroll
+    for (int u = 0; u < 8; ++u) m = fmaxf(fmaxf(m, fmaxf(fabsf(v[u].x), fabsf(v[u].y))), fmaxf(fabsf(v[u].z), fabsf(v[u].w)));
+  }
+  return m;
 }
 
 template <int NP>
@@ -594,14 +613,8 @@
     const int nn = j * 16 + (lane & 15);
     float m = 0.f;
     if (nn < No) {
-      for (int k = (lane >> 4) * 4; k < K1; k += 16) {
-        const float4 v = ld4(B1n + (int64_t)nn * ldn1 + k);
-        m = fmaxf(fmaxf(m, fmaxf(fabsf(v.x), fabsf(v.y))), fmaxf(fabsf(v.z), fabsf(v.w)));
-      }
-      for (int k = (lane >> 4) * 4; k < K2; k += 16) {
-        const float4 v = ld4(B2n + (int64_t)nn * ldn2 + k);
-        m = fmaxf(fmaxf(m, fmaxf(fabsf(v.x), fabsf(v.y))), fmaxf(fabsf(v.z), fabsf(v.w)));
-      }
+      m = pack_row_absmax(B1n + (int64_t)nn * ldn1, K1, (lane >> 4) * 4);
+      if (K2 > 0) m = fmaxf(m, pack_row_absmax(B2n + (int64_t)nn * ldn2, K2, (lane >> 4) * 4));
     }
     const uint32_t fb = h2_scale_field(__builtin_bit_cast(uint32_t, wave_max(m)));
     sb = h2_field_to_scale(fb);
@@ -671,7 +684,8 @@
 
 }
 
-int launch_nn2(const NnRoute& r, const qagnn_gemm_nn_args& a, const float* B1n, int ldn1, const float* B2n, int ldn2, hipStream_t stream) {
+int launch_nn2(const NnRoute& r, const qagnn_gemm_nn_args& a, const float* B1n, int ldn1, const float* B2n, int ldn2, const uint32_t* a1_slots,
+               hipStream_t stream) {
   qagnn_gemm_nn_args b = a;
   b.xcd_remap = 1;
   const int shape = r.b == NnB::IN_KERNEL ? 0 : r.wv == 8 ? 4 : r.np;
@@ -684,9 +698,9 @@
         return QAGNN_EUNSUPPORTED;
       } else {
         if constexpr (NT != 8) {
-          if (r.stats) return nn2::launch_i<NT, false, true, NP, PACKED, WV>(r, b, B1n, ldn1, B2n, ldn2, stream);
-        }
-        return dispatch_bool(r.affine, [&](auto aff) { return nn2::launch_i<NT, aff.value, false, NP, PACKED, WV>(r, b, B1n, ldn1, B2n, ldn2, stream); });
+          if (r.stats) return nn2::launch_i<NT, false, true, NP, PACKED, WV>(r, b, B1n, ldn1, B2n, ldn2, a1_slots, stream);
+        }
+        return dispatch_bool(r.affine, [&](auto aff) { return nn2::launch_i<NT, aff.value, false, NP, PACKED, WV>(r, b, B1n, ldn1, B2n, ldn2, a1_slots, stream); });
       }
     });
   });
diff --git a/qagnn_amd/csrc/gemm_split.hip b/qagnn_amd/csrc/gemm_split.hip
--- a/qagnn_amd/csrc/gemm_split.hip
+++ b/qagnn_amd/csrc/gemm_split.hip
@@ -351,7 +351,13 @@
   }
 }
 
-struct TnAmax { const uint32_t* a; const uint32_t* a2; const uint32_t* b; };
+struct TnAmax { const uint32_t* a; const uint32_t* a2; const uint32_t* b; const uint32_t* b_slots; };
+__device__ __forceinline__ uint32_t tn_b_bits(const TnAmax& amax) {
+  if (!amax.b_slots) return amax.b[0];
+  const uint32_t m = amax_slots_fold(amax.b_slots);
+  if (blockIdx.x == 0 && blockIdx.y == 0 && blockIdx.z == 0 && threadIdx.x == 0) const_cast<uint32_t*>(amax.b)[0] = m;
+  return m;
+}
 template <int KT, int NT, bool AFFINE, bool GATHER, int NP = 3>
 __global__ __launch_bounds__(TTHR) __attribute__((amdgpu_waves_per_eu(2, 2))) void k_gemm_tn_split(
     const float* __restrict__ A, int lda, const float* __restrict__ B, int ldb, float* __restrict__ P, int R, int Ka, int No,
@@ -391,7 +397,7 @@
   float sa = 1.f, sb = 1.f;
   if constexpr (NP <= 2) {
     fa = __builtin_amdgcn_readfirstlane(h2_scale_field(second ? amax.a2[0] : amax.a[0]));
-    fb = __builtin_amdgcn_readfirstlane(h2_scale_field(amax.b[0]));
+    fb = __builtin_amdgcn_readfirstlane(h2_scale_field(tn_b_bits(amax)));
     sa = h2_field_to_scale(fa);
     sb = h2_field_to_scale(fb);
   }
@@ -610,7 +616,7 @@
   float sa = 1.f, sb = 1.f;
   if constexpr (NP <= 2) {
     fa = __builtin_amdgcn_readfirstlane(h2_scale_field(second ? amax.a2[0] : amax.a[0]));
-    fb = __builtin_amdgcn_readfirstlane(h2_scale_field(amax.b[0]));
+    fb = __builtin_amdgcn_readfirstlane(h2_scale_field(tn_b_bits(amax)));
     sa = h2_field_to_scale(fa);
     sb = h2_field_to_scale(fb);
   }
@@ -872,7 +878,7 @@
 
 #define QAGNN_TN_ARGS p.A1, p.lda1, p.B, p.ldb, p.ws, p.R, p.Ka1, p.No, p.a_scale, p.a_shift, r.chunk_rows
 static TnAmax tn_amax(const TnRoute& r, const TnProduct& p) {
-  return r.np == 3 ? TnAmax{nullptr, nullptr, nullptr} : TnAmax{p.amax[0], p.two ? p.amax[1] : nullptr, p.amax[2]};
+  return r.np == 3 ? TnAmax{nullptr, nullptr, nullptr, nullptr} : TnAmax{p.amax[0], p.two ? p.amax[1] : nullptr, p.amax[2], p.b_slots};
 }
 template <int KT, int NT, bool AFFINE, int NP = 3>
 static int launch_tn_ws_i(const TnRoute& r, const TnProduct& p, hipStream_t stream) {
diff --git a/qagnn_amd/csrc/graph_prep.hip b/qagnn_amd/csrc/graph_prep.hip
--- a/qagnn_amd/csrc/graph_prep.hip
+++ b/qagnn_amd/csrc/graph_prep.hip
@@ -449,7 +449,7 @@
 }
 
 extern "C" const char* qagnn_last_error(void) { return g_err; }
-extern "C" int qagnn_abi_version(void) { return 22; }
+extern "C" int qagnn_abi_version(void) { return 23; }
 
 extern "C" int64_t qagnn_graph_storage_elems(int32_t N, int32_t E, int32_t R, int32_t T) {
   const int64_t Ep = (int64_t)E + N, C = (int64_t)R * T * T + T;
diff --git a/qagnn_amd/csrc/hop.hip b/qagnn_amd/csrc/hop.hip
--- a/qagnn_amd/csrc/hop.hip
+++ b/qagnn_amd/csrc/hop.hip
@@ -37,17 +37,21 @@
 }
 
 enum { AM_X = 0, AM_S = 1, AM_AGGR = 2, AM_H1 = 3, AM_Y = 4, AM_DOUT = 5, AM_DH1 = 6, AM_DKMQ = 7 };
+enum { SL_AGGR = 16, SL_Y = SL_AGGR + AMAX_SLOT_WORDS, SL_DOUT = SL_Y + AMAX_SLOT_WORDS };
+static_assert(SL_DOUT + AMAX_SLOT_WORDS == QAGNN_HOP_AMAX_WORDS, "a hop's amax block: 16 words + three slot arrays");
 struct HopAmax {
   bool on;
   uint32_t* x;
   uint32_t* s;
   uint32_t* y;
   uint32_t* own;
+  uint32_t* x_slots;
+  bool y_slots;
 };
 static bool hop_h2(const qagnn_hop_args* h) { return h->gemm_split >= 2 && h->amax != nullptr && h->batch_stats && nn_rows_packed(h->N); }
 static int hop_pieces(const qagnn_hop_args* h) { return h->gemm_split == 3 ? 1 : 0; }
 static HopAmax hop_amax_single(const qagnn_hop_args* h) {
-  HopAmax m{hop_h2(h), nullptr, nullptr, nullptr, h->amax};
+  HopAmax m{hop_h2(h), nullptr, nullptr, nullptr, h->amax, nullptr, false};
   if (m.on) {
     m.x = h->x_amax ? const_cast<uint32_t*>(h->x_amax) : h->amax + AM_X;
     m.s = h->s_amax ? const_cast<uint32_t*>(h->s_amax) : h->amax + AM_S;
@@ -55,10 +59,14 @@
   }
   return m;
 }
+static bool hop_chained(const qagnn_hop_args* hops, int k, int l) {
+  return l > 0 && l < k && hop_h2(&hops[l]) && hop_h2(&hops[l - 1]) && hops[l].X == hops[l - 1].y && hops[l - 1].apply_act && !hops[l].x_amax;
+}
 static HopAmax hop_amax_stack(const qagnn_hop_args* hops, int k, int l) {
   HopAmax m = hop_amax_single(&hops[l]);
   if (!m.on) return m;
-  if (l > 0 && hop_h2(&hops[l - 1]) && hops[l].X == hops[l - 1].y && hops[l - 1].apply_act && !hops[l].x_amax) m.x = hops[l - 1].amax + AM_Y;
+  if (hop_chained(hops, k, l)) { m.x = hops[l - 1].amax + AM_Y; m.x_slots = hops[l - 1].amax + SL_Y; }
+  m.y_slots = hop_chained(hops, k, l + 1);
   if (l > 0 && hop_h2(&hops[0]) && hops[l].S == hops[0].S && hops[l].SP == hops[0].SP && !hops[l].s_amax)
     m.s = hops[0].s_amax ? const_cast<uint32_t*>(hops[0].s_amax) : hops[0].amax + AM_S;
   return m;
@@ -82,13 +90,15 @@
 }
 
 static int hop_nn(const qagnn_hop_args* h, const qagnn_gemm_nn_args* a, const float* B1n, int ldn1, const float* B2n, int ldn2,
-                  float* pkws, int64_t pk_elems, qagnn_stream_t stream) {
-  return gemm_nn(NnProduct{a, h->gemm_split != 0, B1n, ldn1, B2n, ldn2, pkws, pk_elems * 4}, (hipStream_t)stream);
+                  float* pkws, int64_t pk_elems, qagnn_stream_t stream, const uint32_t* a1_slots = nullptr) {
+  return gemm_nn(NnProduct{a, h->gemm_split != 0, B1n, ldn1, B2n, ldn2, pkws, pk_elems * 4, a1_slots}, (hipStream_t)stream);
 }
 static int hop_tn(const qagnn_hop_args* h, const float* A1, int Ka1, const float* A2, int Ka2, const float* B, int No, float* C, const float* sc,
-                  const float* sh, const uint32_t* am_a1, const uint32_t* am_a2, const uint32_t* am_b, float* tnws, qagnn_stream_t stream) {
-  return gemm_tn(tn_product(A1, Ka1, Ka1, A2, Ka2, Ka2, B, No, C, No, h->N, No, sc, sh, tnws, am_a1, am_a2, am_b, h->gemm_split == 3 ? 1 : 2),
-                 (hipStream_t)stream);
+                  const float* sh, const uint32_t* am_a1, const uint32_t* am_a2, const uint32_t* am_b, float* tnws, qagnn_stream_t stream,
+                  const uint32_t* b_slots = nullptr) {
+  TnProduct p = tn_product(A1, Ka1, Ka1, A2, Ka2, Ka2, B, No, C, No, h->N, No, sc, sh, tnws, am_a1, am_a2, am_b, h->gemm_split == 3 ? 1 : 2);
+  p.b_slots = b_slots;
+  return gemm_tn(p, (hipStream_t)stream);
 }
 
 static int hop_fwd_one(const qagnn_hop_args* h, const HopAmax& am, bool x_ready, bool s_ready, qagnn_stream_t stream) {
@@ -113,16 +123,15 @@
   ga.C = h->KMQ; ga.ldc = 3 * DP; ga.M = N; ga.No = 3 * DP;
   ga.rowtab = h->TT; ga.ldt = 3 * DP; ga.rowidx = h->ntype;
   if (am.on) { ga.a_amax1 = am.x; ga.a_amax2 = SP > 0 ? am.s : nullptr; ga.pieces = hop_pieces(h); }
-  HOP_TRY(hop_nn(h, &ga, h->Wx, DP, SP > 0 ? h->Ws : nullptr, SP, pkws, pk_elems, stream));
+  HOP_TRY(hop_nn(h, &ga, h->Wx, DP, SP > 0 ? h->Ws : nullptr, SP, pkws, pk_elems, stream, am.on && x_ready ? am.x_slots : nullptr));
   HOP_TRY(launch_edge_attn_fwd(h->g, h->KMQ, 3 * DP, h->EkEm, 2 * DP, h->HP, h->qscale, score, h->a, h->alpha, h->aggr, DP,
-                               am.on ? ampart : nullptr, (hipStream_t)stream));
-  if (am.on) HOP_TRY(launch_amax_reduce(ampart, N, am.own + AM_AGGR, (hipStream_t)stream));
+                               am.on ? am.own + SL_AGGR : nullptr, (hipStream_t)stream));
   qagnn_gemm_nn_args g1 = {};
   g1.A1 = h->aggr; g1.lda1 = DP; g1.K1 = DP; g1.B1 = h->W1t; g1.ldb1 = DP; g1.C = h->h1; g1.ldc = DP; g1.M = N; g1.No = DP; g1.bias = h->b1;
   const bool fused_stats = h->batch_stats && h->gemm_split && DP > 192 && DP <= 208;
   if (fused_stats) g1.colstat_part = crws;
   if (am.on) { g1.a_amax1 = am.own + AM_AGGR; g1.pieces = hop_pieces(h); }
-  HOP_TRY(hop_nn(h, &g1, h->W1, DP, nullptr, 0, pkws, pk_elems, stream));
+  HOP_TRY(hop_nn(h, &g1, h->W1, DP, nullptr, 0, pkws, pk_elems, stream, am.on ? am.own + SL_AGGR : nullptr));
   const double Rd = (double)N;
   const float unbias = (float)(Rd / (Rd - 1.0 > 1.0 ? Rd - 1.0 : 1.0));
   const bool h1_bound = am.on && fused_stats;
@@ -153,7 +162,10 @@
   HOP_TRY(hop_nn(h, &g2, h->W2, DP, nullptr, 0, pkws, pk_elems, stream));
   if (h->apply_act) {
     QAGNN_REQUIRE(h->p_drop >= 0.f && h->p_drop < 1.f, QAGNN_EINVAL, "hop_fwd: p=%f", h->p_drop);
-    HOP_TRY(launch_gelu_dropout(h->out, nullptr, h->y, (int64_t)N * DP, h->p_drop, h->seed, am.on ? am.y : nullptr, ampart, (hipStream_t)stream));
+    if (am.on && am.y_slots)
+      HOP_TRY(launch_gelu_dropout_slots(h->out, nullptr, h->y, (int64_t)N * DP, h->p_drop, h->seed, am.own + SL_Y, (hipStream_t)stream));
+    else
+      HOP_TRY(launch_gelu_dropout(h->out, nullptr, h->y, (int64_t)N * DP, h->p_drop, h->seed, am.on ? am.y : nullptr, ampart, (hipStream_t)stream));
   }
   return QAGNN_OK;
 }
@@ -249,10 +261,12 @@
 
   const float* dout = h->dy;
   const bool h2 = am.on && DP > 192 && DP <= 208;
+  const uint32_t* const s_dout = h2 && h->apply_act ? am.own + SL_DOUT : nullptr;
   uint32_t* const w_dout = h2 ? am.own + AM_DOUT : nullptr, *const w_dh1 = h2 ? am.own + AM_DH1 : nullptr, *const w_dkmq = h2 ? am.own + AM_DKMQ : nullptr;
   const uint32_t* const w_h1 = h2 ? am.own + AM_H1 : nullptr, *const w_aggr = h2 ? am.own + AM_AGGR : nullptr;
   if (h->apply_act) {
-    HOP_TRY(launch_gelu_dropout(h->out, h->dy, bufA, (int64_t)N * DP, h->p_drop, h->seed, w_dout, ampart, (hipStream_t)stream));
+    if (h2) HOP_TRY(launch_gelu_dropout_slots(h->out, h->dy, bufA, (int64_t)N * DP, h->p_drop, h->seed, am.own + SL_DOUT, (hipStream_t)stream));
+    else HOP_TRY(launch_gelu_dropout(h->out, h->dy, bufA, (int64_t)N * DP, h->p_drop, h->seed, nullptr, nullptr, (hipStream_t)stream));
     dout = bufA;
   } else if (h2) {
     HOP_TRY(qagnn_absmax_f32(dout, (int64_t)N * DP, w_dout, stream));
@@ -260,7 +274,7 @@
   if (h->ones_col < 0)
     HOP_TRY(qagnn_colreduce_f32(0, dout, DP, nullptr, DP, N, DP, nullptr, 1, nullptr, nullptr, nullptr, nullptr, nullptr, 1.0f, h->db2, crws, stream));
   if (ss->side) HOP_TRY(stream_after(ss->side, ss->main, ss->take()));
-  HOP_TRY(hop_tn(h, h->h1, DP, nullptr, 0, dout, DP, h->dW2t, scale, shift, w_h1, nullptr, w_dout, tnws, wstream));
+  HOP_TRY(hop_tn(h, h->h1, DP, nullptr, 0, dout, DP, h->dW2t, scale, shift, w_h1, nullptr, w_dout, tnws, wstream, s_dout));
   if (h->ones_col >= 0 && h->db2 != h->dW2t + (int64_t)h->ones_col * DP) {
     hipError_t he = hipMemcpyAsync(h->db2, h->dW2t + (int64_t)h->ones_col * DP, (size_t)DP * sizeof(float), hipMemcpyDeviceToDevice, (hipStream_t)wstream);
     if (he != hipSuccess) { set_error("hop_bwd: db2 copy failed: %s", hipGetErrorString(he)); return QAGNN_EHIP; }
@@ -268,7 +282,7 @@
   qagnn_gemm_nn_args gr = {};
   gr.A1 = dout; gr.lda1 = DP; gr.K1 = DP; gr.B1 = h->W2; gr.ldb1 = DP; gr.C = bufB; gr.ldc = DP; gr.M = N; gr.No = DP;
   gr.a_amax1 = w_dout; gr.pieces = hop_pieces(h);
-  HOP_TRY(hop_nn(h, &gr, h->W2t, DP, nullptr, 0, pkws, pk_elems, stream));
+  HOP_TRY(hop_nn(h, &gr, h->W2t, DP, nullptr, 0, pkws, pk_elems, stream, s_dout));
   HOP_TRY(qagnn_colreduce_f32(2, bufB, DP, h->h1, DP, N, DP, nullptr, 1, mean, invstd, scale, shift, nullptr, 1.0f, h->dbn, crws, stream));
   HOP_TRY(launch_bn_relu_bwd_colsum(bufB, h->h1, bufC, DP, N, DP, mean, invstd, scale, shift, h->gamma, h->dbn, h->dbn + DP,
                                     h->batch_stats ? (float)(1.0 / (double)N) : 0.f, nullptr, h->db1, crws, w_dh1, (hipStream_t)stream));
```
